# YujiaoShi/HighlyAccurate

Hardware: AMD Instinct MI355X
Metric: image-pairs/sec through N-iter LM pose loop, KITTI shapes (higher is better)
Workload: dtype bf16; 1 GPU; BASELINE configs[1]: LM_S2GP.forward(mode='test'), sat 512x512, grd 256x1024, VGG-16 two-branch, level 3, 5 LM iters x 3 levels, 3-DoF, random-init weights; pairs_per_gpu=32, global_batch=32, parallelism=batch-sharded x1, no collective

## Files before the change

### highlyaccurate_amd/VGG.py

```python
from __future__ import annotations

import ctypes as C

import torch
import torch.nn as nn

from . import _lib

_W_ORDER = ['conv0', 'conv2', 'conv5', 'conv7', 'conv10', 'conv12', 'conv14',
            'conv_dec1.1', 'conv_dec1.3', 'conv_dec2.1', 'conv_dec2.3', 'conv_dec3.1', 'conv_dec3.3',
            'conf0.1', 'conf1.1', 'conf2.1', 'conf3.1']
_LEVEL_SEL = {-1: [0], -2: [1], -3: [2], 2: [1, 2], 3: [0, 1, 2], 4: [0, 1, 2, 3]}
_CH = (256, 128, 64, 16)


def _dtype_code(precision: str) -> int:
    if precision == 'bf16':
        return _lib.HLA_BF16
    if precision == 'fp16':
        return _lib.HLA_F16
    if precision == 'fp32':
        return _lib.HLA_F32
    if precision == 'fp16x3':
        return _lib.HLA_F16X3
# ... 21 lines not shown
            b = sd[name + '.bias']
            if i == 0:
                versions.append((b.data_ptr(), b._version))
            b = b.detach().contiguous().float()
            keep.append(b)
            prm.b[i] = b.data_ptr()
    return prm, keep, tuple(versions)


def _packed_weights(module: 'VGGUnet', prm, versions, dt: int, device):
    key = (dt, str(device), versions)
    cache = module.__dict__.setdefault('_hla_packed', {})
    if cache.get('key') != key:
        lib = _lib.load()
        buf = cache.get('buf')
        nbytes = lib.hla_vgg_packed_weight_bytes(dt)
        if buf is None or buf.numel() != nbytes or buf.device != device:
            buf = torch.empty(nbytes, dtype=torch.uint8, device=device)
        _lib.check(lib.hla_vgg_pack_weights(C.byref(prm), _lib.ptr(buf), dt, _lib.stream_ptr()), 'hla_vgg_pack_weights')
        cache['key'], cache['buf'] = key, buf
    return cache['buf']


def _image_window(x: torch.Tensor):
    x = x.float()
    B, _, H, W = x.shape
    sb, sc, sh, sw = x.stride()
    if not (sw == 1 and sh == W and sc >= H * W and (B == 1 or sb == 3 * sc)):
        x = x.contiguous()
        sc = H * W
    return x, sc


@_lib.on_device(lambda module, x, *a, **k: x)
def vgg_forward_nhwc(module: 'VGGUnet', x: torch.Tensor, want_conf: bool = True, defer_norm: bool = False,
                     save_for_backward: bool = False, first_row8: int = 0, feat16: bool = False):
    _lib.require_gpu(x, 'VGGUnet input')
    if x.dim() != 4 or x.shape[1] != 3:
        raise ValueError(f'expected [B,3,H,W], got {tuple(x.shape)}')
    lib = _lib.load()
    x, x_plane = _image_window(x)
    B, _, H, W = x.shape
    _lib.same_device(('input', x), ('parameters', module.conv0.weight))
    dt = _dtype_code(module.precision)
    prm, keep, versions = _param_table(module)
    packed = _packed_weights(module, prm, versions, dt, x.device)
    L = 4 if module.level == 4 else 3
    fdt = torch.float32
    if feat16:
        if not (defer_norm and not save_for_backward and L == 3 and dt in (_lib.HLA_BF16, _lib.HLA_F16)):
            raise ValueError("feat16 needs precision 'bf16' / 'fp16', defer_norm=True, level 3 and no save_for_backward")
        fdt = torch.float16
    fold = bool(getattr(module, 'folded', False))
    if fold:
        if feat16 or first_row8:
            raise ValueError('VGGUnet_G2S: feat16 / first_row8 do not apply to the folded maps')
        if W % 16:
            raise ValueError(f'VGGUnet_G2S folds [h,w] -> [2h,w/2] down to the W/8-wide map: W must be a multiple of 16, got {W}')

    def hw(l, folded):
        h, w = H >> (3 - l), W >> (3 - l)
        return (2 * h, w // 2) if folded else (h, w)

    feats = [torch.empty(B, *hw(l, fold), 64 if l == 3 else _CH[l], device=x.device, dtype=fdt) for l in range(L)]
    confs = [torch.empty(B, *hw(l, fold and l > 0), device=x.device, dtype=torch.float32) if want_conf else None
             for l in range(L)]
    inv_norm = torch.empty(L, B, device=x.device, dtype=torch.float64)
    fp = (C.c_void_p * 4)(*([f.data_ptr() for f in feats] + [0] * (4 - L)))
    cp = (C.c_void_p * 4)(*([(c.data_ptr() if c is not None else 0) for c in confs] + [0] * (4 - L)))
    flags = (_lib.HLA_VGG_WANT_CONF if want_conf else 0) | (_lib.HLA_VGG_DEFER_NORM if defer_norm else 0) | \
            (_lib.HLA_VGG_FEAT16 if feat16 else 0) | (_lib.HLA_VGG_FOLD_DECODER if fold else 0)
    nbytes = lib.hla_vgg_workspace_bytes_flags(B, H, W, L, dt, flags) if fold else lib.hla_vgg_workspace_bytes(B, H, W, L, dt)
    ws = torch.empty(nbytes, dtype=torch.uint8, device=x.device)
    if save_for_backward:
        if not defer_norm:
            raise ValueError('save_for_backward needs defer_norm=True (the backward works on the raw maps)')
        flags |= _lib.HLA_VGG_SAVE_FOR_BACKWARD
    rc = lib.hla_vgg_forward(_lib.ptr(x), x_plane, C.byref(prm), _lib.ptr(packed), fp, cp, _lib.ptr(inv_norm), _lib.ptr(ws), nbytes,
                             B, H, W, L, dt, flags, int(first_row8), _lib.stream_ptr())
    _lib.check(rc, 'hla_vgg_forward')
    if save_for_backward:
        return feats, confs, inv_norm, dict(x=x, x_version=x._version, x_plane=x_plane, ws=ws, feats=feats, inv_norm=inv_norm, dt=dt, L=L)
    return feats, confs, inv_norm


@_lib.on_device(lambda module, ctx, *a, **k: ctx['x'])
def vgg_backward_nhwc(module: 'VGGUnet', ctx: dict, d_feats, confs=None, d_confs=None, scale_invariant: bool = False,
                      first_row8: int = 0, flat: bool = False, dense: bool = False, stats: dict = None,
                      wgrad_two_phase: int = 0):
    lib = _lib.load()
    x, dt = ctx['x'], ctx['dt']
    if x._version != ctx.get('x_version', x._version):
        raise RuntimeError('the input image saved for the backward of VGGUnet has been modified by an inplace operation '
                           f"(version {x._version}, expected {ctx['x_version']}): conv0's weight gradient reads it again")
    B, _, H, W = x.shape
    prm, keep, versions = _param_table(module)
    cache = module.__dict__.setdefault('_hla_packed_T', {})
    key = (dt, str(x.device), versions)
    if cache.get('key') != key:
        buf = torch.empty(lib.hla_vgg_packed_weight_T_bytes(dt), dtype=torch.uint8, device=x.device)
        _lib.check(lib.hla_vgg_pack_weights_T(C.byref(prm), _lib.ptr(buf), dt, _lib.stream_ptr()), 'hla_vgg_pack_weights_T')
        cache['key'], cache['buf'] = key, buf
    sd = dict(module.named_parameters())
    grads, gs = {}, _lib.VggGrads()
    shapes = [(name + '.weight', tuple(sd[name + '.weight'].shape)) for name in _W_ORDER[:11]] + \
             [(name + '.bias', tuple(sd[name + '.bias'].shape)) for name in _W_ORDER[:7]]
    sizes = [int(torch.Size(shp).numel()) for _, shp in shapes]
    flat_buf = torch.empty(sum(sizes), device=x.device, dtype=torch.float32)
    o = 0
    for (key, shp), n in zip(shapes, sizes):
        grads[key] = flat_buf[o:o + n].view(shp)
        o += n
    for i, name in enumerate(_W_ORDER[:11]):
        gs.dw[i] = grads[name + '.weight'].data_ptr()
        if i < 7:
            gs.db[i] = grads[name + '.bias'].data_ptr()
    L = ctx.get('L', 3)
    padded = {}
    if L == 4:
        for i, name, shape in ((11, 'conv_dec3.1', (64, 128, 3, 3)), (12, 'conv_dec3.3', (64, 64, 3, 3))):
            g = torch.empty(shape, device=x.device, dtype=torch.float32)
            padded[name + '.weight'] = g
            gs.dw[i] = g.data_ptr()
    cp = dcp = None
    if d_confs is not None:
        dcs = [d.contiguous().float() for d in d_confs]
        cp = (C.c_void_p * 4)(*([c.data_ptr() for c in confs] + [0] * (4 - L)))
        dcp = (C.c_void_p * 4)(*([d.data_ptr() for d in dcs] + [0] * (4 - L)))
        for l in range(L):
            name = f'conf{l}.1.weight'
            if l == 3:
                g = torch.empty(1, 64, 3, 3, device=x.device, dtype=torch.float32)
                padded[name] = g
            else:
                g = torch.empty_like(sd[name], dtype=torch.float32, memory_format=torch.contiguous_format)
                grads[name] = g
            gs.dw[13 + l] = g.data_ptr()
    dfs = [d.contiguous().float() for d in d_feats]
    fp = (C.c_void_p * 4)(*([f.data_ptr() for f in ctx['feats']] + [0] * (4 - L)))
    dp = (C.c_void_p * 4)(*([d.data_ptr() for d in dfs] + [0] * (4 - L)))
    fold = bool(getattr(module, 'folded', False))
    nbytes = lib.hla_vgg_bwd_workspace_bytes_flags(B, H, W, L, dt, _lib.HLA_VGG_BWD_FOLD_DECODER) if fold \
        else lib.hla_vgg_bwd_workspace_bytes(B, H, W, L, dt)
    ws = torch.empty(nbytes, dtype=torch.uint8, device=x.device)
    rc = lib.hla_vgg_backward(_lib.ptr(x), ctx.get('x_plane', 0), C.byref(prm), _lib.ptr(cache['buf']), _lib.ptr(ctx['ws']), fp, _lib.ptr(ctx['inv_norm']),
                              dp, cp, dcp, C.byref(gs), _lib.ptr(ws), nbytes, B, H, W, L, dt,
                              (_lib.HLA_VGG_BWD_SCALE_INVARIANT if scale_invariant else 0)
                              | (_lib.HLA_VGG_BWD_DENSE if dense else 0)
                              | (_lib.HLA_VGG_BWD_WGRAD_TWO_PHASE if int(wgrad_two_phase) & 1 else 0)
                              | (_lib.HLA_VGG_BWD_WGRAD0_UNFUSED if int(wgrad_two_phase) & 2 else 0)
                              | (_lib.HLA_VGG_BWD_FOLD_DECODER if getattr(module, 'folded', False) else 0),
                              int(first_row8), _lib.stream_ptr())
    _lib.check(rc, 'hla_vgg_backward')
    if stats is not None and fold:
        stats['live_tiles'], stats['total_tiles'] = 0, 0
    elif stats is not None:
        torch.cuda.current_stream().synchronize()
        live, total = C.c_longlong(0), C.c_longlong(0)
        _lib.check(lib.hla_vgg_backward_live_tiles(_lib.ptr(ws), B, H, W, L, dt, C.byref(live), C.byref(total)),
                   'hla_vgg_backward_live_tiles')
        stats['live_tiles'], stats['total_tiles'] = live.value, total.value
    for name, g in padded.items():
        co, ci = sd[name].shape[:2]
        grads[name] = g[:co, :ci].contiguous()
    return (grads, flat_buf) if flat else grads

# ... 78 lines not shown
```

### highlyaccurate_amd/_lib.py

```python
from __future__ import annotations

import ctypes as C
import os

import torch

HERE = os.path.dirname(os.path.abspath(__file__))
LIB_PATH = os.environ.get('HLA_LIB') or os.path.join(HERE, 'libhla.so')

HLA_F32, HLA_BF16, HLA_F16, HLA_F16X3 = 0, 1, 2, 3
HLA_VGG_WANT_CONF, HLA_VGG_DEFER_NORM, HLA_VGG_SAVE_FOR_BACKWARD, HLA_VGG_FEAT16 = 1, 2, 4, 8
HLA_VGG_FOLD_DECODER = 16
HLA_VGG_BWD_SCALE_INVARIANT = 1
HLA_VGG_BWD_DENSE = 2
HLA_VGG_BWD_WGRAD_TWO_PHASE = 4
HLA_VGG_BWD_WGRAD0_UNFUSED = 8
HLA_VGG_BWD_FOLD_DECODER = 16
ABI_VERSION = 24


class HlaError(RuntimeError):
    pass


class VggParams(C.Structure):
    _fields_ = [('w', C.c_void_p * 17), ('b', C.c_void_p * 7)]


class S2GLevel(C.Structure):
    _fields_ = [('sat_feat', C.c_void_p), ('grd_feat', C.c_void_p), ('grd_conf', C.c_void_p), ('xyz', C.c_void_p),
                ('sat_inv_norm', C.c_void_p), ('grd_inv_norm', C.c_void_p),
                ('A', C.c_int), ('h', C.c_int), ('w', C.c_int), ('C', C.c_int), ('row0', C.c_int), ('grd_row_skip', C.c_int),
                ('meter_per_pixel', C.c_double), ('centre', C.c_double), ('feat_dtype', C.c_int)]


class S2GConfig(C.Structure):
    _fields_ = [('ford', C.c_int), ('n_levels', C.c_int), ('n_iters', C.c_int), ('level_first', C.c_int),
                ('using_weight', C.c_int), ('use_hessian', C.c_int), ('dof', C.c_int),
                ('shift_range_lat', C.c_double), ('shift_range_lon', C.c_double), ('rotation_range', C.c_double),
                ('damping', C.c_double * 3), ('keep', C.c_void_p), ('keep_stride', C.c_size_t),
                ('optimizer', C.c_int), ('beta1', C.c_double), ('beta2', C.c_double), ('count_in_view', C.c_int),
                ('grd_grad_overwrite', C.c_int), ('deterministic', C.c_int), ('proj', C.c_int)]


class FillRegion(C.Structure):
    _fields_ = [('ptr', C.c_void_p), ('chunk_bytes', C.c_size_t), ('stride_bytes', C.c_size_t), ('n_chunks', C.c_int)]


class VggGrads(C.Structure):
    _fields_ = [('dw', C.c_void_p * 17), ('db', C.c_void_p * 7)]


class S2GLevelGrad(C.Structure):
    _fields_ = [('d_sat_feat', C.c_void_p), ('d_grd_feat', C.c_void_p), ('d_grd_conf', C.c_void_p)]


class ProfRecord(C.Structure):
    _fields_ = [('kernel_id', C.c_int), ('ms', C.c_float), ('flops', C.c_double), ('bytes', C.c_double)]


HLA_POSE_LOSS_F32, HLA_POSE_LOSS_F64 = 0, 1


class PoseLossArgs(C.Structure):
    _fields_ = [('x', C.c_void_p * 3), ('x_stride', (C.c_longlong * 3) * 3), ('gt', C.c_void_p * 3), ('gt_stride', C.c_longlong * 3),
                ('coe', C.c_double * 3), ('B', C.c_int), ('N', C.c_int), ('L', C.c_int), ('gt_dtype', C.c_int)]


_lib = None


def _check_binary(lib: C.CDLL, path: str) -> None:
    lib.hla_abi_version.restype = C.c_int
    have = lib.hla_abi_version()
    if have != ABI_VERSION:
        raise HlaError(f'{path}: ABI version {have}, this binding needs {ABI_VERSION}; rebuild it '
                       f'(python -m highlyaccurate_amd.build --force)')
    try:
        fn = lib.hla_sizeof_struct
    except AttributeError:
        raise HlaError(f'{path}: no hla_sizeof_struct export; rebuild it') from None
    fn.restype, fn.argtypes = C.c_size_t, [C.c_int]
    for sid, cls in enumerate((VggParams, VggGrads, S2GLevel, S2GConfig, S2GLevelGrad, ProfRecord, PoseLossArgs, FillRegion)):
        if fn(sid) != C.sizeof(cls):
            raise HlaError(f'{path}: sizeof({cls.__name__}) is {fn(sid)} in the library and {C.sizeof(cls)} in the binding')


def load() -> C.CDLL:
    global _lib
    if _lib is not None:
        return _lib
    from . import build as _b
    try:
        want = _b.source_hash()
    except _b.SourcesMissing as e:
        if not os.path.exists(LIB_PATH):
            raise HlaError(f'{LIB_PATH} is missing and so are its sources: {e}') from None
        want = _b.lib_hash(LIB_PATH)
    if _b.lib_hash(LIB_PATH) != want and not (os.environ.get('HLA_LIB') and os.environ.get('HLA_ALLOW_STALE') == '1'):
        if os.environ.get('HLA_LIB'):
            raise HlaError(f'{LIB_PATH} (HLA_LIB) was not built from the sources in {_b.CSRC}; rebuild it')
        if not _b.have_compiler():
            what = 'is missing' if not os.path.exists(LIB_PATH) else 'is stale (built from different sources)'
            raise HlaError(f'{LIB_PATH} {what} and there is no hipcc to rebuild it; highlyaccurate_amd has no fallback path')
        _b.build()
    lib = C.CDLL(LIB_PATH)
    _check_binary(lib, LIB_PATH)
    vp, i, sz = C.c_void_p, C.c_int, C.c_size_t
    lib.hla_last_error.restype = C.c_char_p
    lib.hla_source_hash.restype = C.c_char_p
    lib.hla_vgg_workspace_bytes.restype = sz
    lib.hla_vgg_workspace_bytes.argtypes = [i, i, i, i, i]
    lib.hla_vgg_workspace_bytes_flags.restype = sz
    lib.hla_vgg_workspace_bytes_flags.argtypes = [i, i, i, i, i, i]
    lib.hla_vgg_forward.restype = i
    lib.hla_vgg_forward.argtypes = [vp, sz, C.POINTER(VggParams), vp, C.POINTER(vp), C.POINTER(vp), vp, vp, sz,
                                    i, i, i, i, i, i, i, vp]
    lib.hla_vgg_packed_weight_bytes.restype = sz
    lib.hla_vgg_packed_weight_bytes.argtypes = [i]
    lib.hla_vgg_pack_weights.restype = i
    lib.hla_vgg_pack_weights.argtypes = [C.POINTER(VggParams), vp, i, vp]
    lib.hla_vgg_packed_weight_T_bytes.restype = sz
    lib.hla_vgg_packed_weight_T_bytes.argtypes = [i]
    lib.hla_vgg_pack_weights_T.restype = i
    lib.hla_vgg_pack_weights_T.argtypes = [C.POINTER(VggParams), vp, i, vp]
    lib.hla_vgg_bwd_workspace_bytes.restype = sz
    lib.hla_vgg_bwd_workspace_bytes.argtypes = [i, i, i, i, i]
    lib.hla_vgg_bwd_workspace_bytes_flags.restype = sz
    lib.hla_vgg_bwd_workspace_bytes_flags.argtypes = [i, i, i, i, i, i]
    lib.hla_vgg_backward_live_tiles.restype = i
    lib.hla_vgg_backward_live_tiles.argtypes = [vp, i, i, i, i, i, C.POINTER(C.c_longlong), C.POINTER(C.c_longlong)]
    lib.hla_vgg_backward.restype = i
    lib.hla_vgg_backward.argtypes = [vp, sz, C.POINTER(VggParams), vp, vp, C.POINTER(vp), vp, C.POINTER(vp), C.POINTER(vp), C.POINTER(vp), C.POINTER(VggGrads),
                                     vp, sz, i, i, i, i, i, i, i, vp]
    lib.hla_resize_bilinear.restype = i
    lib.hla_resize_bilinear.argtypes = [vp, vp, vp, i, vp, vp, i, vp, vp, i, i, i, i, i, vp]
    lib.hla_sat_tile.restype = i
    lib.hla_sat_tile.argtypes = [vp, vp, vp, i, i, i, vp]
    lib.hla_grid_sample.restype = i
    lib.hla_grid_sample.argtypes = [vp, vp, vp, vp, vp, i, i, i, i, i, i, i, vp]
    lib.hla_grid_sample_bwd.restype = i
    lib.hla_grid_sample_bwd.argtypes = [vp, vp, vp, vp, vp, vp, vp, vp, i, i, i, i, i, i, i, vp]
    lib.hla_s2g_workspace_bytes.restype = sz
    lib.hla_s2g_workspace_bytes.argtypes = [C.POINTER(S2GConfig), C.POINTER(S2GLevel), i]
    lib.hla_g2s_workspace_bytes.restype = sz
    lib.hla_g2s_workspace_bytes.argtypes = [C.POINTER(S2GConfig), C.POINTER(S2GLevel), i]
    lib.hla_g2s_lm_solve.restype = i
    lib.hla_g2s_lm_solve.argtypes = [C.POINTER(S2GConfig), C.POINTER(S2GLevel), vp, i, i, vp, vp, vp, vp, sz, i, vp]
    lib.hla_g2s_bwd_workspace_bytes.restype = sz
    lib.hla_g2s_bwd_workspace_bytes.argtypes = [C.POINTER(S2GConfig), C.POINTER(S2GLevel), i]
    lib.hla_g2s_lm_solve_bwd.restype = i
    lib.hla_g2s_lm_solve_bwd.argtypes = [C.POINTER(S2GConfig), C.POINTER(S2GLevel), C.POINTER(S2GLevelGrad), vp, i, i, vp, vp,
                                         vp, vp, vp, vp, sz, i, vp]
    lib.hla_s2g_lm_solve.restype = i
    lib.hla_s2g_lm_solve.argtypes = [C.POINTER(S2GConfig), C.POINTER(S2GLevel), vp, vp, vp, vp, vp, vp, vp, sz, i, vp]
    lib.hla_s2g_bwd_workspace_bytes.restype = sz
    lib.hla_s2g_bwd_workspace_bytes.argtypes = [C.POINTER(S2GConfig), C.POINTER(S2GLevel), i]
    lib.hla_s2g_lm_solve_bwd.restype = i
    lib.hla_s2g_lm_solve_bwd.argtypes = [C.POINTER(S2GConfig), C.POINTER(S2GLevel), C.POINTER(S2GLevelGrad), vp, vp, vp, vp,
                                         vp, vp, vp, vp, sz, i, vp]
    lib.hla_zero_fill.restype = i
    lib.hla_zero_fill.argtypes = [C.POINTER(FillRegion), i, i, vp]
    lib.hla_pose_loss.restype = i
    lib.hla_pose_loss.argtypes = [C.POINTER(PoseLossArgs), vp, vp]
    lib.hla_pose_loss_bwd.restype = i
    lib.hla_pose_loss_bwd.argtypes = [C.POINTER(PoseLossArgs), C.POINTER(vp), C.POINTER(vp), C.POINTER((C.c_longlong * 3) * 3), vp]
    ll, dbl = C.c_longlong, C.c_double
    lib.hla_orien_corr_workspace_bytes.restype = sz
    lib.hla_orien_corr_workspace_bytes.argtypes = [i, i, i, i, i]
    lib.hla_orien_corr.restype = i
    lib.hla_orien_corr.argtypes = [vp, vp, vp, vp, vp, vp, vp, vp, vp, sz, i, i, i, i, i, vp]
    lib.hla_orien_corr_bwd.restype = i
    lib.hla_orien_corr_bwd.argtypes = [vp, vp, vp, vp, vp, vp, vp, vp, vp, vp, vp, sz, i, i, i, i, i, vp]
    lib.hla_orien_window_bwd.restype = i
    lib.hla_orien_window_bwd.argtypes = [vp, vp, vp, vp, i, i, i, i, i, i, vp]
    lib.hla_orien_triplet_loss.restype = i
    lib.hla_orien_triplet_loss.argtypes = [vp, vp, ll, dbl, dbl, vp, i, i, i, vp]
    lib.hla_orien_triplet_loss_bwd.restype = i
    lib.hla_orien_triplet_loss_bwd.argtypes = [vp, vp, ll, dbl, dbl, vp, vp, i, i, vp]
    lib.hla_prof_enable.restype = i
    lib.hla_prof_enable.argtypes = [i]
    lib.hla_prof_kernel_name.restype = C.c_char_p
    lib.hla_prof_kernel_name.argtypes = [i]
    lib.hla_prof_mfma_peak.restype = i
    lib.hla_prof_mfma_peak.argtypes = [i, i, C.c_float, C.POINTER(C.c_float), vp]
    lib.hla_prof_fetch.restype = i
    lib.hla_prof_fetch.argtypes = [C.POINTER(ProfRecord), i, C.POINTER(i)]
    _lib = lib
    return lib


def zero_fill(regions, max_blocks: int = 0, stream=None) -> None:
    if not regions:
        return
    arr = (FillRegion * len(regions))()
    for k, (t, cb, sb, n) in enumerate(regions):
        arr[k].ptr = t.data_ptr() if hasattr(t, 'data_ptr') else int(t)
        arr[k].chunk_bytes, arr[k].stride_bytes, arr[k].n_chunks = int(cb), int(sb), int(n)
    check(load().hla_zero_fill(arr, len(regions), int(max_blocks), stream_ptr() if stream is None else stream), 'hla_zero_fill')

# ... 60 lines not shown
```

### highlyaccurate_amd/_s2gp.py

```python
from __future__ import annotations

import ctypes as C

import numpy as np
import torch
import torch.nn as nn

from . import _lib, utils
from .VGG import VGGUnet, vgg_forward_nhwc, vgg_backward_nhwc

KITTI_K = [[582.9802, 0.0, 496.2420], [0.0, 482.7076, 125.0034], [0.0, 0.0, 1.0]]
FORD_K_FL = [945.391406, 0.0, 855.502825, 0.0, 945.668274, 566.372868, 0.0, 0.0, 1.0]
FORD_H_FL, FORD_W_FL = 860, 1656


_FEAT_DTYPES = {torch.float32: _lib.HLA_F32, torch.bfloat16: _lib.HLA_BF16, torch.float16: _lib.HLA_F16}

PHASE_HOOK = None


def _phase(name: str):
    h = PHASE_HOOK
    if h is not None:
        h(name)


def ground_plane_table(K_ori, grd_H, grd_W, ori_H, ori_W):
    K = torch.tensor(K_ori, dtype=torch.float32).reshape(1, 3, 3)
    Ks = K.clone()
    Ks[:, :1, :] = K[:, :1, :] * grd_W / ori_W
    Ks[:, 1:2, :] = K[:, 1:2, :] * grd_H / ori_H
    Kinv = torch.inverse(Ks)
    v, u = torch.meshgrid(torch.arange(0, grd_H, dtype=torch.float32),
                          torch.arange(0, grd_W, dtype=torch.float32), indexing='ij')
    uv1 = torch.stack([u, v, torch.ones_like(u)], dim=-1).unsqueeze(0)
    xyz_w = torch.sum(Kinv[:, None, None, :, :] * uv1[:, :, :, None, :], dim=-1)
    y = xyz_w[..., 1:2]
    w = utils.Camera_height / torch.where(torch.abs(y) > utils.EPS, y, utils.EPS * torch.ones_like(y))
    return (xyz_w * w)[0].contiguous()


def polar_plane_table(grd_H, grd_W):
    v, u = torch.meshgrid(torch.arange(0, grd_H, dtype=torch.float32),
                          torch.arange(0, grd_W, dtype=torch.float32), indexing='ij')
    theta = u / grd_W * np.pi / 4
    radius = (1 - v / grd_H) * 30
    z = radius * torch.cos(np.pi / 4 - theta)
    x = -radius * torch.sin(np.pi / 4 - theta)
    y = utils.Camera_height * torch.ones_like(z)
    return torch.stack([x, y, z], dim=-1).contiguous()


def ford_K_network_input():
    K = torch.tensor(FORD_K_FL, dtype=torch.float32).reshape(3, 3)
    out = torch.zeros_like(K)
    out[0] = K[0] / FORD_W_FL * 1024
    out[1] = K[1] / FORD_H_FL * 256
    out[2] = K[2]
    return out.tolist()


def _loss_tensor_ops(shift_lats, shift_lons, thetas, gt_shift_lat, gt_shift_lon, gt_theta, coe_shift_lat, coe_shift_lon, coe_theta):
    d_lat = torch.abs(shift_lats - gt_shift_lat[:, None, None]).mean(dim=0)
    d_lon = torch.abs(shift_lons - gt_shift_lon[:, None, None]).mean(dim=0)
    d_th = torch.abs(thetas - gt_theta[:, None, None]).mean(dim=0)
    losses = coe_shift_lat * d_lat + coe_shift_lon * d_lon + coe_theta * d_th
    return (losses.mean(), losses[0] - losses[-1], d_lat[0] - d_lat[-1], d_lon[0] - d_lon[-1], d_th[0] - d_th[-1],
            losses[-1], d_lat[-1], d_lon[-1], d_th[-1])


def _pose_loss_args(xs, gts, coes):
    a = _lib.PoseLossArgs()
    B, N, L = xs[0].shape
    for k in range(3):
        a.x[k], a.gt[k], a.gt_stride[k], a.coe[k] = xs[k].data_ptr(), gts[k].data_ptr(), gts[k].stride(0), float(coes[k])
        for j in range(3):
            a.x_stride[k][j] = xs[k].stride(j)
    a.B, a.N, a.L = B, N, L
    a.gt_dtype = _lib.HLA_POSE_LOSS_F64 if gts[0].dtype == torch.float64 else _lib.HLA_POSE_LOSS_F32
    return a


class _PoseLossFn(torch.autograd.Function):

    @staticmethod
    def forward(ctx, cols, coes, gt_lat, gt_lon, gt_th, *xs):
        views = [xs[0][..., c] for c in cols] if cols is not None else list(xs)
        gts = (gt_lat, gt_lon, gt_th)
        L = views[0].shape[2]
        out = torch.empty(1 + 8 * L, dtype=gt_lat.dtype, device=views[0].device)
        args = _pose_loss_args(views, gts, coes)
        _lib.check(_lib.load().hla_pose_loss(C.byref(args), _lib.ptr(out), _lib.stream_ptr()), 'hla_pose_loss')
# ... 221 lines not shown
        p0 = init_pose.to(dev).float().contiguous() if init_pose is not None else None
        rc = lib.hla_s2g_lm_solve(C.byref(cfg), lv, _lib.ptr(R_FL), _lib.ptr(T_FL), _lib.ptr(p0), _lib.ptr(rand_uv),
                                  _lib.ptr(trace), _lib.ptr(neq), _lib.ptr(ws), nbytes, B, _lib.stream_ptr())
        _lib.check(rc, 'hla_s2g_lm_solve')
        risky = cfg.optimizer == 3 or (cfg.optimizer == 0 and (cfg.use_hessian or min(cfg.damping[i] for i in range(3)) <= 0.0))
        if risky or strict:
            raise_like_reference(trace, neq[:, :, 14] if strict else None, level_first,
                                 gn_norm2=neq[:, :, 0] if cfg.optimizer == 3 else None)
        self.last_trace, self.last_normal_eq = trace.detach(), neq
        return trace

    def lm_grad_buffers(self, sat_feats, grd_feats, grd_confs, row0s, row_skips, grd_first_row8=0, overwrite=True, deterministic=False):
        L = len(sat_feats)
        regions = []
        d_sat = [torch.empty_like(t) for t in sat_feats]
        if not deterministic:
            regions += [(d, d.numel() * 4, d.numel() * 4, 1) for d in d_sat]
        d_grd = []
        for l, t in enumerate(grd_feats):
            d = torch.empty_like(t)
            lo, hi = (max(0, (grd_first_row8 << l) - 2) if grd_first_row8 else 0), row0s[l] - row_skips[l]
            if not overwrite:
                hi = t.shape[1]
            if hi > lo:
                row = t.shape[2] * t.shape[3] * 4
                regions.append((d.data_ptr() + lo * row, (hi - lo) * row, t.shape[1] * row, t.shape[0]))
            d_grd.append(d)
        d_conf = [torch.empty_like(grd_confs[l]) if (self.using_weight and grd_confs[l] is not None) else None for l in range(L)]
        regions += [(d, d.numel() * 4, d.numel() * 4, 1) for d in d_conf if d is not None]
        d_lambda = torch.empty(4, device=sat_feats[0].device, dtype=torch.float64)
        keep = d_sat + d_grd
        for k0 in range(0, len(regions), 16):
            _lib.zero_fill(regions[k0:k0 + 16])
        del keep
        return d_sat, d_grd, d_conf, d_lambda

    @_lib.on_device(lambda self, sat_feats, *a, **k: sat_feats[0])
    def lm_backward(self, sat_feats, grd_feats, grd_confs, grd_hw, trace, normal_eq, d_trace, extra=None, level_first=0,
                    init_pose=None, sat_inv_norm=None, grd_inv_norm=None, keep=None, grd_first_row8=0, overwrite=True):
        lib = _lib.load()
        dev = sat_feats[0].device
        B, L = sat_feats[0].shape[0], len(sat_feats)
        cfg, lv, R_FL, T_FL = self._lm_structs(sat_feats, grd_feats, grd_confs, grd_hw, extra, level_first,
                                               sat_inv_norm, grd_inv_norm)
        if keep is not None:
            cfg.keep, cfg.keep_stride = keep.data_ptr(), keep.shape[1]
        det = bool(getattr(self.args, 'deterministic_backward', 0))
        cfg.deterministic = 1 if det else 0
        cfg.grd_grad_overwrite = 1 if overwrite else 0
        d_sat, d_grd, d_conf, d_lambda = self.lm_grad_buffers(sat_feats, grd_feats, grd_confs, [lv[l].row0 for l in range(L)],
                                                              [lv[l].grd_row_skip for l in range(L)], grd_first_row8, overwrite, det)
        gr = (_lib.S2GLevelGrad * L)()
        for l in range(L):
            gr[l].d_sat_feat, gr[l].d_grd_feat = d_sat[l].data_ptr(), d_grd[l].data_ptr()
            gr[l].d_grd_conf = d_conf[l].data_ptr() if d_conf[l] is not None else 0
        dtr = d_trace.to(dev).float().contiguous()
        nbytes = lib.hla_s2g_bwd_workspace_bytes(C.byref(cfg), lv, B)
        ws = torch.empty(nbytes, dtype=torch.uint8, device=dev)
        p0 = init_pose.to(dev).float().contiguous() if init_pose is not None else None
        for attempt, bits in enumerate((1, 30) if det else (0,)):
            cfg.deterministic = bits
            if attempt:
                for t in d_conf:
                    if t is not None:
                        t.zero_()
                if not overwrite:
                    for t in d_grd:
                        t.zero_()
            rc = lib.hla_s2g_lm_solve_bwd(C.byref(cfg), lv, gr, _lib.ptr(R_FL), _lib.ptr(T_FL), _lib.ptr(p0), _lib.ptr(trace),
                                          _lib.ptr(normal_eq), _lib.ptr(dtr), _lib.ptr(d_lambda), _lib.ptr(ws), nbytes, B,
                                          _lib.stream_ptr())
            _lib.check(rc, 'hla_s2g_lm_solve_bwd')
            if not det or float(d_lambda[3]) == 0.0:
                break
        else:
            raise RuntimeError(f'deterministic_backward: the fixed-point range of d(loss)/d(sat map) was exceeded in {int(d_lambda[3])} '
                               '(step, sample) pairs even with 2^20 of head room -- the adjoints of the LM chain grow by more than that '
                               'from its last step to an earlier one; the result is not valid (run without args.deterministic_backward)')
        return d_sat, d_grd, d_conf, d_lambda[:3]

    def _features(self, sat_map, grd_img, want_conf, return_confs):
        f16 = (self.SatFeatureNet.precision in ('bf16', 'fp16') and self.level == 3 and bool(getattr(self.args, 'lm_feat16', 1)))
        small = sat_map.shape[0] <= int(getattr(self.args, 'small_batch_two_streams', 4))
        if small:
            cur = torch.cuda.current_stream()
            side = _side_stream(sat_map.device)
            side.wait_stream(cur)
            with torch.cuda.stream(side):
                sat_feats, _, sat_inv = vgg_forward_nhwc(self.SatFeatureNet, sat_map, want_conf=False, defer_norm=True, feat16=f16)
            sat_map.record_stream(side)
        else:
            sat_feats, _, sat_inv = vgg_forward_nhwc(self.SatFeatureNet, sat_map, want_conf=False, defer_norm=True, feat16=f16)
        grd_in = grd_img
        dead_ok = (not return_confs and self.level == 3 and getattr(self.args, 'Optimizer', 'LM') == 'LM'
                   and bool(getattr(self.args, 'ground_crop', 1)) and not self.polar)
        skip = dead_ground_rows(grd_img.shape[-2]) if dead_ok else 0
        if skip:
            grd_in = grd_img[:, :, skip:, :]
        f8 = ((grd_img.shape[-2] // 8) // 2 - skip // 8) if dead_ok else 0
        f8 = f8 if f8 >= 4 else 0
        grd_feats, grd_confs, grd_inv = vgg_forward_nhwc(self.GrdFeatureNet, grd_in, want_conf=want_conf, defer_norm=True,
                                                         first_row8=f8, feat16=f16)
        if small:
            cur.wait_stream(side)
            for t in list(sat_feats) + [sat_inv]:
                t.record_stream(cur)
        L = self._levels
        return L(sat_feats), L(sat_inv), L(grd_feats), L(grd_confs), L(grd_inv)

    @_lib.on_device(lambda self, sat_map, *a, **k: sat_map)
    def localise(self, sat_map, grd_img, want_conf, extra, level_first, init_pose, return_confs=True):
        if sat_map.dim() != 4 or grd_img.dim() != 4 or sat_map.shape[0] != grd_img.shape[0] or sat_map.shape[1] != 3 \
                or grd_img.shape[1] != 3 or sat_map.shape[2] != sat_map.shape[3]:
            raise ValueError(f'expected sat_map [B,3,A,A] and grd_img [B,3,H,W] with one B, got {tuple(sat_map.shape)} '
                             f'and {tuple(grd_img.shape)}')
        _lib.same_device(('sat_map', sat_map), ('grd_img', grd_img), ('parameters', self.damping))
        if self.polar and self.ford and level_first:
            raise NotImplementedError("LM_S2GP_Ford(proj='polar') with level_first=1: the reference's level-first loop reads only "
                                      "the bottom half of the polar maps (it has no proj branch); that combination is not built")
        if torch.is_grad_enabled() and any(p.requires_grad for p in self.parameters()):
            names = [n for n, _ in self.named_parameters()]
            params = [p for _, p in self.named_parameters()]
            out = _LocaliseFn.apply(self, names, sat_map, grd_img, want_conf, extra, level_first, init_pose, *params)
            return out[0], list(out[1:]) if want_conf else [None] * self.level
        sat_feats, sat_inv, grd_feats, grd_confs, grd_inv = self._features(sat_map, grd_img, want_conf, return_confs)
        trace = self.lm_solve(sat_feats, grd_feats, grd_confs, grd_img.shape[-2:], extra, level_first, init_pose,
                              sat_inv, grd_inv)
        return trace, grd_confs


def draw_reinit(n_steps: int, B: int, device):
    r = torch.rand(n_steps, 2, B).mul_(2.0).add_(-1.0)
    if torch.device(device).type == 'cuda':
        return r.pin_memory().to(device, non_blocking=True)
    return r.to(device)


def raise_like_reference(trace, in_view, level_first, gn_norm2=None):
    B, N, L, _ = trace.shape
    steps = N * L
    tr = (trace.permute(0, 2, 1, 3) if level_first else trace).reshape(B, steps, 3)
    bad = ~torch.isfinite(tr).all(-1)
    if gn_norm2 is not None:
        first = torch.where(bad.any(1), bad.float().argmax(1), torch.full((B,), steps - 1, device=bad.device))
        poisoned = bad.any(1) & (gn_norm2.t().gather(1, first[:, None])[:, 0] == 0)
        bad = bad & ~poisoned[:, None]
    bad = bad.any(0)
    k_s = int(torch.nonzero(bad)[0]) if bool(bad.any()) else steps
    k_a = steps
    if in_view is not None:
        empty = in_view.sum(1) == 0
        k_a = int(torch.nonzero(empty)[0]) if bool(empty.any()) else steps
    if k_a < steps and k_a <= k_s:
        raise AssertionError(f'grid_sample: no pixel of the batch is sampled inside the map in LM step {k_a} (jacobian.py:172)')
    if k_s < steps:
        raise RuntimeError(f'linalg.inv: the normal matrix of LM step {k_s} is singular '
                           '(use_hessian / zero damping / Gauss-Newton with no Jacobian support in one pose component)')


_SIDE_STREAMS = {}


def _side_stream(device) -> 'torch.cuda.Stream':
    idx = torch.device(device).index if torch.device(device).index is not None else torch.cuda.current_device()
    st = _SIDE_STREAMS.get(idx)
    if st is None:
        st = _SIDE_STREAMS[idx] = torch.cuda.Stream(device=idx)
    return st


def dead_ground_rows(H: int) -> int:
    return max(0, ((H // 2 - 34) // 8) * 8)


def _bwd_first_row8(model, grd_hw, x21_rows: int) -> int:
    inv = getattr(model.args, 'Optimizer', 'LM') == 'LM' and not model.polar
    f8 = (grd_hw[0] // 8) // 2 - (grd_hw[0] - x21_rows * 2) // 8
    return f8 if (inv and f8 >= 4 and model.level == 3 and bool(getattr(model.args, 'bwd_trim', 1))) else 0


class _LocaliseFn(torch.autograd.Function):

    @staticmethod
# ... 98 lines not shown
```

### highlyaccurate_amd/csrc/capi.hip

```cpp
#include "common.h"
#include <string.h>

static thread_local char g_err[512] = "";

void hla_set_error(const char* fmt, ...) {
  va_list ap;
  va_start(ap, fmt);
  vsnprintf(g_err, sizeof(g_err), fmt, ap);
  va_end(ap);
}

extern "C" const char* hla_last_error(void) { return g_err; }
extern "C" int hla_abi_version(void) { return HLA_ABI_VERSION; }

#ifndef HLA_SOURCE_HASH_HEX
#define HLA_SOURCE_HASH_HEX "unknown"
#endif
static const char kSourceHash[] = "HLA_SOURCE_HASH=" HLA_SOURCE_HASH_HEX;
extern "C" const char* hla_source_hash(void) { return kSourceHash + 16; }

extern "C" size_t hla_sizeof_struct(int id) {
  switch (id) {
    case HLA_STRUCT_VGG_PARAMS: return sizeof(hla_vgg_params);
    case HLA_STRUCT_VGG_GRADS: return sizeof(hla_vgg_grads);
    case HLA_STRUCT_S2G_LEVEL: return sizeof(hla_s2g_level);
    case HLA_STRUCT_S2G_CONFIG: return sizeof(hla_s2g_config);
    case HLA_STRUCT_S2G_LEVEL_GRAD: return sizeof(hla_s2g_level_grad);
    case HLA_STRUCT_PROF_RECORD: return sizeof(hla_prof_record);
    case HLA_STRUCT_POSE_LOSS_ARGS: return sizeof(hla_pose_loss_args);
    case HLA_STRUCT_FILL_REGION: return sizeof(hla_fill_region);
    default: return 0;
  }
}
```

### highlyaccurate_amd/csrc/conv_kernels.h

```cpp
#pragma once
#include "common.h"
#include <type_traits>

typedef __bf16 bf16;
typedef _Float16 f16;
using f32x16 = __attribute__((ext_vector_type(16))) float;
using bf16x8 = __attribute__((ext_vector_type(8))) __bf16;
using f16x8 = __attribute__((ext_vector_type(8))) _Float16;
using f16x4 = __attribute__((ext_vector_type(4))) _Float16;

struct split32 {
  float v;
  split32() = default;
  __host__ __device__ explicit split32(float f) : v(f) {}
  __host__ __device__ explicit operator float() const { return v; }
};
template <typename T> struct Prec { static constexpr bool SPLIT = false; static constexpr int CEPL = 16 / (int)sizeof(T); };
template <> struct Prec<split32> { static constexpr bool SPLIT = true; static constexpr int CEPL = 8; };

__device__ __host__ __forceinline__ float split_scale(unsigned amax_bits) {
  int E = (int)(amax_bits >> 23) & 0xff;
  E = E < 81 ? 81 : (E > 201 ? 201 : E);
  const unsigned bits = (unsigned)(127 + 141 - E) << 23;
  float f;
// ... 234 lines not shown
    constexpr int EPV = 16 / (int)sizeof(E), NIT = 32 * CPP / 64;
    if (PLAIN || !(mask || add)) {
#pragma unroll
      for (int c0 = 0; c0 < 32 * CPP; c0 += 64) {
        const int c = c0 + lane;
        if (c0 < chunks && c < chunks) {
          const int px = c / CPP, part = c % CPP;
          if (px < npx_valid) {
            const unsigned off = (unsigned)px * (unsigned)Cout * (unsigned)sizeof(E) + part * 16;
            *(uint4*)((char*)dst + off) = *(const uint4*)(stage + px * PITCH + part * 16);
          }
        }
      }
      return vmax;
    }
    constexpr int G = NIT < GG ? NIT : GG;
#pragma unroll
    for (int g0 = 0; g0 < NIT; g0 += G) {
      bool ok[G], ap[G];
      unsigned off[G];
      int pxs[G], parts[G];
      uint4 mk[G], ad[G];
#pragma unroll
      for (int k = 0; k < G; ++k) {
        const int c0 = (g0 + k) * 64, c = c0 + lane;
        const int px = c / CPP, part = c % CPP;
        ok[k] = c0 < chunks && c < chunks && px < npx_valid;
        pxs[k] = px; parts[k] = part;
        off[k] = ok[k] ? (unsigned)px * (unsigned)Cout * (unsigned)sizeof(E) + part * 16 : 0u;
        ap[k] = add && ok[k] && px >= add_px_lo && px < add_px_hi;
      }
      if (mask) {
#pragma unroll
        for (int k = 0; k < G; ++k) mk[k] = *(const uint4*)((const char*)mask + off[k]);
      }
      if (add) {
#pragma unroll
        for (int k = 0; k < G; ++k) ad[k] = *(const uint4*)((const char*)add + (ap[k] ? off[k] : 0u));
      }
#pragma unroll
      for (int k = 0; k < G; ++k) {
        if (ok[k]) {
          uint4 v = *(const uint4*)(stage + pxs[k] * PITCH + parts[k] * 16);
          E e[EPV], m[EPV], a2[EPV];
          __builtin_memcpy(e, &v, 16);
          if (mask) __builtin_memcpy(m, &mk[k], 16);
          if (add) __builtin_memcpy(a2, &ad[k], 16);
#pragma unroll
          for (int j = 0; j < EPV; ++j) {
            float f = (float)e[j];
            if (mask && !((float)m[j] > 0.f)) f = 0.f;
            if (ap[k]) f += (float)a2[j];
            e[j] = (E)f;
            vmax = fmaxf(vmax, fabsf(f));
          }
          __builtin_memcpy(&v, e, 16);
          *(uint4*)((char*)dst + off[k]) = v;
        }
      }
    }
    return vmax;
  }
};

enum { EPI_GENERIC = 0,
       EPI_ACT = 1,
       EPI_ACT_RAW = 2,
       EPI_ACT_RAW_NOBIAS = 3,
       EPI_DGRAD = 4,
       EPI_DGRAD_WG0 = 5 };
__host__ __device__ __forceinline__ int epilogue_mode(const ConvArgs& a) {
  if (a.wg0_part) return EPI_DGRAD_WG0;
  if (a.mask_act && a.out_act && !a.relu_act && !a.bias && !a.out_raw && !a.sumsq && !a.idx_out && !a.pool_sum) return EPI_DGRAD;
  if (!a.out_act && a.out_raw && a.raw16 && a.sumsq && !a.bias && !a.mask_act && !a.add_src && !a.idx_out && !a.pool_sum)
    return EPI_ACT_RAW_NOBIAS;
  if (a.mask_act || a.add_src || a.idx_out || a.pool_sum || !a.out_act || !a.relu_act) return EPI_GENERIC;
  if (!a.out_raw) return a.sumsq ? EPI_GENERIC : EPI_ACT;
  return a.sumsq ? (a.bias ? EPI_ACT_RAW : EPI_ACT_RAW_NOBIAS) : EPI_GENERIC;
}
template <typename T, int MT, int NT, bool POOL, int EPI = EPI_GENERIC, bool R16 = false, int STGW = 0, int SHAPE = SHAPE_32x32x16>
__device__ __forceinline__ void conv_epilogue(typename AccMap<SHAPE>::Tile (&acc)[MT][NT], const ConvArgs& a, int b, int yrow0, int x0,
                                              int cb, float* red, char* stage, float dsc = 1.f,
                                              PixBox addb = PixBox{0, 1 << 30, 0, 1 << 30},
                                              const float4* prebias = nullptr) {
  using RawT = std::conditional_t<R16, f16, float>;
  constexpr bool GEN = EPI == EPI_GENERIC, RAW = EPI == EPI_ACT_RAW || EPI == EPI_ACT_RAW_NOBIAS, DG = EPI == EPI_DGRAD;
  constexpr bool NOBIAS = EPI == EPI_ACT_RAW_NOBIAS || DG || sizeof(T) == 2;
  const bool has_raw = GEN ? a.out_raw != nullptr : RAW;
  const bool has_act = GEN ? a.out_act != nullptr : true;
  const bool relu = GEN ? a.relu_act != 0 : !DG;
  const bool pool_sum = GEN && a.pool_sum;
  const bool has_sumsq = GEN ? a.sumsq != nullptr : RAW;
  int tid = threadIdx.x;
  asm volatile("" : "+v"(tid));
  const int lane = tid & 63, wv = __builtin_amdgcn_readfirstlane(tid >> 6), even = !POOL || !(lane & 1);
  using M = AccMap<SHAPE>;
  const int Ho = POOL ? a.H >> 1 : a.H, Wo = POOL ? a.W >> 1 : a.W;
  constexpr int NPX = POOL ? 16 : 32;
  int pxq[4];
  bool colok[4];
#pragma unroll
  for (int q = 0; q < 4; ++q) {
    const int xq = M::px(lane, q);
    pxq[q] = POOL ? xq >> 1 : xq;
    colok[q] = (x0 + xq < a.W) && even;
  }
  float4 bias[NT][4];
#pragma unroll
  for (int j = 0; j < NT; ++j)
#pragma unroll
    for (int q = 0; q < 4; ++q)
      bias[j][q] = make_float4(0.f, 0.f, 0.f, 0.f);
  if (!NOBIAS && prebias) {
#pragma unroll
    for (int j = 0; j < NT; ++j)
#pragma unroll
      for (int q = 0; q < 4; ++q) bias[j][q] = prebias[j * 4 + q];
  } else if (!NOBIAS && a.bias) {
#pragma unroll
    for (int j = 0; j < NT; ++j)
#pragma unroll
      for (int q = 0; q < 4; ++q) bias[j][q] = *(const float4*)(a.bias + cb + j * 32 + M::ch(lane, q));
  }
  const int xo0 = POOL ? x0 >> 1 : x0;
  const int nvalid = min(NPX, Wo - xo0);
  float ss = 0.f, mx = 0.f;
  constexpr int ROWB = 32 * RowStager<T, NT>::PITCH;
  constexpr bool BATCH = EPI == EPI_ACT && STGW >= 2 * ROWB;
  if constexpr (BATCH) {
    constexpr int STEP = POOL ? 2 : 1, NR = MT / STEP;
    constexpr int RB = STGW / ROWB >= NR ? NR : 2;
    static_assert(NR % RB == 0, "row batches");
#pragma unroll
    for (int r0 = 0; r0 < NR; r0 += RB) {
#pragma unroll
      for (int rr = 0; rr < RB; ++rr) {
        const int i = (r0 + rr) * STEP;
        const bool rowok = yrow0 + i < a.H;
#pragma unroll
        for (int j = 0; j < NT; ++j)
#pragma unroll
          for (int q = 0; q < 4; ++q) {
            float w[4];
#pragma unroll
            for (int e = 0; e < 4; ++e) {
              float t = M::get(acc[i][j], q, e);
              if (POOL) {
                t = fmaxf(t, M::get(acc[i + 1][j], q, e));
                t = fmaxf(t, lane_xor1(t));
              }
              if (Prec<T>::SPLIT) t *= dsc;
              w[e] = t;
            }
            if (!NOBIAS) { w[0] += bias[j][q].x; w[1] += bias[j][q].y; w[2] += bias[j][q].z; w[3] += bias[j][q].w; }
            w[0] = fmaxf(w[0], 0.f); w[1] = fmaxf(w[1], 0.f); w[2] = fmaxf(w[2], 0.f); w[3] = fmaxf(w[3], 0.f);
            if (Prec<T>::SPLIT && rowok && colok[q]) mx = fmaxf(fmaxf(mx, fmaxf(w[0], w[1])), fmaxf(w[2], w[3]));
            if (even) RowStager<T, NT>::put(stage + rr * ROWB, pxq[q], j * 32 + M::ch(lane, q), w[0], w[1], w[2], w[3]);
          }
      }
      __builtin_amdgcn_sched_barrier(0);
#pragma unroll
      for (int rr = 0; rr < RB; ++rr) {
        const int y = yrow0 + (r0 + rr) * STEP;
        const size_t pix0 = ((size_t)b * Ho + (POOL ? y >> 1 : y)) * Wo + xo0;
        if (y < a.H) RowStager<T, NT>::template flush<true>(stage + rr * ROWB, (T*)a.out_act + pix0 * a.Cout + cb, NPX, nvalid, a.Cout, lane);
      }
      __builtin_amdgcn_sched_barrier(0);
// ... 48 lines not shown
              w2 = (float)(f16)fminf(fmaxf(w2, -65504.f), 65504.f); w3 = (float)(f16)fminf(fmaxf(w3, -65504.f), 65504.f);
            }
            RowStager<RawT, NT>::put(stage, pxq[q], j * 32 + M::ch(lane, q), w0, w1, w2, w3);
            if (quad_ok(q)) ss = sumsq4(ss, w0, w1, w2, w3);
            if (a.out_act)
              RowStager<T, NT>::put(stage2, pxq[q], j * 32 + M::ch(lane, q), fmaxf(w0, 0.f), fmaxf(w1, 0.f), fmaxf(w2, 0.f), fmaxf(w3, 0.f));
          }
      }
      asm volatile("" : "+v"(ss));
      __builtin_amdgcn_sched_barrier(0);
      if (row_ok) {
        RowStager<RawT, NT>::template flush<true>(stage, (RawT*)a.out_raw + pix0 * a.Cout + cb, NPX, nvalid, a.Cout, lane);
        if (a.out_act) RowStager<T, NT>::template flush<true>(stage2, (T*)a.out_act + pix0 * a.Cout + cb, NPX, nvalid, a.Cout, lane);
      }
      __builtin_amdgcn_sched_barrier(0);
      continue;
    }
    if (has_raw) {
      if (even) {
#pragma unroll
        for (int j = 0; j < NT; ++j)
#pragma unroll
          for (int q = 0; q < 4; ++q) {
            RowStager<float, NT>::put(stage, pxq[q], j * 32 + M::ch(lane, q), v[j][q][0], v[j][q][1], v[j][q][2], v[j][q][3]);
            if (quad_ok(q)) ss = sumsq4(ss, v[j][q][0], v[j][q][1], v[j][q][2], v[j][q][3]);
          }
      }
      if (row_ok) RowStager<float, NT>::template flush<true>(stage, a.out_raw + pix0 * a.Cout + cb, NPX, nvalid, a.Cout, lane);
    }
    if (has_act) {
      if (even) {
#pragma unroll
        for (int j = 0; j < NT; ++j)
#pragma unroll
          for (int q = 0; q < 4; ++q) {
            float w0 = v[j][q][0], w1 = v[j][q][1], w2 = v[j][q][2], w3 = v[j][q][3];
            if (relu) { w0 = fmaxf(w0, 0.f); w1 = fmaxf(w1, 0.f); w2 = fmaxf(w2, 0.f); w3 = fmaxf(w3, 0.f); }
            if (Prec<T>::SPLIT && quad_ok(q) && !((GEN || DG) && (a.mask_act || a.add_src)))
              mx = fmaxf(fmaxf(mx, fmaxf(fabsf(w0), fabsf(w1))), fmaxf(fabsf(w2), fabsf(w3)));
            RowStager<T, NT>::put(stage, pxq[q], j * 32 + M::ch(lane, q), w0, w1, w2, w3);
          }
      }
      const size_t o = pix0 * a.Cout + cb;
      if (GEN || DG) {
        if (row_ok) {
          const float fm = RowStager<T, NT>::template flush<false, (MT >= 4 ? 4 : 2)>(stage, (T*)a.out_act + o, NPX, nvalid, a.Cout, lane,
                                                   a.mask_act ? (const T*)a.mask_act + o : nullptr,
                                                   (a.add_src && yo >= max(a.add_row_lo, addb.y0) && yo < addb.y1) ? (const T*)a.add_src + o : nullptr,
                                                   addb.x0 - xo0, addb.x1 - xo0);
          if (Prec<T>::SPLIT) mx = fmaxf(mx, fm);
        }
      } else {
        if (row_ok) RowStager<T, NT>::template flush<true>(stage, (T*)a.out_act + o, NPX, nvalid, a.Cout, lane);
      }
    }
    if (GEN && POOL && a.idx_out) {
#pragma unroll
      for (int j = 0; j < NT; ++j)
#pragma unroll
        for (int q = 0; q < 4; ++q) {
          float am[4];
#pragma unroll
          for (int e = 0; e < 4; ++e) {
            const float t0 = M::get(acc[i][j], q, e), u = M::get(acc[i + 1][j], q, e);
            const float rown = u > t0 ? 1.f : 0.f;
            const float t = fmaxf(t0, u);
            const float t2 = lane_xor1(t), r2 = lane_xor1(rown);
            am[e] = t2 > t ? 2.f * r2 + 1.f : 2.f * rown;
          }
          if (!(lane & 1)) RowStager<unsigned char, NT>::put(stage, pxq[q], j * 32 + M::ch(lane, q), am[0], am[1], am[2], am[3]);
        }
      if (row_ok) RowStager<unsigned char, NT>::flush(stage, a.idx_out + pix0 * a.Cout + cb, NPX, nvalid, a.Cout, lane);
    }
  }
  const bool want_max = Prec<T>::SPLIT && a.amax_out;
  if (has_sumsq || want_max) {
    ss = wave_sum_f32(ss);
    if (want_max) mx = wave_max_f32(mx);
    if (lane == 0) { red[wv] = ss; red[4 + wv] = mx; }
    __syncthreads();
    if (tid == 0) {
      if (has_sumsq) {
        const int np = a.tiles_x * a.tiles_y * gridDim.y;
        const int tile = (xcd_contiguous(blockIdx.x, gridDim.x) % (a.tiles_x * a.tiles_y)) * gridDim.y + blockIdx.y;
        a.sumsq[(size_t)b * np + tile] = ((double)red[0] + (double)red[1]) + ((double)red[2] + (double)red[3]);
      }
      if (want_max) {
        const unsigned mb = __float_as_uint(fmaxf(fmaxf(red[4], red[5]), fmaxf(red[6], red[7])));
        if (mb > __hip_atomic_load(a.amax_out + b, __ATOMIC_RELAXED, __HIP_MEMORY_SCOPE_AGENT)) atomicMax(a.amax_out + b, mb);
      }
    }
  }
}

template <typename T, int MT>
__device__ __forceinline__ void conv_epilogue_wg0(f32x16 (&acc)[MT][1], const ConvArgs& a, int b, int y0, int x0, char* lds, float dsc) {
  constexpr bool SPLIT = Prec<T>::SPLIT;
  using ET = std::conditional_t<SPLIT, float, T>;
  using FT = std::conditional_t<SPLIT, f16, ET>;
  constexpr int TH = 2 * MT, IH = TH + 2, IW = 48;
  constexpr int PITCH = RowStager<ET, 1>::PITCH, CPP = RowStager<ET, 1>::CPP, NIT = 32 * CPP / 64, EPV = 16 / (int)sizeof(ET);
  constexpr int HP = RowStager<f16, 1>::PITCH, HTILE = 32 * HP;
  constexpr int KPX = KStep<FT>::PX, STG = 5120;
  static_assert(32 * PITCH <= STG && 2 * HTILE <= STG, "wave stager");
  static_assert(4 * STG + 3 * IH * IW * 4 + 2 * 16 * 64 * 4 + 16 <= 2 * (TH + 2) * HWID * PSTR, "fits the halo buffers");
  int tid = threadIdx.x;
  asm volatile("" : "+v"(tid));
  const int lane = tid & 63, wv = __builtin_amdgcn_readfirstlane(tid >> 6), wm = wv >> 1, wn = wv & 1, x = lane & 31, g = lane >> 5;
  char* stage = lds + wv * STG;
  float* in = (float*)(lds + 4 * STG);
  float* xr = in + 3 * IH * IW;
  float* redm = xr + 2 * 16 * 64;
  const int nvalid = min(32, a.W - x0), cb = wn * 32;

  int pxs[NIT], parts[NIT];
  unsigned voff[NIT];
#pragma unroll
  for (int k = 0; k < NIT; ++k) {
    const int c = k * 64 + lane;
    pxs[k] = c / CPP; parts[k] = c % CPP;
    voff[k] = pxs[k] < nvalid ? (unsigned)pxs[k] * 64u * (unsigned)sizeof(ET) + parts[k] * 16 : 0u;
  }
  constexpr int PRE = sizeof(ET) == 2 ? MT : 2;
  uint4 mk[MT][NIT];
  auto load_mask = [&](int i) __attribute__((always_inline)) {
    const int y = min(y0 + wm * MT + i, a.H - 1);
    const char* mrow = (const char*)((const ET*)a.mask_act + (((size_t)b * a.H + y) * a.W + x0) * 64 + cb);
#pragma unroll
    for (int k = 0; k < NIT; ++k) mk[i][k] = *(const uint4*)(mrow + voff[k]);
  };
#pragma unroll
  for (int i = 0; i < PRE; ++i) load_mask(i);

  constexpr int NIN = (3 * IH * IW + 255) / 256;
  float vin[NIN], amx = 0.f;
#pragma unroll
  for (int it = 0; it < NIN; ++it) {
    const int e = tid + it * 256;
    const int c = e / (IH * IW), r = e % (IH * IW), iy = r / IW, ix = r % IW;
    const int y = y0 - 1 + iy, xx = x0 - 1 + ix;
    vin[it] = 0.f;
    if (e < 3 * IH * IW && ix < HWID && y >= 0 && y < a.H && xx >= 0 && xx < a.W)
      vin[it] = a.wg0_x[((size_t)b * 3 + c) * a.wg0_x_plane + (size_t)y * a.W + xx];
  }
#pragma unroll
  for (int it = 0; it < NIN; ++it) {
    const int e = tid + it * 256;
    if (e < 3 * IH * IW) in[e] = vin[it];
    if (SPLIT) amx = fmaxf(amx, fabsf(vin[it]));
  }
  if (SPLIT) {
    amx = wave_max_f32(amx);
    if (lane == 0) redm[wv] = amx;
  }
  __syncthreads();
  float s_in = 1.f;
  if (SPLIT) s_in = split_scale(__float_as_uint(fmaxf(fmaxf(redm[0], redm[1]), fmaxf(redm[2], redm[3]))));

  f32x16 accw;
#pragma unroll
  for (int r = 0; r < 16; ++r) accw[r] = 0.f;
  const int j = lane & 31, g5 = lane >> 5;
  const int jc = j < 27 ? j / 9 : 0, jky = (j % 9) / 3, jkx = j % 3;
#pragma unroll
  for (int i = 0; i < MT; ++i) {
    if (i + PRE < MT) load_mask(i + PRE);
    const int rt = wm * MT + i;
// ... 101 lines not shown
  const uint4* wq[NT];

  __device__ __forceinline__ void prime() {
#pragma unroll
    for (int d = 0; d < WD; ++d)
#pragma unroll
      for (int kg = 0; kg < 2; ++kg)
#pragma unroll
        for (int j = 0; j < NT; ++j) wb[d][kg][j] = wq[j][(d * 2 + kg) * 64];
  }
  __device__ __forceinline__ void next_stage() {
#pragma unroll
    for (int j = 0; j < NT; ++j) wq[j] += 18 * 64;
    if (9 % RS != 0) {
      uint4 tmp[WD][2][NT];
#pragma unroll
      for (int d = 0; d < WD; ++d)
#pragma unroll
        for (int kg = 0; kg < 2; ++kg)
#pragma unroll
          for (int j = 0; j < NT; ++j) tmp[d][kg][j] = wb[(9 + d) % RS][kg][j];
#pragma unroll
      for (int d = 0; d < WD; ++d)
#pragma unroll
        for (int kg = 0; kg < 2; ++kg)
#pragma unroll
          for (int j = 0; j < NT; ++j) wb[d][kg][j] = tmp[d][kg][j];
    }
  }
};

__device__ __forceinline__ void stagger_priority() {
  const unsigned slot = __builtin_amdgcn_s_getreg((3 << 11) | (0 << 6) | 4);
  if (slot & 1) __builtin_amdgcn_s_setprio(1);
}

template <typename T, int MT, int NT, int WD, int PF, int SHAPE = SHAPE_32x32x16, typename Mid>
__device__ __forceinline__ void stage_mma(typename AccMap<SHAPE>::Tile (&acc)[MT][NT], const char* cur, const FragOff& fo,
                                          WeightRing<T, MT, NT, WD, PF>& ring, Mid&& mid) {
  constexpr int RS = WD + 1;
#pragma unroll
  for (int tap = 0; tap < 9; ++tap) {
#pragma unroll
    for (int kg = 0; kg < 2; ++kg)
#pragma unroll
      for (int j = 0; j < NT; ++j) ring.wb[(tap + WD) % RS][kg][j] = ring.wq[j][((tap + WD) * 2 + kg) * 64];
    mid(tap);
    constexpr int FPT = MT * 2, DEPTH = PF;
    auto frag_ptr = [&](int f) {
      const int tp = tap + f / FPT, r = f % FPT;
      return cur + fo.o[tp % 3][r & 1] + (tp / 3 + (r >> 1)) * HWID * PSTR;
    };
    if (tap == 0) {
#pragma unroll
      for (int f = 0; f < DEPTH; ++f) ring.pf[f] = *(const uint4*)frag_ptr(f);
    }
    __builtin_amdgcn_sched_barrier(0);
#pragma unroll
    for (int f = 0; f < FPT; ++f) {
      const int slot = (tap * FPT + f) % (DEPTH + 1), nslot = (tap * FPT + f + DEPTH) % (DEPTH + 1);
      if (tap * FPT + f + DEPTH < 9 * FPT) ring.pf[nslot] = *(const uint4*)frag_ptr(f + DEPTH);
      const int i = f >> 1, kg = f & 1;
      if constexpr (Prec<T>::SPLIT) {
#pragma unroll
        for (int c = 0; c < (kg == 0 ? 2 : 1); ++c)
#pragma unroll
          for (int j = 0; j < NT; ++j) mma16<T>(acc[i][j], ring.wb[tap % RS][c][j], ring.pf[slot]);
      } else if constexpr (SHAPE == SHAPE_16x16x32) {
#pragma unroll
        for (int c = 0; c < 2; ++c)
#pragma unroll
          for (int j = 0; j < NT; ++j) mma32<T>(acc[i][j].t[2 * kg + c], ring.wb[tap % RS][c][j], ring.pf[slot]);
      } else {
#pragma unroll
        for (int j = 0; j < NT; ++j) mma16<T>(acc[i][j], ring.wb[tap % RS][kg][j], ring.pf[slot]);
      }
      __builtin_amdgcn_sched_barrier(0);
    }
  }
  ring.next_stage();
}

template <typename T, int MT, int NT, int WM, int WN, bool POOL, int WD, bool UNPOOL = false, int SHAPE = SHAPE_32x32x16>
__global__ __launch_bounds__(256, NT == 1 ? 3 : 2) void conv3x3_kernel(ConvArgs a) {
  static_assert(WM * WN == 4, "4 waves per block");
  static_assert(SHAPE == SHAPE_32x32x16 || (sizeof(T) == 2 && !UNPOOL), "16x16x32: bf16 / f16 forward kernels only");
  using M = AccMap<SHAPE>;
  constexpr int EPL = 16 / sizeof(T), KC = SB / sizeof(T);
  constexpr int TH = WM * MT, HPIX = (TH + 2) * HWID;
  constexpr int NPIECE = (HPIX * 4 + 255) / 256;
  constexpr bool DMA = sizeof(T) == 2 && !UNPOOL && !Prec<T>::SPLIT;
  constexpr int BUF = (DMA ? NPIECE * 64 : HPIX) * PSTR;
  constexpr int NHALF = (NPIECE + 1) / 2;
  constexpr int STG = 32 * (RowStager<float, NT>::PITCH + (sizeof(T) == 2 ? RowStager<T, NT>::PITCH : 0));
  constexpr int LDSB = 2 * BUF > 4 * STG ? 2 * BUF : 4 * STG;
  __shared__ __attribute__((aligned(16))) char lds[LDSB];
  __shared__ float red[8];

  HLA_STAMP(0);
  HLA_STAMP_HWID();
  const int t = threadIdx.x, lane = t & 63, wv = __builtin_amdgcn_readfirstlane(t >> 6), wm = wv / WN, wn = wv % WN;
  const int sy0 = a.src_row_lo, sy1 = a.H;
  int tx, ty, b;
  struct { int lo0, lo1, lo2, hi0, hi1, hi2; } sb = {0, 0, 0, a.W, a.W, a.W};
  if (a.dyn) {
    const ConvDyn& d = *(const ConvDyn*)(a.dyn + a.dyn_desc);
    const int nl = d.n_live, nlive = nl * a.B;
    if ((int)blockIdx.x >= nlive) return;
    int bid = xcd_contiguous(blockIdx.x, nlive);
    b = bid / nl;
    const int e = a.dyn[d.list + bid % nl];
    ty = e >> 16; tx = e & 0xffff;
    if (d.src_bands >= 0) {
      const int sh = (a.up1 || a.unpool_idx) ? 1 : 0, nb = ((a.H >> sh) + 7) >> 3, yy = a.row_begin + ty * TH;
      const int b0 = min(max(yy - 1, 0) >> sh >> 3, nb - 1), b1 = min(yy >> sh >> 3, nb - 1), b2 = min((yy + TH) >> sh >> 3, nb - 1);
      sb.lo0 = a.dyn[d.src_bands + 2 * b0] << sh; sb.hi0 = min(a.dyn[d.src_bands + 2 * b0 + 1] << sh, a.W);
      sb.lo1 = a.dyn[d.src_bands + 2 * b1] << sh; sb.hi1 = min(a.dyn[d.src_bands + 2 * b1 + 1] << sh, a.W);
      sb.lo2 = a.dyn[d.src_bands + 2 * b2] << sh; sb.hi2 = min(a.dyn[d.src_bands + 2 * b2 + 1] << sh, a.W);
    }
  } else {
    int bid = xcd_contiguous(blockIdx.x, gridDim.x);
    tx = bid % a.tiles_x; bid /= a.tiles_x;
    ty = bid % a.tiles_y;
    b = bid / a.tiles_y;
  }
  const int y0 = a.row_begin + ty * TH, x0 = tx * 32;
  const int nstage = (a.C1 + a.C2) / KC;
  const int part = t & 3, pbase = t >> 2;
  float sx = 1.f, dsc = 1.f;
  if constexpr (Prec<T>::SPLIT) {
    unsigned m = a.amax1[b];
    if (a.amax2) m = max(m, a.amax2[b]);
    sx = split_scale(m);
    dsc = 1.f / (sx * *a.wscale);
  }

  constexpr int ES = (int)sizeof(T);
  const int sh1 = (a.up1 || a.unpool_idx) ? 1 : 0, Hs1 = a.H >> sh1, Ws1 = a.W >> sh1;
  const char* s1b = (const char*)a.src1 + (size_t)b * Hs1 * Ws1 * a.C1 * ES;
  const char* s2b = (const char*)a.src2 + (size_t)b * a.H * a.W * a.C2 * ES;
  const unsigned char* idxb = a.unpool_idx ? a.unpool_idx + (size_t)b * Hs1 * Ws1 * a.C1 : nullptr;
  int off1[NPIECE], off2[NPIECE], wo[NPIECE];
  {
    const int lo0 = __builtin_amdgcn_readfirstlane(sb.lo0), lo1 = __builtin_amdgcn_readfirstlane(sb.lo1),
              lo2 = __builtin_amdgcn_readfirstlane(sb.lo2), hi0 = __builtin_amdgcn_readfirstlane(sb.hi0),
              hi1 = __builtin_amdgcn_readfirstlane(sb.hi1), hi2 = __builtin_amdgcn_readfirstlane(sb.hi2);
#pragma unroll
    for (int i = 0; i < NPIECE; ++i) {
      const int pix = pbase + 64 * i;
      const int hy = pix / HWID, hx = pix - hy * HWID;
      const int y = y0 - 1 + hy, x = x0 - 1 + hx;
      const int xlo = hy == 0 ? lo0 : (hy == TH + 1 ? lo2 : lo1), xhi = hy == 0 ? hi0 : (hy == TH + 1 ? hi2 : hi1);
      const bool ok = pix < HPIX && y >= sy0 && y < sy1 && x >= xlo && x < xhi;
      const int psrc = DMA ? (part ^ halo_key(hx)) : part;
      constexpr int BAD = DMA ? (int)0x80000000 : -1;
      off1[i] = ok ? ((((y >> sh1) * Ws1 + (x >> sh1)) * a.C1 * ES + psrc * 16) | (DMA ? 0 : (((y & 1) << 1) | (x & 1)))) : BAD;
      off2[i] = ok ? ((y * a.W + x) * a.C2 * ES + psrc * 16) : BAD;
      wo[i] = pix >= HPIX ? -1 : (Prec<T>::SPLIT ? halo_off(pix, hx, part >> 1) + (part & 1) * 8 : halo_off(pix, hx, part));
    }
  }
  constexpr int IDW = UNPOOL ? (EPL == 8 ? 2 : 1) : 1;
  struct StageIds { unsigned w[NHALF][IDW]; };
  auto load_stage = [&](int sg, int half, uint4 (&st)[NHALF], StageIds& ids) __attribute__((always_inline)) {
    const int c0 = sg * KC;
    const bool first = c0 < a.C1;
    const char* base = first ? s1b + (size_t)c0 * ES : s2b + (size_t)(c0 - a.C1) * ES;
#pragma unroll
    for (int ii = 0; ii < NHALF; ++ii) {
      const int i = half * NHALF + ii;
      uint4 v = make_uint4(0, 0, 0, 0);
      const int o = i < NPIECE ? (first ? off1[i] : off2[i]) : -1;
      if constexpr (UNPOOL) {
#pragma unroll
        for (int k = 0; k < IDW; ++k) ids.w[ii][k] = 0xffffffffu;
      }
      if (o >= 0) {
        const unsigned ob = (unsigned)o & ~15u;
        v = *(const uint4*)(base + ob);
        if constexpr (UNPOOL) {
          const unsigned char* idp = idxb + ob / ES + c0;
#pragma unroll
          for (int k = 0; k < IDW; ++k) ids.w[ii][k] = ((const unsigned*)idp)[k];
        }
      }
      st[ii] = v;
    }
  };
  auto write_stage = [&](char* buf, int sg, int half, uint4 (&st)[NHALF], const StageIds& ids) __attribute__((always_inline)) {
#pragma unroll
    for (int ii = 0; ii < NHALF; ++ii) {
      const int i = half * NHALF + ii;
      const int w = i < NPIECE ? wo[i] : -1;
      if constexpr (UNPOOL) {
        const bool first = sg * KC < a.C1;
        const unsigned pos = (unsigned)(i < NPIECE ? (first ? off1[i] : off2[i]) : 0) & 3u;
        uint4 v = st[ii];
        if constexpr (sizeof(T) == 2) {
          typedef short s16x2 __attribute__((ext_vector_type(2)));
          const unsigned m0 = ids.w[ii][0] ^ (pos * 0x01010101u), m1 = ids.w[ii][1] ^ (pos * 0x01010101u);
          auto keep = [](unsigned m, unsigned sel) {
            s16x2 w2 = __builtin_bit_cast(s16x2, __builtin_amdgcn_perm(0u, m, sel));
            w2 = (w2 - (short)1) >> 15;
            return __builtin_bit_cast(unsigned, w2);
          };
// ... 63 lines not shown

  const int ntg0 = (blockIdx.y * WN + wn) * NT;
  typename M::Tile acc[MT][NT];
#pragma unroll
  for (int j = 0; j < NT; ++j)
#pragma unroll
    for (int q = 0; q < 4; ++q) {
      float4 b4 = make_float4(0.f, 0.f, 0.f, 0.f);
      if (sizeof(T) == 2 && a.bias) b4 = *(const float4*)(a.bias + (ntg0 + j) * 32 + M::ch(lane, q));
#pragma unroll
      for (int i = 0; i < MT; ++i) {
        M::set(acc[i][j], q, 0, b4.x); M::set(acc[i][j], q, 1, b4.y); M::set(acc[i][j], q, 2, b4.z); M::set(acc[i][j], q, 3, b4.w);
      }
    }

  const FragOff fo = frag_offsets<SHAPE>(lane, wm * MT);
  constexpr int PF = NT == 1 ? (UNPOOL && sizeof(T) == 2 ? 3 : 4) : 3;
  WeightRing<T, MT, NT, WD, PF> ring;
#pragma unroll
  for (int j = 0; j < NT; ++j) ring.wq[j] = a.wpk + (size_t)(ntg0 + j) * nstage * 18 * 64 + lane;

  uint4 st[NHALF];
  StageIds ids;
  ring.prime();
  if constexpr (DMA) {
    dma_stage(0, 0);
    asm volatile("s_waitcnt vmcnt(0)" ::: "memory");
  } else {
    uint4 st1[NHALF];
    StageIds ids1;
    load_stage(0, 0, st, ids);
    load_stage(0, 1, st1, ids1);
    write_stage(lds, 0, 0, st, ids);
    write_stage(lds, 0, 1, st1, ids1);
  }
  __syncthreads();
  HLA_STAMP(1);
  stagger_priority();

  for (int sg = 0; sg < nstage; ++sg) {
    const bool more = sg + 1 < nstage;
    char* nxt = lds + ((sg + 1) & 1) * BUF;
    stage_mma<T, MT, NT, WD, PF, SHAPE>(acc, lds + (sg & 1) * BUF, fo, ring, [&](int tap) __attribute__((always_inline)) {
      if constexpr (DMA) {
        if (tap == HLA_CONV_DMA_TAP && more) dma_stage(sg + 1, (sg + 1) & 1);
      } else {
        if (tap == HALO_TAP0 && more) load_stage(sg + 1, 0, st, ids);
        if (tap == HALO_TAP1 && more) { write_stage(nxt, sg + 1, 0, st, ids); load_stage(sg + 1, 1, st, ids); }
      }
    });
    if constexpr (DMA) {
      static_assert(!DMA || HLA_CONV_DMA_TAP <= 8 - WD, "the halo DMA must be issued before the next stage's weight fragments");
      if (more) asm volatile("s_waitcnt vmcnt(%0)" ::"n"(2 * NT * WD) : "memory");
    } else {
      if (more) write_stage(nxt, sg + 1, 1, st, ids);
    }
    if (sg == 0) HLA_STAMP(2);
    __syncthreads();
    if (sg == 0) HLA_STAMP(3);
  }
  HLA_STAMP(4);
  static_assert((LDSB / 4) % 16 == 0, "stager alignment");
  {
    char* stager = lds + wv * (LDSB / 4);
    const int mode = epilogue_mode(a);
    PixBox addb{a.add_row_lo, 1 << 30, 0, 1 << 30};
    if (a.dyn) {
      const ConvDyn& d = *(const ConvDyn*)(a.dyn + a.dyn_desc);
      if (d.add_bands >= 0) {
        const int band = (POOL ? y0 >> 1 : y0) >> 3;
        addb.x0 = a.dyn[d.add_bands + 2 * band];
        addb.x1 = a.dyn[d.add_bands + 2 * band + 1];
      }
    }
    constexpr bool RAW_SPECIAL = POOL || NT == 1;
    constexpr bool T16 = sizeof(T) == 2;
    if constexpr (UNPOOL && NT == 1 && MT == 4 && WN == 2) {
      if (mode == EPI_DGRAD_WG0) {
        conv_epilogue_wg0<T, MT>(acc, a, b, y0, x0, lds, dsc);
        HLA_STAMP(5);
        return;
      }
    }
    if (mode == EPI_ACT) conv_epilogue<T, MT, NT, POOL, EPI_ACT, false, LDSB / 4, SHAPE>(acc, a, b, y0 + wm * MT, x0, ntg0 * 32, red, stager, dsc, addb);
    else if (T16 && RAW_SPECIAL && a.raw16 && mode == EPI_ACT_RAW)
      conv_epilogue<T, MT, NT, POOL, (T16 && RAW_SPECIAL) ? EPI_ACT_RAW : EPI_GENERIC, T16 && RAW_SPECIAL, 0, SHAPE>(acc, a, b, y0 + wm * MT, x0, ntg0 * 32, red, stager, dsc, addb);
    else if (T16 && a.raw16 && mode == EPI_ACT_RAW_NOBIAS)
      conv_epilogue<T, MT, NT, POOL, T16 ? EPI_ACT_RAW_NOBIAS : EPI_GENERIC, T16, 0, SHAPE>(acc, a, b, y0 + wm * MT, x0, ntg0 * 32, red, stager, dsc, addb);
    else if (RAW_SPECIAL && mode == EPI_ACT_RAW) conv_epilogue<T, MT, NT, POOL, RAW_SPECIAL ? EPI_ACT_RAW : EPI_GENERIC, false, 0, SHAPE>(acc, a, b, y0 + wm * MT, x0, ntg0 * 32, red, stager, dsc, addb);
    else if (SHAPE == SHAPE_32x32x16 && mode == EPI_DGRAD)
      conv_epilogue<T, MT, NT, POOL, SHAPE == SHAPE_32x32x16 ? EPI_DGRAD : EPI_GENERIC, false, 0, SHAPE>(acc, a, b, y0 + wm * MT, x0, ntg0 * 32, red, stager, dsc, addb);
    else if ((RAW_SPECIAL || sizeof(T) == 2) && mode == EPI_ACT_RAW_NOBIAS)
      conv_epilogue<T, MT, NT, POOL, (RAW_SPECIAL || sizeof(T) == 2) ? EPI_ACT_RAW_NOBIAS : EPI_GENERIC, false, 0, SHAPE>(acc, a, b, y0 + wm * MT, x0, ntg0 * 32, red, stager, dsc, addb);
    else conv_epilogue<T, MT, NT, POOL, EPI_GENERIC, false, 0, SHAPE>(acc, a, b, y0 + wm * MT, x0, ntg0 * 32, red, stager, dsc, addb);
  }
  HLA_STAMP(5);
}

struct Conv02Args {
  const float* x;
  size_t x_plane;
  const uint4* w0;
  const float* b0;
  const uint4* w2;
  const float* b2;
  void* out_act;
  void* a0_out;
  unsigned char* idx_out;
  void* a2_out;
  int B, H, W, tiles_x, tiles_y;
  int row_begin;
  const float* wtail;
  unsigned* amax_out;
  unsigned* amax_a2_out;
  unsigned* amax_a0_out;
#if HLA_CONV_STAMPS
  unsigned long long* stamps;
#endif
};

template <typename T> constexpr int conv02_rounds() { return sizeof(T) == 4 ? 2 : 1; }
template <typename T> constexpr int conv02_lds_bytes() {
  return (64 * (int)sizeof(T) / SB) / conv02_rounds<T>() * (10 * HWID * PSTR) + 3 * 12 * 36 * 4;
}

template <typename T, int WD>
__global__ __launch_bounds__(256, Prec<T>::SPLIT ? 2 : 3) void conv02_kernel(Conv02Args a0) {
  constexpr bool SPLIT = Prec<T>::SPLIT;
  constexpr bool FOLD = sizeof(T) == 2 && !SPLIT;
  constexpr int EPL = Prec<T>::CEPL, KC = SB / sizeof(T), NSG = 64 / KC, NFRAG = 32 / (2 * EPL), NH = SPLIT ? 2 : 1;
  constexpr int MT = 4, NT = 1, WN = 2, TH = 8, HPIX = (TH + 2) * HWID, BUF = HPIX * PSTR, IW = 36, IH = 12;
  constexpr int ROUNDS = conv02_rounds<T>(), SPR = NSG / ROUNDS, JPR = 2 / ROUNDS;
  extern __shared__ __attribute__((aligned(16))) char smem[];
  char* lds = smem;
  float* in = (float*)(smem + SPR * BUF);
  __shared__ float red[8];
  __shared__ float red2[4];
  float a0mx = 0.f;
#if HLA_CONV_STAMPS
  struct { unsigned long long* stamps; } a = {a0.stamps};
#endif
  HLA_STAMP(0);
  HLA_STAMP_HWID();

  const int t = threadIdx.x, lane = t & 63, wv = __builtin_amdgcn_readfirstlane(t >> 6), wm = wv / WN, wn = wv % WN;
  int bid = blockIdx.x;
  const int tx = bid % a0.tiles_x; bid /= a0.tiles_x;
  const int ty = bid % a0.tiles_y;
  const int b = bid / a0.tiles_y;
  const int y0 = a0.row_begin + ty * TH, x0 = tx * 32;
  const int x = lane & 31, g = lane >> 5;

  WeightRing<T, MT, NT, WD> ring;
  ring.wq[0] = a0.w2 + (size_t)wn * NSG * 18 * 64 + lane;
  ring.prime();

  float amx = 0.f;
  constexpr int NIN = (3 * IH * IW + 255) / 256;
  float vin[NIN];
#pragma unroll
  for (int it = 0; it < NIN; ++it) {
    const int e = t + it * 256;
    const int c = e / (IH * IW), r = e % (IH * IW), iy = r / IW, ix = r % IW;
    const int y = y0 - 2 + iy, xx = x0 - 2 + ix;
    vin[it] = 0.f;
    if (e < 3 * IH * IW && y >= 0 && y < a0.H && xx >= 0 && xx < a0.W)
      vin[it] = a0.x[((size_t)b * 3 + c) * a0.x_plane + (size_t)y * a0.W + xx];
  }
#pragma unroll
  for (int it = 0; it < NIN; ++it) {
    const int e = t + it * 256;
    if (e < 3 * IH * IW) in[e] = vin[it];
    if (SPLIT) amx = fmaxf(amx, fabsf(vin[it]));
  }
  uint4 wf0[JPR][NFRAG][NH];
  auto load_w0 = [&](int j0) __attribute__((always_inline)) {
#pragma unroll
    for (int jj = 0; jj < JPR; ++jj)
#pragma unroll
      for (int f = 0; f < NFRAG; ++f)
#pragma unroll
        for (int h = 0; h < NH; ++h) wf0[jj][f][h] = a0.w0[(((j0 + jj) * NFRAG + f) * NH + h) * 64 + lane];
  };
  load_w0(0);
  if (SPLIT) {
    amx = wave_max_f32(amx);
    if (lane == 0) red[4 + wv] = amx;
  }
  __syncthreads();
  HLA_STAMP(1);

  float4 bias0[JPR][4];
  auto load_b0 = [&](int j0) __attribute__((always_inline)) {
#pragma unroll
    for (int jj = 0; jj < JPR; ++jj)
#pragma unroll
      for (int q = 0; q < 4; ++q) bias0[jj][q] = *(const float4*)(a0.b0 + (j0 + jj) * 32 + q * 8 + g * 4);
  };
  float s_in = 1.f, s_a0 = 1.f, d0 = 1.f, dsc2 = 1.f;
  if constexpr (SPLIT) {
    const float m = fmaxf(fmaxf(red[4], red[5]), fmaxf(red[6], red[7]));
    float bm = fabsf(a0.b0[lane]);
    bm = wave_max_f32(bm);
    s_in = split_scale(__float_as_uint(m));
    s_a0 = split_scale(__float_as_uint(a0.wtail[16] * m + bm));
    d0 = 1.f / (s_in * a0.wtail[0]);
    dsc2 = 1.f / (s_a0 * a0.wtail[1]);
  }
  f32x16 acc[MT][NT];
  float4 bias2[4];
#pragma unroll
  for (int q = 0; q < 4; ++q) bias2[q] = make_float4(0.f, 0.f, 0.f, 0.f);
  const FragOff fo = frag_offsets(lane, wm * MT);
#pragma unroll
  for (int rd = 0; rd < ROUNDS; ++rd) {
  const int j0 = rd * JPR;
  if (rd == 0 && !FOLD) load_b0(0);
  if (rd > 0) __syncthreads();
  for (int m = wv; m * 32 < HPIX; m += 4) {
    const int p = m * 32 + x, pc = p < HPIX ? p : HPIX - 1;
    const int hy = pc / HWID, hx = pc - hy * HWID;
    const float* ib = in + hy * IW + hx;
    const int yy = y0 - 1 + hy, xx = x0 - 1 + hx;
    const bool inside = yy >= 0 && yy < a0.H && xx >= 0 && xx < a0.W;
    f32x16 c0[2];
#pragma unroll
    for (int j = j0; j < j0 + JPR; ++j)
#pragma unroll
      for (int r = 0; r < 16; ++r) c0[j][r] = 0.f;
// ... 84 lines not shown
  for (int sg = 0; sg < SPR; ++sg)
    stage_mma<T, MT, NT, WD>(acc, lds + sg * BUF, fo, ring, [](int) {});
  HLA_STAMP(4);
  if (rd + 1 < ROUNDS) {
#pragma unroll
    for (int jj = 0; jj < JPR; ++jj) {
#pragma unroll
      for (int f = 0; f < NFRAG; ++f)
#pragma unroll
        for (int h = 0; h < NH; ++h) asm volatile("" : "+v"(wf0[jj][f][h].x), "+v"(wf0[jj][f][h].y), "+v"(wf0[jj][f][h].z), "+v"(wf0[jj][f][h].w));
      if (!FOLD) {
#pragma unroll
        for (int q = 0; q < 4; ++q) asm volatile("" : "+v"(bias0[jj][q].x), "+v"(bias0[jj][q].y), "+v"(bias0[jj][q].z), "+v"(bias0[jj][q].w));
      }
    }
  } else if (sizeof(T) == 4) {
#pragma unroll
    for (int q = 0; q < 4; ++q) asm volatile("" : "+v"(bias2[q].x), "+v"(bias2[q].y), "+v"(bias2[q].z), "+v"(bias2[q].w));
  }
  if (rd + 1 == ROUNDS) __builtin_amdgcn_s_waitcnt(0x0F70);
  if (a0.a0_out) {
    constexpr int PPP = 64 * (int)sizeof(T) / 16 / ROUNDS;
    static_assert(TH * 32 * PPP % 256 == 0, "a0 pieces per thread");
    const size_t a0s = (size_t)a0.H * a0.W * 64 * sizeof(T);
    const unsigned long long pb = (unsigned long long)a0.a0_out + (size_t)b * a0s;
    const void* pu = (const void*)(((unsigned long long)__builtin_amdgcn_readfirstlane((int)(unsigned)(pb >> 32)) << 32) |
                                   (unsigned)__builtin_amdgcn_readfirstlane((int)(unsigned)pb));
    const __amdgpu_buffer_rsrc_t ra = __builtin_amdgcn_make_buffer_rsrc((void*)pu, 0, __builtin_amdgcn_readfirstlane((int)a0s), 0x00020000);
    typedef unsigned u32x4 __attribute__((ext_vector_type(4)));
#pragma unroll
    for (int it = 0; it < TH * 32 * PPP / 256; ++it) {
      const int e = t + it * 256;
      const int pxl = e / PPP, piece = e % PPP, sgi = piece / 4, part = piece % 4;
      const int r = pxl / 32, c = pxl % 32, yy = y0 + r, xx = x0 + c;
      const bool ok = yy < a0.H && xx < a0.W;
      const int off = ok ? (yy * a0.W + xx) * 64 * (int)sizeof(T) + (rd * PPP + piece) * 16 : (int)0x80000000;
      const char* sb = lds + sgi * BUF;
      const int hpix = (r + 1) * HWID + c + 1;
      if constexpr (SPLIT) {
        const f16x4 h = __builtin_bit_cast(f16x4, *(const uint2*)(sb + halo_off(hpix, c + 1, part >> 1) + (part & 1) * 8));
        const f16x4 l = __builtin_bit_cast(f16x4, *(const uint2*)(sb + halo_off(hpix, c + 1, 2 + (part >> 1)) + (part & 1) * 8));
        const float is = 1.f / s_a0;
        const float4 o4 = make_float4(((float)h[0] + (float)l[0]) * is, ((float)h[1] + (float)l[1]) * is,
                                      ((float)h[2] + (float)l[2]) * is, ((float)h[3] + (float)l[3]) * is);
        __builtin_amdgcn_raw_buffer_store_b128(__builtin_bit_cast(u32x4, o4), ra, off, 0, 0);
        if (ok) a0mx = fmaxf(fmaxf(a0mx, fmaxf(o4.x, o4.y)), fmaxf(o4.z, o4.w));
      } else {
        __builtin_amdgcn_raw_buffer_store_b128(__builtin_bit_cast(u32x4, *(const uint4*)(sb + halo_off(hpix, c + 1, part))), ra, off, 0, 0);
      }
    }
  }
  }
  if (SPLIT && a0.a0_out && a0.amax_a0_out) {
    a0mx = wave_max_f32(a0mx);
    if (lane == 0) red2[wv] = a0mx;
  }

#if HLA_CONV_STAMPS
  ConvArgs ae{};
#define a ae
#else
  ConvArgs a{};
#endif
  a.bias = a0.b2; a.out_act = a0.out_act; a.B = a0.B; a.H = a0.H; a.W = a0.W; a.Cout = 64; a.relu_act = 1;
  a.tiles_x = a0.tiles_x; a.tiles_y = a0.tiles_y; a.idx_out = a0.idx_out; a.amax_out = a0.amax_out;
  __syncthreads();
  if (SPLIT && a0.a0_out && a0.amax_a0_out && t == 0) {
    const unsigned mb = __float_as_uint(fmaxf(fmaxf(red2[0], red2[1]), fmaxf(red2[2], red2[3])));
    if (mb > __hip_atomic_load(a0.amax_a0_out + b, __ATOMIC_RELAXED, __HIP_MEMORY_SCOPE_AGENT)) atomicMax(a0.amax_a0_out + b, mb);
  }
  const float4* pb2 = sizeof(T) == 4 ? bias2 : nullptr;
  if (a0.a2_out) {
    ConvArgs f = a;
    f.out_act = a0.a2_out; f.idx_out = nullptr; f.amax_out = a0.amax_a2_out;
    conv_epilogue<T, MT, NT, false, EPI_ACT, false, SPR * BUF / 4>(acc, f, b, y0 + wm * MT, x0, wn * 32, red, lds + wv * (SPR * BUF / 4), dsc2, PixBox{0, 1 << 30, 0, 1 << 30}, pb2);
    if (SPLIT) __syncthreads();
  }
  if (a.idx_out) conv_epilogue<T, MT, NT, true, EPI_GENERIC>(acc, a, b, y0 + wm * MT, x0, wn * 32, red, lds + wv * (SPR * BUF / 4), dsc2, PixBox{0, 1 << 30, 0, 1 << 30}, pb2);
  else conv_epilogue<T, MT, NT, true, EPI_ACT, false, SPR * BUF / 4>(acc, a, b, y0 + wm * MT, x0, wn * 32, red, lds + wv * (SPR * BUF / 4), dsc2, PixBox{0, 1 << 30, 0, 1 << 30}, pb2);
#if HLA_CONV_STAMPS
#undef a
  { struct { unsigned long long* stamps; } a = {a0.stamps}; HLA_STAMP(5); }
#endif
}

template <typename T>
__device__ __forceinline__ void pack_weights_body(const float* __restrict__ w, T* __restrict__ out, int Cout, int Cin, int first,
                                                  size_t e0, size_t stride, const float* __restrict__ b0 = nullptr,
                                                  int shape = SHAPE_32x32x16) {
  constexpr int EPL = 16 / sizeof(T), KC = SB / sizeof(T), NFRAG = 32 / (2 * EPL);
  const size_t total = first == 1 ? (size_t)(Cout / 32) * NFRAG * 64 * EPL : (size_t)Cout * Cin * 9;
  for (size_t e = e0; e < total; e += stride) {
    size_t r = e;
    const int j = r % EPL; r /= EPL;
    const int lane = r % 64; r /= 64;
    float v = 0.f;
    if (first == 1) {
      const int f = r % NFRAG; r /= NFRAG;
      const int nt = (int)r;
      const int k = f * 2 * EPL + (lane >> 5) * EPL + j, cout = nt * 32 + (lane & 31);
      if (k < 27) v = w[(size_t)cout * 27 + k];
      else if (b0 && k == 27) v = (float)(T)b0[cout];
      else if (b0 && k == 28) v = b0[cout] - (float)(T)b0[cout];
    } else {
      const int kg = r % 2; r /= 2;
      const int tap = r % 9; r /= 9;
      const int nsg = Cin / KC;
      const int sg = r % nsg; r /= nsg;
      const int nt = (int)r;
      const bool s16 = sizeof(T) == 2 && shape == SHAPE_16x16x32;
      const int cout = s16 ? nt * 32 + kg * 16 + (lane & 15) : nt * 32 + (lane & 31);
      const int cin = s16 ? sg * KC + (lane >> 4) * EPL + j : sg * KC + kg * 2 * EPL + (lane >> 5) * EPL + j;
      v = first == 2 ? w[((size_t)cin * Cout + cout) * 9 + (8 - tap)] : w[((size_t)cout * Cin + cin) * 9 + tap];
    }
    out[e] = (T)v;
  }
}
template <typename T>
__global__ void pack_weights_kernel(const float* __restrict__ w, T* __restrict__ out, int Cout, int Cin, int first) {
  pack_weights_body<T>(w, out, Cout, Cin, first, (size_t)blockIdx.x * blockDim.x + threadIdx.x, (size_t)gridDim.x * blockDim.x);
}
struct PackTable {
  const float* w[16]; size_t off[16];
  int cout[16], cin[16], first[16];
  int shape[16];
  const float* b0;
};
template <typename T>
__global__ void pack_weights_multi_kernel(PackTable tb, char* __restrict__ packed) {
  const int l = blockIdx.y;
  pack_weights_body<T>(tb.w[l], (T*)(packed + tb.off[l]), tb.cout[l], tb.cin[l], tb.first[l],
                       (size_t)blockIdx.x * blockDim.x + threadIdx.x, (size_t)gridDim.x * blockDim.x, tb.first[l] == 1 ? tb.b0 : nullptr,
                       tb.shape[l]);
}

struct SplitPackTable {
  const float* w[16]; size_t off[16];
  int cout[16], cin[16], first[16], slot[16];
};
static __device__ __forceinline__ void pack_weights_split_body(const float* __restrict__ w, f16* __restrict__ out, int Cout, int Cin, int first,
                                                               const unsigned* __restrict__ wmax_bits, float* __restrict__ scale_out) {
  const float sw = split_scale(*wmax_bits);
  if (blockIdx.x == 0 && threadIdx.x == 0) *scale_out = sw;
  const size_t total = first == 1 ? (size_t)(Cout / 32) * 2 * 2 * 64 * 8 : (size_t)Cout * Cin * 9 * 2;
  for (size_t e = (size_t)blockIdx.x * blockDim.x + threadIdx.x; e < total; e += (size_t)gridDim.x * blockDim.x) {
    size_t r = e;
    const int j = r % 8; r /= 8;
    const int lane = r % 64; r /= 64;
    const int hl = r % 2; r /= 2;
    float v = 0.f;
    if (first == 1) {
      const int f = r % 2; r /= 2;
      const int nt = (int)r;
      const int k = f * 16 + (lane >> 5) * 8 + j, cout = nt * 32 + (lane & 31);
      if (k < 27) v = w[(size_t)cout * 27 + k];
    } else {
      const int tap = r % 9; r /= 9;
      const int nsg = Cin / 16;
      const int sg = r % nsg; r /= nsg;
      const int nt = (int)r;
      const int cout = nt * 32 + (lane & 31), cin = sg * 16 + (lane >> 5) * 8 + j;
      v = first == 2 ? w[((size_t)cin * Cout + cout) * 9 + (8 - tap)] : w[((size_t)cout * Cin + cin) * 9 + tap];
    }
    v *= sw;
    const f16 h = (f16)v;
    out[e] = hl ? (f16)(v - (float)h) : h;
// ... 26 lines not shown

static __global__ void absmax_kernel(const float* __restrict__ w, size_t n, int row, unsigned* __restrict__ amax, unsigned* __restrict__ l1max) {
  float m = 0.f;
  for (size_t e = (size_t)blockIdx.x * blockDim.x + threadIdx.x; e < n; e += (size_t)gridDim.x * blockDim.x) m = fmaxf(m, fabsf(w[e]));
  m = wave_max_f32(m);
  if ((threadIdx.x & 63) == 0) atomicMax(amax, __float_as_uint(m));
  if (l1max && blockIdx.x == 0)
    for (size_t r0 = threadIdx.x; r0 * row < n; r0 += blockDim.x) {
      float s = 0.f;
      for (int k = 0; k < row; ++k) s += fabsf(w[r0 * row + k]);
      atomicMax(l1max, __float_as_uint(s));
    }
}

constexpr int CONF_TH = 8, CONF_TW = 32, CONF_HW = CONF_TW + 2, CONF_HPIX = (CONF_TH + 2) * CONF_HW;
constexpr int CONF_NT = (CONF_HPIX + 31) / 32;
template <typename T, int C>
__global__ __launch_bounds__(256) void conf_kernel(const T* __restrict__ act, const float* __restrict__ w,
                                                   float* __restrict__ out, int B, int H, int W) {
  constexpr int EPL = 16 / sizeof(T), KS = 2 * EPL, NS = C / KS;
  constexpr bool SPLITW = sizeof(T) == 2;
  __shared__ float td[CONF_NT * 32 * 9];
  const int lane = threadIdx.x & 63, wv = threadIdx.x >> 6, n = lane & 31, g = lane >> 5;
  const int tiles_x = (W + CONF_TW - 1) / CONF_TW, tiles_y = (H + CONF_TH - 1) / CONF_TH;
  int bid = blockIdx.x;
  const int x0 = (bid % tiles_x) * CONF_TW; bid /= tiles_x;
  const int y0 = (bid % tiles_y) * CONF_TH;
  const size_t b = bid / tiles_y;
  uint4 wh[NS], wl[SPLITW ? NS : 1];
#pragma unroll
  for (int s = 0; s < NS; ++s) {
    T hi[EPL], lo[EPL];
#pragma unroll
    for (int k = 0; k < EPL; ++k) {
      const float v = n < 9 ? w[(s * KS + g * EPL + k) * 9 + n] : 0.f;
      hi[k] = (T)v;
      lo[k] = (T)(v - to_f32(hi[k]));
    }
    __builtin_memcpy(&wh[s], hi, 16);
    if (SPLITW) __builtin_memcpy(&wl[s], lo, 16);
  }
  for (int t = wv; t < CONF_NT; t += 4) {
    const int hp = t * 32 + n, hy = hp / CONF_HW, hx = hp - hy * CONF_HW, y = y0 - 1 + hy, x = x0 - 1 + hx;
    const bool ok = hp < CONF_HPIX && y >= 0 && y < H && x >= 0 && x < W;
    const T* src = act + ((b * H + (ok ? y : 0)) * W + (ok ? x : 0)) * C + g * EPL;
    uint4 a[NS];
#pragma unroll
    for (int s = 0; s < NS; ++s) a[s] = ok ? *(const uint4*)(src + s * KS) : make_uint4(0, 0, 0, 0);
    f32x16 acc;
#pragma unroll
    for (int r = 0; r < 16; ++r) acc[r] = 0.f;
#pragma unroll
    for (int s = 0; s < NS; ++s) {
      mma16<T>(acc, wh[s], a[s]);
      if (SPLITW) mma16<T>(acc, wl[s], a[s]);
    }
#pragma unroll
    for (int r = 0; r < 8; ++r) {
      const int tap = (r & 3) + 8 * (r >> 2) + 4 * g;
      if (tap < 9) td[hp * 9 + tap] = acc[r];
    }
  }
  __syncthreads();
  const int py = threadIdx.x / CONF_TW, px = threadIdx.x % CONF_TW, y = y0 + py, x = x0 + px;
  if (y < H && x < W) {
    float s = 0.f;
#pragma unroll
    for (int tap = 0; tap < 9; ++tap) s += td[((py + tap / 3) * CONF_HW + px + tap % 3) * 9 + tap];
    const float sg = 1.f / (1.f + __expf(-s));
    out[(b * H + y) * W + x] = 1.f / (1.f + __expf(sg));
  }
}

static __global__ __launch_bounds__(256) void inv_norm_kernel(const double* __restrict__ sumsq, int np, double* __restrict__ inv) {
  __shared__ double sh[4];
  const int b = blockIdx.x;
  double s = 0.0;
  for (int i = threadIdx.x; i < np; i += 256) s += sumsq[(size_t)b * np + i];
  s = wave_sum_f64(s);
  if ((threadIdx.x & 63) == 0) sh[threadIdx.x >> 6] = s;
  __syncthreads();
  if (threadIdx.x == 0) inv[b] = 1.0 / fmax(sqrt((sh[0] + sh[1]) + (sh[2] + sh[3])), 1e-12);
}
struct InvNormArgs { const double* ss[4]; int np[4]; double* inv; int B; };
static __global__ __launch_bounds__(256) void inv_norm_multi_kernel(InvNormArgs a) {
  __shared__ double sh[4];
  const int b = blockIdx.x, l = blockIdx.y, np = a.np[l];
  const double* sumsq = a.ss[l];
  double s = 0.0;
  for (int i = threadIdx.x; i < np; i += 256) s += sumsq[(size_t)b * np + i];
  s = wave_sum_f64(s);
  if ((threadIdx.x & 63) == 0) sh[threadIdx.x >> 6] = s;
  __syncthreads();
  if (threadIdx.x == 0) a.inv[(size_t)l * a.B + b] = 1.0 / fmax(sqrt((sh[0] + sh[1]) + (sh[2] + sh[3])), 1e-12);
}
static __global__ __launch_bounds__(256) void scale_kernel(float* __restrict__ x, const double* __restrict__ inv, size_t per_sample,
                                                    int blocks_per_sample) {
  const int b = blockIdx.x / blocks_per_sample, k = blockIdx.x % blocks_per_sample;
  const double scale = inv[b];
  float4* p = (float4*)(x + (size_t)b * per_sample);
  const size_t n4 = per_sample / 4;
  for (size_t i = (size_t)k * 256 + threadIdx.x; i < n4; i += (size_t)blocks_per_sample * 256) {
    float4 v = p[i];
    v.x = (float)((double)v.x * scale); v.y = (float)((double)v.y * scale);
    v.z = (float)((double)v.z * scale); v.w = (float)((double)v.w * scale);
    p[i] = v;
  }
}


constexpr int CONV_SMALL_GRID = 320;
enum { CONV_CLASS_NT2 = 0,
       CONV_CLASS_NT2_POOL = 1,
       CONV_CLASS_NT1 = 2 };
constexpr int kConvClassShape[3] = {SHAPE_16x16x32, SHAPE_16x16x32, SHAPE_32x32x16};
constexpr int conv_class(int cout, bool pool) { return cout >= 128 ? (pool ? CONV_CLASS_NT2_POOL : CONV_CLASS_NT2) : CONV_CLASS_NT1; }
template <typename T, bool BWD> constexpr int conv_shape(int cls) { return (sizeof(T) == 2 && !BWD) ? kConvClassShape[cls] : SHAPE_32x32x16; }
template <typename T, bool BWD = false>
static bool launch_conv(hipStream_t st, ConvArgs a, bool pool) {
  if (a.unpool_idx && !(BWD && !pool)) {
    hla_set_error("launch_conv: an un-pooled source needs the UNPOOL kernel (backward, no pooling epilogue)");
    return false;
  }
  a.tiles_x = (a.W + 31) / 32;
  a.tiles_y = (a.H - a.row_begin + 7) / 8;
#if HLA_CONV_STAMPS
  a.stamps = nullptr;
  if (g_hla_stamp.buf && g_hla_stamp.counter++ == g_hla_stamp.want) {
    a.stamps = g_hla_stamp.buf;
    g_hla_stamp.grid_x = a.tiles_x * a.tiles_y * a.B; g_hla_stamp.grid_y = a.Cout >= 128 ? a.Cout / 128 : 1;
  }
#endif
  const bool big = a.Cout >= 128;
  const dim3 grid(a.tiles_x * a.tiles_y * a.B, big ? a.Cout / 128 : 1);
  const size_t es = sizeof(T), P = (size_t)a.B * (a.H - a.row_begin) * a.W, Po = pool ? P / 4 : P;
  const double flops = 2.0 * 9.0 * (a.C1 + a.C2) * a.Cout * (double)P + (a.wg0_part ? 2.0 * 27 * 64 * (double)P : 0.0);
  const double bytes = (double)P * ((a.up1 ? a.C1 / 4.0 : a.C1) + a.C2) * es + (double)Po * a.Cout * ((a.out_act ? es : 0) + (a.out_raw ? 4 : 0));
  hla_prof_begin_dyn(a.Cout >= 128 ? (pool ? K_CONV_NT2_POOL : K_CONV_NT2) : (pool ? K_CONV_NT1_POOL : K_CONV_NT1), flops, bytes, st,
                     a.dyn ? a.dyn + a.dyn_desc : nullptr, a.tiles_x * a.tiles_y);
  constexpr int S_NT2 = conv_shape<T, BWD>(CONV_CLASS_NT2), S_NT2P = conv_shape<T, BWD>(CONV_CLASS_NT2_POOL),
                S_NT1 = conv_shape<T, BWD>(CONV_CLASS_NT1);
  if constexpr (!BWD) {
    const int gy = big ? a.Cout / 128 : 1;
    if (!a.dyn && !a.sumsq && !a.unpool_idx && a.tiles_x * a.tiles_y * a.B * gy < CONV_SMALL_GRID) {
      a.tiles_y = (a.H - a.row_begin + 3) / 4;
      const dim3 g4(a.tiles_x * a.tiles_y * a.B, gy);
      if (big) {
        if (pool) hipLaunchKernelGGL((conv3x3_kernel<T, 2, 2, 2, 2, true, 1, false, S_NT2P>), g4, dim3(256), 0, st, a);
        else hipLaunchKernelGGL((conv3x3_kernel<T, 2, 2, 2, 2, false, 1, false, S_NT2>), g4, dim3(256), 0, st, a);
      } else {
        if (pool) hipLaunchKernelGGL((conv3x3_kernel<T, 2, 1, 2, 2, true, 2, false, S_NT1>), g4, dim3(256), 0, st, a);
        else hipLaunchKernelGGL((conv3x3_kernel<T, 2, 1, 2, 2, false, 2, false, S_NT1>), g4, dim3(256), 0, st, a);
      }
      hla_prof_end(st);
      return true;
    }
  }
  if (big) {
    if (pool) hipLaunchKernelGGL((conv3x3_kernel<T, 4, 2, 2, 2, true, 1, false, S_NT2P>), grid, dim3(256), 0, st, a);
    else if (BWD && a.unpool_idx) hipLaunchKernelGGL((conv3x3_kernel<T, 4, 2, 2, 2, false, 1, BWD, S_NT2>), grid, dim3(256), 0, st, a);
    else hipLaunchKernelGGL((conv3x3_kernel<T, 4, 2, 2, 2, false, 1, false, S_NT2>), grid, dim3(256), 0, st, a);
  } else {
    if (pool) hipLaunchKernelGGL((conv3x3_kernel<T, 4, 1, 2, 2, true, 2, false, S_NT1>), grid, dim3(256), 0, st, a);
    else if (BWD && a.unpool_idx) hipLaunchKernelGGL((conv3x3_kernel<T, 4, 1, 2, 2, false, 2, BWD, S_NT1>), grid, dim3(256), 0, st, a);
    else hipLaunchKernelGGL((conv3x3_kernel<T, 4, 1, 2, 2, false, 2, false, S_NT1>), grid, dim3(256), 0, st, a);
  }
  hla_prof_end(st);
  return true;
}
```

### highlyaccurate_amd/csrc/vgg.hip

```cpp
#include "conv_kernels.h"
#include "vgg_layers.h"
#include <type_traits>

template <typename T>
void vgg_pack_all(const hla_vgg_params* prm, char* packed, int dtype, hipStream_t st) {
  float* tail = (float*)(packed + packed_offset(kAllLayers, dtype));
  unsigned* scratch = (unsigned*)tail + 32;
  if (Prec<T>::SPLIT) (void)hipMemsetAsync(tail, 0, kPackTailBytes, st);
  if constexpr (!Prec<T>::SPLIT) {
    PackTable tb{};
    tb.b0 = prm->b[0];
    int n = 0;
    for (int l = 0; l < kAllLayers; ++l) {
      if (l >= kPackedLayers && !prm->w[l]) continue;
      tb.w[n] = prm->w[l]; tb.off[n] = packed_offset(l, dtype); tb.cout[n] = kLayers[l].cout; tb.cin[n] = kLayers[l].cin;
      tb.first[n] = l == 0 ? 1 : 0;
      tb.shape[n] = l >= 2 ? conv_shape<T, false>(conv_class(kLayers[l].cout, kLayers[l].pool != 0)) : SHAPE_32x32x16;
      ++n;
    }
    hla_prof_begin(K_PACK, 0, (double)packed_offset(kAllLayers, dtype) * (1.0 + 4.0 / sizeof(T)), st);
    hipLaunchKernelGGL((pack_weights_multi_kernel<T>), dim3(256, n), dim3(256), 0, st, tb, packed);
    hla_prof_end(st);
    return;
  }
  if constexpr (Prec<T>::SPLIT) {
    SplitPackTable tb{};
    int n = 0;
    for (int l = 0; l < kAllLayers; ++l) {
      if (l >= kPackedLayers && !prm->w[l]) continue;
      tb.w[n] = prm->w[l]; tb.off[n] = packed_offset(l, dtype); tb.cout[n] = kLayers[l].cout; tb.cin[n] = kLayers[l].cin;
      tb.first[n] = l == 0 ? 1 : 0; tb.slot[n] = l;
      ++n;
    }
    hla_prof_begin(K_PACK, 0, (double)packed_offset(kAllLayers, dtype) * 3.0, st);
    hipLaunchKernelGGL(absmax_multi_kernel, dim3(64, n), dim3(256), 0, st, tb, scratch, (unsigned*)tail + 16);
    hipLaunchKernelGGL(pack_weights_split_multi_kernel, dim3(256, n), dim3(256), 0, st, tb, packed, (const unsigned*)scratch, tail);
    hla_prof_end(st);
  }
}

template <typename T>
int vgg_forward_t(const float* x, size_t x_plane, const hla_vgg_params* prm, const char* packed, int dtype, void* const feat[4],
                         float* const conf[4], double* inv_norm, char* ws, const VggPlan& pl, int B, int H, int W,
                         int flags, int first_row8, hipStream_t st) {
  const bool level4 = pl.x2r != 0;
  const int NL = level4 ? 4 : 3;
  const bool fold = (flags & HLA_VGG_FOLD_DECODER) != 0;
  auto dH = [&](int d) { return fold ? 2 * (H / d) : H / d; };
  auto dW = [&](int d) { return fold ? (W / d) / 2 : W / d; };
  auto W_ = [&](int l) { return (const uint4*)(packed + packed_offset(l, dtype)); };
  char* w = ws;
  constexpr bool SPLIT = Prec<T>::SPLIT;
  const float* wtail = (const float*)(packed + packed_offset(kAllLayers, dtype));
  unsigned* amax = (unsigned*)(w + pl.amax);
  auto AM = [&](int slot) { return (SPLIT && slot >= 0) ? amax + (size_t)slot * B : (unsigned*)nullptr; };
  if (SPLIT) HLA_CHECK_HIP(hipMemsetAsync(amax, 0, (size_t)kAmaxSlots * B * sizeof(unsigned), st));
  auto conv02 = [&]() -> int {
    Conv02Args a{};
    a.x_plane = x_plane ? x_plane : (size_t)H * W;
    a.x = x; a.w0 = W_(0); a.b0 = prm->b[0]; a.w2 = W_(1); a.b2 = prm->b[1];
    a.out_act = w + pl.x3;
    if (flags & HLA_VGG_SAVE_FOR_BACKWARD) {
      a.a0_out = w + pl.a0;
      a.idx_out = (unsigned char*)(w + pl.idx3);
    }
    if (level4) a.a2_out = w + pl.x2r;
    a.wtail = wtail; a.amax_out = AM(AM_X3); a.amax_a2_out = level4 ? AM(AM_X2) : nullptr;
    a.amax_a0_out = (flags & HLA_VGG_SAVE_FOR_BACKWARD) ? AM(AM_A0) : nullptr;
    const int f0 = (level4 || (flags & HLA_VGG_SAVE_FOR_BACKWARD)) ? 0 : first_row8;
    a.row_begin = f0 ? 8 * f0 - 32 : 0;
    a.B = B; a.H = H; a.W = W; a.tiles_x = (W + 31) / 32; a.tiles_y = (H - a.row_begin + 7) / 8;
    const double P = (double)B * (H - a.row_begin) * W;
    constexpr int lds_bytes = conv02_lds_bytes<T>();
    static HlaPerDeviceOnce attr_once;
    HLA_CHECK_HIP(attr_once.run([] {
      return hipFuncSetAttribute((const void*)conv02_kernel<T, 2>, hipFuncAttributeMaxDynamicSharedMemorySize, lds_bytes);
    }));
#if HLA_CONV_STAMPS
    a.stamps = nullptr;
    if (g_hla_stamp.buf && g_hla_stamp.want <= -10 && g_hla_stamp.want++ == -10) {
      a.stamps = g_hla_stamp.buf; g_hla_stamp.want = -1000;
      g_hla_stamp.grid_x = a.tiles_x * a.tiles_y * B; g_hla_stamp.grid_y = 1;
    }
#endif
    hla_prof_begin(K_CONV02, 2.0 * 9 * (3 + 64) * 64 * P, P * (3 * 4 + 16 * sizeof(T)), st);
    hipLaunchKernelGGL((conv02_kernel<T, 2>), dim3(a.tiles_x * a.tiles_y * B), dim3(256), lds_bytes, st, a);
    hla_prof_end(st);
    return HLA_OK;
  };
  const bool train = flags & HLA_VGG_SAVE_FOR_BACKWARD;
  int np_used[4] = {pl.np[0], pl.np[1], pl.np[2], pl.np[3]};
  bool launch_ok = true;
  auto conv = [&](int l, const void* s1, int C1, int H_, int W_h, void* act, int relu, bool pool, const void* s2 = nullptr,
                  int C2 = 0, int up1 = 0, void* raw = nullptr, double* ss = nullptr, unsigned char* idx = nullptr,
                  int row_begin = 0, int norm_level = -1) {
    if (pool != (kLayers[l].pool != 0)) {
      hla_set_error("vgg_forward: layer %d launched with pool = %d, the layer table says %d", l, (int)pool, kLayers[l].pool);
      launch_ok = false;
      return;
    }
    ConvArgs a{};
    a.raw16 = (raw && (flags & HLA_VGG_FEAT16)) ? 1 : 0;
    a.row_begin = row_begin < 0 ? 0 : row_begin;
    a.idx_out = train ? idx : nullptr;
    a.src1 = s1; a.src2 = s2;
    a.C1 = C1; a.C2 = C2; a.up1 = up1; a.wpk = W_(l);
    a.bias = kLayers[l].has_bias ? prm->b[l] : nullptr;
    a.out_act = act; a.out_raw = (float*)raw; a.sumsq = ss;
    a.B = B; a.H = H_; a.W = W_h; a.Cout = kLayers[l].cout;
    a.relu_act = relu;
    if (SPLIT) {
      static const signed char kAm[13][3] = {{-1, -1, -1}, {-1, -1, -1}, {AM_X3, -1, AM_A5}, {AM_A5, -1, AM_X8}, {AM_X8, -1, AM_A10},
                                             {AM_A10, -1, AM_A12}, {AM_A12, -1, AM_X15}, {AM_X15, AM_X8, AM_D1A}, {AM_D1A, -1, AM_X18},
                                             {AM_X18, AM_X3, AM_D2A}, {AM_D2A, -1, AM_X21}, {AM_X21, AM_X2, AM_D3A}, {AM_D3A, -1, AM_X24}};
      a.amax1 = AM(kAm[l][0]); a.amax2 = AM(kAm[l][1]); a.amax_out = AM(kAm[l][2]); a.wscale = wtail + l;
    }
    if (!launch_conv<T>(st, a, pool)) launch_ok = false;
    if (norm_level >= 0)
      np_used[norm_level] = ((W_h + 31) / 32) * ((H_ - a.row_begin + 7) / 8) * (a.Cout >= 128 ? a.Cout / 128 : 1);
  };
  const int f = (level4 || train) ? 0 : first_row8;
  const int wc = ((flags & HLA_VGG_WANT_CONF) && conf) ? 1 : 0;
  const int r_c5 = f ? 4 * f - 15 : 0, r_c7 = f ? 4 * f - 14 : 0, r_c10 = f ? 2 * f - 6 : 0, r_c12 = f ? 2 * f - 5 : 0,
            r_c14 = f ? 2 * f - 4 : 0, r_d11 = f ? 2 * f - 2 - wc : 0, r_d13 = f ? 2 * f - 1 - wc : 0,
            r_d21 = f ? 4 * f - 1 - wc : 0, r_d23 = f ? 4 * f - wc : 0;
  if (const int rc = conv02()) return rc;
  conv(2, w + pl.x3, 64, H / 2, W / 2, w + pl.a5, 1, false, nullptr, 0, 0, nullptr, nullptr, nullptr, r_c5);
  conv(3, w + pl.a5, 128, H / 2, W / 2, w + pl.x8, 1, true, nullptr, 0, 0, nullptr, nullptr,
       (unsigned char*)(w + pl.idx8), r_c7);
  conv(4, w + pl.x8, 128, H / 4, W / 4, w + pl.a10, 1, false, nullptr, 0, 0, nullptr, nullptr, nullptr, r_c10);
  conv(5, w + pl.a10, 256, H / 4, W / 4, w + pl.a12, 1, false, nullptr, 0, 0, nullptr, nullptr, nullptr, r_c12);
  conv(6, w + pl.a12, 256, H / 4, W / 4, w + pl.x15r, 1, true, nullptr, 0, 0, feat[0],
       (double*)(w + pl.ss[0]), (unsigned char*)(w + pl.idx15), r_c14, 0);
  conv(7, w + pl.x15r, 256, dH(4), dW(4), w + pl.d1a, 1, false, w + pl.x8, 128, 1, nullptr, nullptr, nullptr, r_d11);
  conv(8, w + pl.d1a, 128, dH(4), dW(4), w + pl.x18r, 1, false, nullptr, 0, 0, feat[1],
       (double*)(w + pl.ss[1]), nullptr, r_d13, 1);
  const bool x21r_dead = !level4 && !wc && !train && (flags & HLA_VGG_FEAT16) && sizeof(T) == 2;
  conv(9, w + pl.x18r, 128, dH(2), dW(2), w + pl.d2a, 1, false, w + pl.x3, 64, 1, nullptr, nullptr, nullptr, r_d21);
  conv(10, w + pl.d2a, 64, dH(2), dW(2), x21r_dead ? (char*)nullptr : w + pl.x21r, 1, false, nullptr, 0, 0, feat[2],
       (double*)(w + pl.ss[2]), nullptr, r_d23, 2);
  if (level4) {
    conv(11, w + pl.x21r, 64, dH(1), dW(1), w + pl.d3a, 1, false, w + pl.x2r, 64, 1);
    conv(12, w + pl.d3a, 64, dH(1), dW(1), w + pl.x24r, 1, false, nullptr, 0, 0, feat[3],
         (double*)(w + pl.ss[3]), nullptr, 0, 3);
  }
  if ((flags & HLA_VGG_WANT_CONF) && conf) {
    using CT = std::conditional_t<SPLIT, float, T>;
    const CT* acts[4] = {(const CT*)(w + pl.x15r), (const CT*)(w + pl.x18r), (const CT*)(w + pl.x21r), (const CT*)(w + pl.x24r)};
    const int Cs[4] = {256, 128, 64, 64}, hs[4] = {H / 8, dH(4), dH(2), dH(1)}, wsz[4] = {W / 8, dW(4), dW(2), dW(1)};
    for (int l = 0; l < NL; ++l) {
      if (!conf[l]) continue;
      const size_t npix = (size_t)B * hs[l] * wsz[l];
      const int grid = B * ((hs[l] + CONF_TH - 1) / CONF_TH) * ((wsz[l] + CONF_TW - 1) / CONF_TW);
      hla_prof_begin(K_CONF, 2.0 * 9 * Cs[l] * (double)npix, (double)npix * (Cs[l] * sizeof(CT) + 4), st);
      if (Cs[l] == 256) hipLaunchKernelGGL((conf_kernel<CT, 256>), dim3(grid), dim3(256), 0, st, acts[l], prm->w[13 + l], conf[l], B, hs[l], wsz[l]);
      else if (Cs[l] == 128) hipLaunchKernelGGL((conf_kernel<CT, 128>), dim3(grid), dim3(256), 0, st, acts[l], prm->w[13 + l], conf[l], B, hs[l], wsz[l]);
      else hipLaunchKernelGGL((conf_kernel<CT, 64>), dim3(grid), dim3(256), 0, st, acts[l], prm->w[13 + l], conf[l], B, hs[l], wsz[l]);
      hla_prof_end(st);
    }
  }
  {
    const size_t per[4] = {(size_t)(H / 8) * (W / 8) * 256, (size_t)(H / 4) * (W / 4) * 128, (size_t)(H / 2) * (W / 2) * 64,
                           (size_t)H * W * 64};
    double* inv = inv_norm ? inv_norm : (double*)(w + pl.inv);
    {
      InvNormArgs ia{};
      double bytes = 0;
      for (int l = 0; l < NL; ++l) { ia.ss[l] = (const double*)(w + pl.ss[l]); ia.np[l] = np_used[l]; bytes += (double)B * pl.np[l] * 8; }
      ia.inv = inv; ia.B = B;
      hla_prof_begin(K_L2NORM, 0, bytes, st);
      hipLaunchKernelGGL(inv_norm_multi_kernel, dim3(B, NL), dim3(256), 0, st, ia);
      hla_prof_end(st);
    }
    for (int l = 0; l < NL; ++l) {
      if (flags & HLA_VGG_DEFER_NORM) continue;
      int bps = (int)(per[l] / 4 / 256 / 4);
      bps = bps < 1 ? 1 : (bps > 64 ? 64 : bps);
      hla_prof_begin(K_L2NORM, 0, (double)B * per[l] * 8, st);
      hipLaunchKernelGGL(scale_kernel, dim3(B * bps), dim3(256), 0, st, (float*)feat[l], inv + (size_t)l * B, per[l], bps);
      hla_prof_end(st);
    }
  }
  HLA_CHECK_HIP(hipGetLastError());
  return launch_ok ? HLA_OK : HLA_ERR_ARG;
}

#if HLA_TU_DTYPE >= 0
template void vgg_pack_all<TuT>(const hla_vgg_params* prm, char* packed, int dtype, hipStream_t st);
template int vgg_forward_t<TuT>(const float* x, size_t x_plane, const hla_vgg_params* prm, const char* packed, int dtype, void* const feat[4],
                              float* const conf[4], double* inv_norm, char* ws, const VggPlan& pl, int B, int H, int W,
                              int flags, int first_row8, hipStream_t st);
#else
#define HLA_EXTERN_T(T) \
  extern template void vgg_pack_all<T>(const hla_vgg_params* prm, char* packed, int dtype, hipStream_t st); \
  extern template int vgg_forward_t<T>(const float* x, size_t x_plane, const hla_vgg_params* prm, const char* packed, int dtype, void* const feat[4],                               float* const conf[4], double* inv_norm, char* ws, const VggPlan& pl, int B, int H, int W,                               int flags, int first_row8, hipStream_t st);
HLA_EXTERN_T(float) HLA_EXTERN_T(bf16) HLA_EXTERN_T(f16) HLA_EXTERN_T(split32)

extern "C" size_t hla_vgg_packed_weight_bytes(int dtype) {
  return packed_offset(kAllLayers, dtype) + (dtype == HLA_F16X3 ? kPackTailBytes : 0);
}

extern "C" int hla_vgg_pack_weights(const hla_vgg_params* params, void* packed, int dtype, hla_stream_t stream) {
  HLA_REQUIRE(params && packed, "hla_vgg_pack_weights: null argument");
  HLA_REQUIRE(hla_dtype_ok(dtype), "hla_vgg_pack_weights: bad dtype %d", dtype);
  HLA_REQUIRE(params->w[0] && params->b[0], "hla_vgg_pack_weights: conv0's weight and bias are required (the bias is packed with it)");
  if (dtype == HLA_BF16) vgg_pack_all<bf16>(params, (char*)packed, dtype, (hipStream_t)stream);
  else if (dtype == HLA_F16) vgg_pack_all<f16>(params, (char*)packed, dtype, (hipStream_t)stream);
  else if (dtype == HLA_F16X3) vgg_pack_all<split32>(params, (char*)packed, dtype, (hipStream_t)stream);
  else vgg_pack_all<float>(params, (char*)packed, dtype, (hipStream_t)stream);
  HLA_CHECK_HIP(hipGetLastError());
  return HLA_OK;
}

extern "C" size_t hla_vgg_workspace_bytes(int B, int H, int W, int level, int dtype) {
  VggPlan p;
  vgg_plan(B, H, W, dtype, true, &p, level == 4);
  return p.total;
}

extern "C" size_t hla_vgg_workspace_bytes_flags(int B, int H, int W, int level, int dtype, int flags) {
  VggPlan p;
  vgg_plan(B, H, W, dtype, true, &p, level == 4, (flags & HLA_VGG_FOLD_DECODER) != 0);
  return p.total;
}

extern "C" int hla_vgg_forward(const float* x, size_t x_plane, const hla_vgg_params* params, const void* packed_weights,
                               void* const feat[4], float* const conf[4], double* inv_norm, void* workspace,
                               size_t workspace_bytes, int B, int H, int W, int level, int dtype, int flags,
                               int first_row8, hla_stream_t stream) {
  HLA_REQUIRE(x && params && packed_weights && feat && workspace, "hla_vgg_forward: null argument");
  HLA_REQUIRE(hla_dtype_ok(dtype), "hla_vgg_forward: dtype must be HLA_F32, HLA_BF16, HLA_F16 or HLA_F16X3 (got %d)", dtype);
  HLA_REQUIRE(B > 0 && H >= 8 && W >= 8 && H % 8 == 0 && W % 8 == 0, "hla_vgg_forward: H and W must be multiples of 8");
  HLA_REQUIRE(x_plane == 0 || x_plane >= (size_t)H * W, "hla_vgg_forward: x_plane (%zu) must be 0 or >= H*W", x_plane);
  HLA_REQUIRE((size_t)H * W * 64 * 4 < ((size_t)1 << 31), "hla_vgg_forward: image too large (H*W must be below 2^23 pixels)");
  HLA_REQUIRE(level == 3 || level == 4, "hla_vgg_forward: level must be 3 (x15,x18,x21) or 4 (+x24), got %d", level);
  HLA_REQUIRE(feat[0] && feat[1] && feat[2], "hla_vgg_forward: feat[0..2] are required");
  HLA_REQUIRE(level == 3 || (feat[3] && params->w[11] && params->w[12]),
              "hla_vgg_forward: level 4 needs feat[3] ([B,H,W,64], 16 real channels) and the zero-padded conv_dec3 weights in w[11], w[12]");
  HLA_REQUIRE(level == 3 || !(flags & HLA_VGG_WANT_CONF) || !conf || !conf[3] || params->w[16], "hla_vgg_forward: conf[3] needs w[16]");
  HLA_REQUIRE(!(flags & HLA_VGG_DEFER_NORM) || inv_norm, "hla_vgg_forward: HLA_VGG_DEFER_NORM needs inv_norm");
  HLA_REQUIRE(!(flags & HLA_VGG_FEAT16) || ((dtype == HLA_BF16 || dtype == HLA_F16) && (flags & HLA_VGG_DEFER_NORM) &&
                                            !(flags & HLA_VGG_SAVE_FOR_BACKWARD) && level == 3),
              "hla_vgg_forward: HLA_VGG_FEAT16 needs dtype HLA_BF16 / HLA_F16, HLA_VGG_DEFER_NORM, level 3 and no HLA_VGG_SAVE_FOR_BACKWARD");
  HLA_REQUIRE(first_row8 == 0 || (first_row8 >= 4 && first_row8 < H / 8), "hla_vgg_forward: first_row8 must be 0 or in [4, H/8)");
  HLA_REQUIRE(!(flags & HLA_VGG_FOLD_DECODER) || (W % 16 == 0 && first_row8 == 0 && !(flags & HLA_VGG_FEAT16)),
              "hla_vgg_forward: HLA_VGG_FOLD_DECODER needs W %% 16 == 0 (folded maps are W/16, W/8, W/4 wide), first_row8 == 0 and no "
              "HLA_VGG_FEAT16 (got W = %d, first_row8 = %d)", W, first_row8);
  VggPlan pl;
  vgg_plan(B, H, W, dtype, (flags & HLA_VGG_SAVE_FOR_BACKWARD) != 0, &pl, level == 4, (flags & HLA_VGG_FOLD_DECODER) != 0);
  if (workspace_bytes < pl.total) {
    hla_set_error("hla_vgg_forward: workspace %zu < %zu", workspace_bytes, pl.total);
    return HLA_ERR_WORKSPACE;
  }
  if (dtype == HLA_BF16)
    return vgg_forward_t<bf16>(x, x_plane, params, (const char*)packed_weights, dtype, feat, conf, inv_norm, (char*)workspace, pl,
                               B, H, W, flags, first_row8, (hipStream_t)stream);
  if (dtype == HLA_F16)
    return vgg_forward_t<f16>(x, x_plane, params, (const char*)packed_weights, dtype, feat, conf, inv_norm, (char*)workspace, pl,
                              B, H, W, flags, first_row8, (hipStream_t)stream);
  if (dtype == HLA_F16X3)
    return vgg_forward_t<split32>(x, x_plane, params, (const char*)packed_weights, dtype, feat, conf, inv_norm, (char*)workspace, pl,
                                  B, H, W, flags, first_row8, (hipStream_t)stream);
  return vgg_forward_t<float>(x, x_plane, params, (const char*)packed_weights, dtype, feat, conf, inv_norm, (char*)workspace, pl,
                              B, H, W, flags, first_row8, (hipStream_t)stream);
}
#endif
```

### include/hla.h

```cpp
#ifndef HLA_H
#define HLA_H

#include <stddef.h>
#include <stdint.h>

#ifdef __cplusplus
extern "C" {
#endif

typedef void* hla_stream_t;

typedef enum hla_status {
  HLA_OK = 0,
  HLA_ERR_ARG = -1,
  HLA_ERR_HIP = -2,
  HLA_ERR_WORKSPACE = -3
} hla_status;

typedef enum hla_dtype {
  HLA_F32 = 0,
  HLA_BF16 = 1,
  HLA_F16 = 2,
  HLA_F16X3 = 3
} hla_dtype;

const char* hla_last_error(void);

#define HLA_ABI_VERSION 24
int hla_abi_version(void);
const char* hla_source_hash(void);
typedef enum hla_struct_id {
  HLA_STRUCT_VGG_PARAMS = 0, HLA_STRUCT_VGG_GRADS = 1, HLA_STRUCT_S2G_LEVEL = 2, HLA_STRUCT_S2G_CONFIG = 3,
  HLA_STRUCT_S2G_LEVEL_GRAD = 4, HLA_STRUCT_PROF_RECORD = 5, HLA_STRUCT_POSE_LOSS_ARGS = 6, HLA_STRUCT_FILL_REGION = 7
} hla_struct_id;
size_t hla_sizeof_struct(int id);


typedef struct hla_vgg_params {
  const float* w[17];
  const float* b[7];
} hla_vgg_params;

enum {
  HLA_VGG_WANT_CONF = 1,
  HLA_VGG_DEFER_NORM = 2,
  HLA_VGG_SAVE_FOR_BACKWARD = 4,
  HLA_VGG_FOLD_DECODER = 16,
  HLA_VGG_FEAT16 = 8
};

size_t hla_vgg_packed_weight_bytes(int dtype);
int hla_vgg_pack_weights(const hla_vgg_params* params, void* packed, int dtype, hla_stream_t stream);

size_t hla_vgg_workspace_bytes(int B, int H, int W, int level, int dtype);
size_t hla_vgg_workspace_bytes_flags(int B, int H, int W, int level, int dtype, int flags);

int hla_vgg_forward(const float* x, size_t x_plane, const hla_vgg_params* params, const void* packed_weights, void* const feat[4],
                    float* const conf[4], double* inv_norm, void* workspace, size_t workspace_bytes, int B, int H,
                    int W, int level, int dtype, int flags, int first_row8, hla_stream_t stream);

typedef struct hla_vgg_grads {
  float* dw[17];
  float* db[7];
} hla_vgg_grads;

size_t hla_vgg_packed_weight_T_bytes(int dtype);
int hla_vgg_pack_weights_T(const hla_vgg_params* params, void* packed_T, int dtype, hla_stream_t stream);
size_t hla_vgg_bwd_workspace_bytes(int B, int H, int W, int level, int dtype);
size_t hla_vgg_bwd_workspace_bytes_flags(int B, int H, int W, int level, int dtype, int flags);

#define HLA_VGG_BWD_SCALE_INVARIANT 1
#define HLA_VGG_BWD_DENSE 2
#define HLA_VGG_BWD_WGRAD_TWO_PHASE 4
#define HLA_VGG_BWD_FOLD_DECODER 16
#define HLA_VGG_BWD_WGRAD0_UNFUSED 8
int hla_vgg_backward(const float* x, size_t x_plane, const hla_vgg_params* params, const void* packed_weights_T,
                     const void* fwd_workspace, const float* const feat[4], const double* inv_norm,
                     const float* const d_feat[4], const float* const conf[4], const float* const d_conf[4],
                     const hla_vgg_grads* grads, void* workspace, size_t workspace_bytes, int B, int H, int W, int level,
                     int dtype, int flags, int first_row8, hla_stream_t stream);

int hla_vgg_backward_live_tiles(const void* workspace, int B, int H, int W, int level, int dtype, long long* live,
                                long long* total);

int hla_sat_tile(const unsigned char* src, const double* stages, float* out, int B, int S, int crop, hla_stream_t stream);

int hla_resize_bilinear(const unsigned char* src, const int* hbounds, const int* htaps, int hksize, const int* vbounds,
                        const int* vtaps, int vksize, unsigned char* mid, float* out, int B, int H, int W, int out_h,
                        int out_w, hla_stream_t stream);

int hla_grid_sample(const float* image, const float* optical, const float* jac, float* out, float* jac_out,
                    int N, int C, int IH, int IW, int H, int W, int M, hla_stream_t stream);

int hla_grid_sample_bwd(const float* image, const float* optical, const float* jac, const float* d_out,
                        const float* d_jac_out, float* d_image, float* d_optical, float* d_jac,
                        int N, int C, int IH, int IW, int H, int W, int M, hla_stream_t stream);

typedef struct hla_s2g_level {
  const void* sat_feat;
  const void* grd_feat;
  const float* grd_conf;
  const float* xyz;
  const double* sat_inv_norm;
  const double* grd_inv_norm;
  int A, h, w, C;
  int row0;
  int grd_row_skip;
  double meter_per_pixel;
  double centre;
  int feat_dtype;
} hla_s2g_level;

typedef struct hla_s2g_config {
  int ford;
  int n_levels, n_iters;
  int level_first;
  int using_weight;
  int use_hessian;
  int dof;
  double shift_range_lat, shift_range_lon, rotation_range;
  double damping[3];
  const unsigned char* keep;
  size_t keep_stride;
  int optimizer;
  double beta1, beta2;
  int count_in_view;
  int grd_grad_overwrite;
  int deterministic;
  int proj;
} hla_s2g_config;

size_t hla_s2g_workspace_bytes(const hla_s2g_config* cfg, const hla_s2g_level* levels, int B);

int hla_s2g_lm_solve(const hla_s2g_config* cfg, const hla_s2g_level* levels, const float* R_FL,
                     const float* T_FL, const float* pose0, const float* rand_uv, float* trace,
                     double* normal_eq, void* workspace, size_t workspace_bytes, int B, hla_stream_t stream);

size_t hla_g2s_workspace_bytes(const hla_s2g_config* cfg, const hla_s2g_level* levels, int B);
int hla_g2s_lm_solve(const hla_s2g_config* cfg, const hla_s2g_level* levels, const float* camera_k, int ori_h, int ori_w,
                     const float* pose0, float* trace, double* normal_eq, void* workspace, size_t workspace_bytes,
                     int B, hla_stream_t stream);

// ... 73 lines not shown
```

Before: 5342 pairs/s.

## Launch satellite and ground VGG extractors as paired single-grid conv kernels

Adds a paired forward path that runs the satellite and ground VGG branches together, with each conv layer issued as one kernel whose grid covers both branches. Blocks pick their branch's argument block from the kernarg segment. This halves extractor launch count and lets the smaller ground branch fill CUs left idle by the satellite branch, replacing the serial per-branch launches for large batches. It falls back to separate launches when the layer plans differ, and adds a larger kernarg segment plus per-block argument loads.

```diff
diff --git a/highlyaccurate_amd/VGG.py b/highlyaccurate_amd/VGG.py
--- a/highlyaccurate_amd/VGG.py
+++ b/highlyaccurate_amd/VGG.py
@@ -127,6 +127,47 @@
     if save_for_backward:
         return feats, confs, inv_norm, dict(x=x, x_version=x._version, x_plane=x_plane, ws=ws, feats=feats, inv_norm=inv_norm, dt=dt, L=L)
     return feats, confs, inv_norm
+
+
+@_lib.on_device(lambda modules, xs, *a, **k: xs[0])
+def vgg_forward_pair_nhwc(modules, xs, first_row8=(0, 0), feat16: bool = False):
+    lib = _lib.load()
+    if len(modules) != 2 or len(xs) != 2:
+        raise ValueError('vgg_forward_pair_nhwc takes two modules and two images')
+    dt = _dtype_code(modules[0].precision)
+    if _dtype_code(modules[1].precision) != dt or any(m.level == 4 or getattr(m, 'folded', False) for m in modules):
+        raise ValueError('vgg_forward_pair_nhwc: two unfolded extractors of one precision, level 3')
+    if feat16 and dt not in (_lib.HLA_BF16, _lib.HLA_F16):
+        raise ValueError("feat16 needs precision 'bf16' / 'fp16'")
+    if xs[0].dim() != 4 or xs[1].dim() != 4 or xs[0].shape[1] != 3 or xs[1].shape[1] != 3 or xs[0].shape[0] != xs[1].shape[0]:
+        raise ValueError(f'expected two [B,3,H,W] images with one B, got {tuple(xs[0].shape)} and {tuple(xs[1].shape)}')
+    br = (_lib.VggBranch * 2)()
+    keep, out = [], []
+    for k, (module, x) in enumerate(zip(modules, xs)):
+        _lib.require_gpu(x, 'VGGUnet input')
+        x, x_plane = _image_window(x)
+        B, _, H, W = x.shape
+        _lib.same_device(('input', x), ('parameters', module.conv0.weight), ('first input', xs[0]))
+        prm, kp, versions = _param_table(module)
+        packed = _packed_weights(module, prm, versions, dt, x.device)
+        feats = [torch.empty(B, H >> (3 - l), W >> (3 - l), _CH[l], device=x.device, dtype=torch.float16 if feat16 else torch.float32)
+                 for l in range(3)]
+        inv_norm = torch.empty(3, B, device=x.device, dtype=torch.float64)
+        nbytes = lib.hla_vgg_workspace_bytes(B, H, W, 3, dt)
+        ws = torch.empty(nbytes, dtype=torch.uint8, device=x.device)
+        b = br[k]
+        b.x, b.x_plane, b.params, b.packed_weights = x.data_ptr(), x_plane, C.pointer(prm), packed.data_ptr()
+        for l in range(3):
+            b.feat[l] = feats[l].data_ptr()
+        b.inv_norm, b.workspace, b.workspace_bytes = inv_norm.data_ptr(), ws.data_ptr(), nbytes
+        b.H, b.W, b.first_row8 = H, W, int(first_row8[k])
+        keep += [x, prm, kp, packed, ws]
+        out.append((feats, inv_norm))
+    flags = _lib.HLA_VGG_DEFER_NORM | (_lib.HLA_VGG_FEAT16 if feat16 else 0)
+    paired = C.c_int(0)
+    rc = lib.hla_vgg_forward_pair(br, xs[0].shape[0], 3, dt, flags, C.byref(paired), _lib.stream_ptr())
+    _lib.check(rc, 'hla_vgg_forward_pair')
+    return out[0], out[1], bool(paired.value)
 
 
 @_lib.on_device(lambda module, ctx, *a, **k: ctx['x'])
diff --git a/highlyaccurate_amd/_lib.py b/highlyaccurate_amd/_lib.py
--- a/highlyaccurate_amd/_lib.py
+++ b/highlyaccurate_amd/_lib.py
@@ -16,7 +16,7 @@
 HLA_VGG_BWD_WGRAD_TWO_PHASE = 4
 HLA_VGG_BWD_WGRAD0_UNFUSED = 8
 HLA_VGG_BWD_FOLD_DECODER = 16
-ABI_VERSION = 24
+ABI_VERSION = 25
 
 
 class HlaError(RuntimeError):
@@ -41,6 +41,12 @@
                 ('damping', C.c_double * 3), ('keep', C.c_void_p), ('keep_stride', C.c_size_t),
                 ('optimizer', C.c_int), ('beta1', C.c_double), ('beta2', C.c_double), ('count_in_view', C.c_int),
                 ('grd_grad_overwrite', C.c_int), ('deterministic', C.c_int), ('proj', C.c_int)]
+
+
+class VggBranch(C.Structure):
+    _fields_ = [('x', C.c_void_p), ('x_plane', C.c_size_t), ('params', C.POINTER(VggParams)), ('packed_weights', C.c_void_p),
+                ('feat', C.c_void_p * 4), ('conf', C.c_void_p * 4), ('inv_norm', C.c_void_p), ('workspace', C.c_void_p),
+                ('workspace_bytes', C.c_size_t), ('H', C.c_int), ('W', C.c_int), ('first_row8', C.c_int)]
 
 
 class FillRegion(C.Structure):
@@ -81,7 +87,8 @@
     except AttributeError:
         raise HlaError(f'{path}: no hla_sizeof_struct export; rebuild it') from None
     fn.restype, fn.argtypes = C.c_size_t, [C.c_int]
-    for sid, cls in enumerate((VggParams, VggGrads, S2GLevel, S2GConfig, S2GLevelGrad, ProfRecord, PoseLossArgs, FillRegion)):
+    for sid, cls in enumerate((VggParams, VggGrads, S2GLevel, S2GConfig, S2GLevelGrad, ProfRecord, PoseLossArgs, FillRegion,
+                                VggBranch)):
         if fn(sid) != C.sizeof(cls):
             raise HlaError(f'{path}: sizeof({cls.__name__}) is {fn(sid)} in the library and {C.sizeof(cls)} in the binding')
 
@@ -116,6 +123,8 @@
     lib.hla_vgg_forward.restype = i
     lib.hla_vgg_forward.argtypes = [vp, sz, C.POINTER(VggParams), vp, C.POINTER(vp), C.POINTER(vp), vp, vp, sz,
                                     i, i, i, i, i, i, i, vp]
+    lib.hla_vgg_forward_pair.restype = i
+    lib.hla_vgg_forward_pair.argtypes = [C.POINTER(VggBranch), i, i, i, i, C.POINTER(i), vp]
     lib.hla_vgg_packed_weight_bytes.restype = sz
     lib.hla_vgg_packed_weight_bytes.argtypes = [i]
     lib.hla_vgg_pack_weights.restype = i
diff --git a/highlyaccurate_amd/_s2gp.py b/highlyaccurate_amd/_s2gp.py
--- a/highlyaccurate_amd/_s2gp.py
+++ b/highlyaccurate_amd/_s2gp.py
@@ -7,7 +7,7 @@
 import torch.nn as nn
 
 from . import _lib, utils
-from .VGG import VGGUnet, vgg_forward_nhwc, vgg_backward_nhwc
+from .VGG import VGGUnet, vgg_forward_nhwc, vgg_forward_pair_nhwc, vgg_backward_nhwc
 
 KITTI_K = [[582.9802, 0.0, 496.2420], [0.0, 482.7076, 125.0034], [0.0, 0.0, 1.0]]
 FORD_K_FL = [945.391406, 0.0, 855.502825, 0.0, 945.668274, 566.372868, 0.0, 0.0, 1.0]
@@ -395,6 +395,18 @@
     def _features(self, sat_map, grd_img, want_conf, return_confs):
         f16 = (self.SatFeatureNet.precision in ('bf16', 'fp16') and self.level == 3 and bool(getattr(self.args, 'lm_feat16', 1)))
         small = sat_map.shape[0] <= int(getattr(self.args, 'small_batch_two_streams', 4))
+        dead_ok = (not return_confs and self.level == 3 and getattr(self.args, 'Optimizer', 'LM') == 'LM'
+                   and bool(getattr(self.args, 'ground_crop', 1)) and not self.polar)
+        skip = dead_ground_rows(grd_img.shape[-2]) if dead_ok else 0
+        grd_in = grd_img[:, :, skip:, :] if skip else grd_img
+        f8 = ((grd_img.shape[-2] // 8) // 2 - skip // 8) if dead_ok else 0
+        f8 = f8 if f8 >= 4 else 0
+        if (not small and not want_conf and self.level != 4 and bool(getattr(self.args, 'pair_extractor_launches', 1))
+                and self.GrdFeatureNet.precision == self.SatFeatureNet.precision):
+            (sat_feats, sat_inv), (grd_feats, grd_inv), _ = vgg_forward_pair_nhwc(
+                (self.SatFeatureNet, self.GrdFeatureNet), (sat_map, grd_in), first_row8=(0, f8), feat16=f16)
+            L = self._levels
+            return L(sat_feats), L(sat_inv), L(grd_feats), L([None] * 3), L(grd_inv)
         if small:
             cur = torch.cuda.current_stream()
             side = _side_stream(sat_map.device)
@@ -404,14 +416,6 @@
             sat_map.record_stream(side)
         else:
             sat_feats, _, sat_inv = vgg_forward_nhwc(self.SatFeatureNet, sat_map, want_conf=False, defer_norm=True, feat16=f16)
-        grd_in = grd_img
-        dead_ok = (not return_confs and self.level == 3 and getattr(self.args, 'Optimizer', 'LM') == 'LM'
-                   and bool(getattr(self.args, 'ground_crop', 1)) and not self.polar)
-        skip = dead_ground_rows(grd_img.shape[-2]) if dead_ok else 0
-        if skip:
-            grd_in = grd_img[:, :, skip:, :]
-        f8 = ((grd_img.shape[-2] // 8) // 2 - skip // 8) if dead_ok else 0
-        f8 = f8 if f8 >= 4 else 0
         grd_feats, grd_confs, grd_inv = vgg_forward_nhwc(self.GrdFeatureNet, grd_in, want_conf=want_conf, defer_norm=True,
                                                          first_row8=f8, feat16=f16)
         if small:
diff --git a/highlyaccurate_amd/csrc/capi.hip b/highlyaccurate_amd/csrc/capi.hip
--- a/highlyaccurate_amd/csrc/capi.hip
+++ b/highlyaccurate_amd/csrc/capi.hip
@@ -29,6 +29,7 @@
     case HLA_STRUCT_PROF_RECORD: return sizeof(hla_prof_record);
     case HLA_STRUCT_POSE_LOSS_ARGS: return sizeof(hla_pose_loss_args);
     case HLA_STRUCT_FILL_REGION: return sizeof(hla_fill_region);
+    case HLA_STRUCT_VGG_BRANCH: return sizeof(hla_vgg_branch);
     default: return 0;
   }
 }
diff --git a/highlyaccurate_amd/csrc/conv_kernels.h b/highlyaccurate_amd/csrc/conv_kernels.h
--- a/highlyaccurate_amd/csrc/conv_kernels.h
+++ b/highlyaccurate_amd/csrc/conv_kernels.h
@@ -340,7 +340,8 @@
 __device__ __forceinline__ void conv_epilogue(typename AccMap<SHAPE>::Tile (&acc)[MT][NT], const ConvArgs& a, int b, int yrow0, int x0,
                                               int cb, float* red, char* stage, float dsc = 1.f,
                                               PixBox addb = PixBox{0, 1 << 30, 0, 1 << 30},
-                                              const float4* prebias = nullptr) {
+                                              const float4* prebias = nullptr,
+                                              int blk = 0, int nblk = 1) {
   using RawT = std::conditional_t<R16, f16, float>;
   constexpr bool GEN = EPI == EPI_GENERIC, RAW = EPI == EPI_ACT_RAW || EPI == EPI_ACT_RAW_NOBIAS, DG = EPI == EPI_DGRAD;
   constexpr bool NOBIAS = EPI == EPI_ACT_RAW_NOBIAS || DG || sizeof(T) == 2;
@@ -555,7 +556,7 @@
     if (tid == 0) {
       if (has_sumsq) {
         const int np = a.tiles_x * a.tiles_y * gridDim.y;
-        const int tile = (xcd_contiguous(blockIdx.x, gridDim.x) % (a.tiles_x * a.tiles_y)) * gridDim.y + blockIdx.y;
+        const int tile = (xcd_contiguous(blk, nblk) % (a.tiles_x * a.tiles_y)) * gridDim.y + blockIdx.y;
         a.sumsq[(size_t)b * np + tile] = ((double)red[0] + (double)red[1]) + ((double)red[2] + (double)red[3]);
       }
       if (want_max) {
@@ -823,7 +824,7 @@
 }
 
 template <typename T, int MT, int NT, int WM, int WN, bool POOL, int WD, bool UNPOOL = false, int SHAPE = SHAPE_32x32x16>
-__global__ __launch_bounds__(256, NT == 1 ? 3 : 2) void conv3x3_kernel(ConvArgs a) {
+__device__ __forceinline__ void conv3x3_body(const ConvArgs& a, const int blk, const int nblk) {
   static_assert(WM * WN == 4, "4 waves per block");
   static_assert(SHAPE == SHAPE_32x32x16 || (sizeof(T) == 2 && !UNPOOL), "16x16x32: bf16 / f16 forward kernels only");
   using M = AccMap<SHAPE>;
@@ -847,8 +848,8 @@
   if (a.dyn) {
     const ConvDyn& d = *(const ConvDyn*)(a.dyn + a.dyn_desc);
     const int nl = d.n_live, nlive = nl * a.B;
-    if ((int)blockIdx.x >= nlive) return;
-    int bid = xcd_contiguous(blockIdx.x, nlive);
+    if (blk >= nlive) return;
+    int bid = xcd_contiguous(blk, nlive);
     b = bid / nl;
     const int e = a.dyn[d.list + bid % nl];
     ty = e >> 16; tx = e & 0xffff;
@@ -860,7 +861,7 @@
       sb.lo2 = a.dyn[d.src_bands + 2 * b2] << sh; sb.hi2 = min(a.dyn[d.src_bands + 2 * b2 + 1] << sh, a.W);
     }
   } else {
-    int bid = xcd_contiguous(blockIdx.x, gridDim.x);
+    int bid = xcd_contiguous(blk, nblk);
     tx = bid % a.tiles_x; bid /= a.tiles_x;
     ty = bid % a.tiles_y;
     b = bid / a.tiles_y;
@@ -1090,19 +1091,59 @@
         return;
       }
     }
-    if (mode == EPI_ACT) conv_epilogue<T, MT, NT, POOL, EPI_ACT, false, LDSB / 4, SHAPE>(acc, a, b, y0 + wm * MT, x0, ntg0 * 32, red, stager, dsc, addb);
+    if (mode == EPI_ACT) conv_epilogue<T, MT, NT, POOL, EPI_ACT, false, LDSB / 4, SHAPE>(acc, a, b, y0 + wm * MT, x0, ntg0 * 32, red, stager, dsc, addb, nullptr, blk, nblk);
     else if (T16 && RAW_SPECIAL && a.raw16 && mode == EPI_ACT_RAW)
-      conv_epilogue<T, MT, NT, POOL, (T16 && RAW_SPECIAL) ? EPI_ACT_RAW : EPI_GENERIC, T16 && RAW_SPECIAL, 0, SHAPE>(acc, a, b, y0 + wm * MT, x0, ntg0 * 32, red, stager, dsc, addb);
+      conv_epilogue<T, MT, NT, POOL, (T16 && RAW_SPECIAL) ? EPI_ACT_RAW : EPI_GENERIC, T16 && RAW_SPECIAL, 0, SHAPE>(acc, a, b, y0 + wm * MT, x0, ntg0 * 32, red, stager, dsc, addb, nullptr, blk, nblk);
     else if (T16 && a.raw16 && mode == EPI_ACT_RAW_NOBIAS)
-      conv_epilogue<T, MT, NT, POOL, T16 ? EPI_ACT_RAW_NOBIAS : EPI_GENERIC, T16, 0, SHAPE>(acc, a, b, y0 + wm * MT, x0, ntg0 * 32, red, stager, dsc, addb);
-    else if (RAW_SPECIAL && mode == EPI_ACT_RAW) conv_epilogue<T, MT, NT, POOL, RAW_SPECIAL ? EPI_ACT_RAW : EPI_GENERIC, false, 0, SHAPE>(acc, a, b, y0 + wm * MT, x0, ntg0 * 32, red, stager, dsc, addb);
+      conv_epilogue<T, MT, NT, POOL, T16 ? EPI_ACT_RAW_NOBIAS : EPI_GENERIC, T16, 0, SHAPE>(acc, a, b, y0 + wm * MT, x0, ntg0 * 32, red, stager, dsc, addb, nullptr, blk, nblk);
+    else if (RAW_SPECIAL && mode == EPI_ACT_RAW) conv_epilogue<T, MT, NT, POOL, RAW_SPECIAL ? EPI_ACT_RAW : EPI_GENERIC, false, 0, SHAPE>(acc, a, b, y0 + wm * MT, x0, ntg0 * 32, red, stager, dsc, addb, nullptr, blk, nblk);
     else if (SHAPE == SHAPE_32x32x16 && mode == EPI_DGRAD)
-      conv_epilogue<T, MT, NT, POOL, SHAPE == SHAPE_32x32x16 ? EPI_DGRAD : EPI_GENERIC, false, 0, SHAPE>(acc, a, b, y0 + wm * MT, x0, ntg0 * 32, red, stager, dsc, addb);
+      conv_epilogue<T, MT, NT, POOL, SHAPE == SHAPE_32x32x16 ? EPI_DGRAD : EPI_GENERIC, false, 0, SHAPE>(acc, a, b, y0 + wm * MT, x0, ntg0 * 32, red, stager, dsc, addb, nullptr, blk, nblk);
     else if ((RAW_SPECIAL || sizeof(T) == 2) && mode == EPI_ACT_RAW_NOBIAS)
-      conv_epilogue<T, MT, NT, POOL, (RAW_SPECIAL || sizeof(T) == 2) ? EPI_ACT_RAW_NOBIAS : EPI_GENERIC, false, 0, SHAPE>(acc, a, b, y0 + wm * MT, x0, ntg0 * 32, red, stager, dsc, addb);
-    else conv_epilogue<T, MT, NT, POOL, EPI_GENERIC, false, 0, SHAPE>(acc, a, b, y0 + wm * MT, x0, ntg0 * 32, red, stager, dsc, addb);
+      conv_epilogue<T, MT, NT, POOL, (RAW_SPECIAL || sizeof(T) == 2) ? EPI_ACT_RAW_NOBIAS : EPI_GENERIC, false, 0, SHAPE>(acc, a, b, y0 + wm * MT, x0, ntg0 * 32, red, stager, dsc, addb, nullptr, blk, nblk);
+    else conv_epilogue<T, MT, NT, POOL, EPI_GENERIC, false, 0, SHAPE>(acc, a, b, y0 + wm * MT, x0, ntg0 * 32, red, stager, dsc, addb, nullptr, blk, nblk);
   }
   HLA_STAMP(5);
+}
+template <typename T, int MT, int NT, int WM, int WN, bool POOL, int WD, bool UNPOOL = false, int SHAPE = SHAPE_32x32x16>
+__global__ __launch_bounds__(256, NT == 1 ? 3 : 2) void conv3x3_kernel(ConvArgs a) {
+  conv3x3_body<T, MT, NT, WM, WN, POOL, WD, UNPOOL, SHAPE>(a, (int)blockIdx.x, (int)gridDim.x);
+}
+
+template <typename A> struct PairArgs { A s[2]; int n0; };
+template <typename A>
+__device__ __forceinline__ A pair_segment_args(bool second) {
+  static_assert(sizeof(A) % 4 == 0 && offsetof(PairArgs<A>, s) == 0, "the argument blocks lead the kernarg segment");
+  typedef const __attribute__((address_space(4))) unsigned* kptr_t;
+  const kptr_t kp = (kptr_t)__builtin_amdgcn_kernarg_segment_ptr() + (second ? sizeof(A) / 4 : 0);
+  unsigned w[sizeof(A) / 4];
+#pragma unroll
+  for (unsigned i = 0; i < sizeof(A) / 4; ++i) w[i] = kp[i];
+  A a;
+  __builtin_memcpy(&a, w, sizeof(A));
+  return a;
+}
+template <typename P> __device__ __forceinline__ P* pair_global(P* p) {
+  return (P*)(__attribute__((address_space(1))) P*)(unsigned long long)p;
+}
+__device__ __forceinline__ void pair_inference_args(ConvArgs& a) {
+  a.src1 = pair_global(a.src1); a.src2 = pair_global(a.src2); a.wpk = pair_global(a.wpk); a.bias = pair_global(a.bias);
+  a.out_act = pair_global(a.out_act); a.out_raw = pair_global(a.out_raw); a.sumsq = pair_global(a.sumsq);
+  a.amax1 = pair_global(a.amax1); a.amax2 = pair_global(a.amax2); a.amax_out = pair_global(a.amax_out); a.wscale = pair_global(a.wscale);
+  a.dyn = nullptr; a.dyn_desc = 0; a.src_row_lo = 0; a.add_row_lo = 0; a.unpool_idx = nullptr; a.mask_act = nullptr; a.add_src = nullptr;
+  a.idx_out = nullptr; a.pool_sum = 0; a.wg0_x = nullptr; a.wg0_x_plane = 0; a.wg0_part = nullptr;
+#if HLA_CONV_STAMPS
+  a.stamps = nullptr;
+#endif
+}
+template <typename T, int MT, int NT, int WM, int WN, bool POOL, int WD, int SHAPE>
+__global__ __launch_bounds__(256, NT == 1 ? 3 : 2) void conv3x3_pair_kernel(PairArgs<ConvArgs> p) {
+  const int n0 = p.n0;
+  const bool second = (int)blockIdx.x >= n0;
+  ConvArgs a = pair_segment_args<ConvArgs>(second);
+  pair_inference_args(a);
+  conv3x3_body<T, MT, NT, WM, WN, POOL, WD, false, SHAPE>(a, second ? (int)blockIdx.x - n0 : (int)blockIdx.x,
+                                                          second ? (int)gridDim.x - n0 : n0);
 }
 
 struct Conv02Args {
@@ -1133,7 +1174,7 @@
 }
 
 template <typename T, int WD>
-__global__ __launch_bounds__(256, Prec<T>::SPLIT ? 2 : 3) void conv02_kernel(Conv02Args a0) {
+__device__ __forceinline__ void conv02_body(const Conv02Args& a0, const int blk) {
   constexpr bool SPLIT = Prec<T>::SPLIT;
   constexpr bool FOLD = sizeof(T) == 2 && !SPLIT;
   constexpr int EPL = Prec<T>::CEPL, KC = SB / sizeof(T), NSG = 64 / KC, NFRAG = 32 / (2 * EPL), NH = SPLIT ? 2 : 1;
@@ -1152,7 +1193,7 @@
   HLA_STAMP_HWID();
 
   const int t = threadIdx.x, lane = t & 63, wv = __builtin_amdgcn_readfirstlane(t >> 6), wm = wv / WN, wn = wv % WN;
-  int bid = blockIdx.x;
+  int bid = blk;
   const int tx = bid % a0.tiles_x; bid /= a0.tiles_x;
   const int ty = bid % a0.tiles_y;
   const int b = bid / a0.tiles_y;
@@ -1403,6 +1444,23 @@
 #undef a
   { struct { unsigned long long* stamps; } a = {a0.stamps}; HLA_STAMP(5); }
 #endif
+}
+template <typename T, int WD>
+__global__ __launch_bounds__(256, Prec<T>::SPLIT ? 2 : 3) void conv02_kernel(Conv02Args a0) {
+  conv02_body<T, WD>(a0, (int)blockIdx.x);
+}
+template <typename T, int WD>
+__global__ __launch_bounds__(256, Prec<T>::SPLIT ? 2 : 3) void conv02_pair_kernel(PairArgs<Conv02Args> p) {
+  const int n0 = p.n0;
+  const bool second = (int)blockIdx.x >= n0;
+  Conv02Args a0 = pair_segment_args<Conv02Args>(second);
+  a0.x = pair_global(a0.x); a0.w0 = pair_global(a0.w0); a0.b0 = pair_global(a0.b0); a0.w2 = pair_global(a0.w2); a0.b2 = pair_global(a0.b2);
+  a0.out_act = pair_global(a0.out_act); a0.wtail = pair_global(a0.wtail); a0.amax_out = pair_global(a0.amax_out);
+  a0.a0_out = nullptr; a0.idx_out = nullptr; a0.a2_out = nullptr; a0.amax_a2_out = nullptr; a0.amax_a0_out = nullptr;
+#if HLA_CONV_STAMPS
+  a0.stamps = nullptr;
+#endif
+  conv02_body<T, WD>(a0, second ? (int)blockIdx.x - n0 : (int)blockIdx.x);
 }
 
 template <typename T>
@@ -1595,7 +1653,7 @@
   __syncthreads();
   if (threadIdx.x == 0) inv[b] = 1.0 / fmax(sqrt((sh[0] + sh[1]) + (sh[2] + sh[3])), 1e-12);
 }
-struct InvNormArgs { const double* ss[4]; int np[4]; double* inv; int B; };
+struct InvNormArgs { const double* ss[8]; int np[8]; double* inv[8]; };
 static __global__ __launch_bounds__(256) void inv_norm_multi_kernel(InvNormArgs a) {
   __shared__ double sh[4];
   const int b = blockIdx.x, l = blockIdx.y, np = a.np[l];
@@ -1605,7 +1663,7 @@
   s = wave_sum_f64(s);
   if ((threadIdx.x & 63) == 0) sh[threadIdx.x >> 6] = s;
   __syncthreads();
-  if (threadIdx.x == 0) a.inv[(size_t)l * a.B + b] = 1.0 / fmax(sqrt((sh[0] + sh[1]) + (sh[2] + sh[3])), 1e-12);
+  if (threadIdx.x == 0) a.inv[l][b] = 1.0 / fmax(sqrt((sh[0] + sh[1]) + (sh[2] + sh[3])), 1e-12);
 }
 static __global__ __launch_bounds__(256) void scale_kernel(float* __restrict__ x, const double* __restrict__ inv, size_t per_sample,
                                                     int blocks_per_sample) {
@@ -1629,55 +1687,91 @@
 constexpr int kConvClassShape[3] = {SHAPE_16x16x32, SHAPE_16x16x32, SHAPE_32x32x16};
 constexpr int conv_class(int cout, bool pool) { return cout >= 128 ? (pool ? CONV_CLASS_NT2_POOL : CONV_CLASS_NT2) : CONV_CLASS_NT1; }
 template <typename T, bool BWD> constexpr int conv_shape(int cls) { return (sizeof(T) == 2 && !BWD) ? kConvClassShape[cls] : SHAPE_32x32x16; }
-template <typename T, bool BWD = false>
-static bool launch_conv(hipStream_t st, ConvArgs a, bool pool) {
+struct ConvPlan { bool small; int gx, gy, kid; double flops, bytes; };
+template <typename T, bool BWD>
+static ConvPlan conv_plan(ConvArgs& a, bool pool) {
+  a.tiles_x = (a.W + 31) / 32;
+  a.tiles_y = (a.H - a.row_begin + 7) / 8;
+  const bool big = a.Cout >= 128;
+  ConvPlan p{};
+  p.gy = big ? a.Cout / 128 : 1;
+  const size_t es = sizeof(T), P = (size_t)a.B * (a.H - a.row_begin) * a.W, Po = pool ? P / 4 : P;
+  p.flops = 2.0 * 9.0 * (a.C1 + a.C2) * a.Cout * (double)P + (a.wg0_part ? 2.0 * 27 * 64 * (double)P : 0.0);
+  p.bytes = (double)P * ((a.up1 ? a.C1 / 4.0 : a.C1) + a.C2) * es + (double)Po * a.Cout * ((a.out_act ? es : 0) + (a.out_raw ? 4 : 0));
+  p.kid = big ? (pool ? K_CONV_NT2_POOL : K_CONV_NT2) : (pool ? K_CONV_NT1_POOL : K_CONV_NT1);
+  p.small = !BWD && !a.dyn && !a.sumsq && !a.unpool_idx && a.tiles_x * a.tiles_y * a.B * p.gy < CONV_SMALL_GRID;
+  if (p.small) a.tiles_y = (a.H - a.row_begin + 3) / 4;
+  p.gx = a.tiles_x * a.tiles_y * a.B;
+  return p;
+}
+template <typename T, int MT, int NT, bool POOL, int WD, bool UNPOOL, int SHAPE, bool PAIR>
+static void conv_dispatch(hipStream_t st, const ConvArgs& a, const ConvPlan& p, const ConvArgs& a2, const ConvPlan& p2) {
+  if constexpr (PAIR) {
+    static_assert(!UNPOOL, "two-segment launches: forward inference forms only");
+    PairArgs<ConvArgs> pa{{a, a2}, p.gx};
+    hipLaunchKernelGGL((conv3x3_pair_kernel<T, MT, NT, 2, 2, POOL, WD, SHAPE>), dim3(p.gx + p2.gx, p.gy), dim3(256), 0, st, pa);
+  } else {
+    hipLaunchKernelGGL((conv3x3_kernel<T, MT, NT, 2, 2, POOL, WD, UNPOOL, SHAPE>), dim3(p.gx, p.gy), dim3(256), 0, st, a);
+  }
+}
+template <typename T, bool BWD, bool PAIR>
+static bool launch_conv_impl(hipStream_t st, ConvArgs a, ConvArgs a2, bool pool) {
   if (a.unpool_idx && !(BWD && !pool)) {
     hla_set_error("launch_conv: an un-pooled source needs the UNPOOL kernel (backward, no pooling epilogue)");
     return false;
   }
-  a.tiles_x = (a.W + 31) / 32;
-  a.tiles_y = (a.H - a.row_begin + 7) / 8;
+  const ConvPlan p = conv_plan<T, BWD>(a, pool);
+  ConvPlan p2{};
+  if constexpr (PAIR) {
+    p2 = conv_plan<T, BWD>(a2, pool);
+    auto infer = [](const ConvArgs& c) {
+      return !c.dyn && !c.src_row_lo && !c.add_row_lo && !c.unpool_idx && !c.mask_act && !c.add_src && !c.idx_out && !c.pool_sum && !c.wg0_part;
+    };
+    if (BWD || !infer(a) || !infer(a2) || p2.small != p.small || p2.gy != p.gy || a2.Cout != a.Cout) {
+      hla_set_error("launch_conv: the two segments of a paired launch do not take the same kernel");
+      return false;
+    }
+  }
 #if HLA_CONV_STAMPS
-  a.stamps = nullptr;
-  if (g_hla_stamp.buf && g_hla_stamp.counter++ == g_hla_stamp.want) {
+  a.stamps = a2.stamps = nullptr;
+  if (!PAIR && g_hla_stamp.buf && g_hla_stamp.counter++ == g_hla_stamp.want) {
     a.stamps = g_hla_stamp.buf;
-    g_hla_stamp.grid_x = a.tiles_x * a.tiles_y * a.B; g_hla_stamp.grid_y = a.Cout >= 128 ? a.Cout / 128 : 1;
+    g_hla_stamp.grid_x = a.tiles_x * ((a.H - a.row_begin + 7) / 8) * a.B; g_hla_stamp.grid_y = p.gy;
   }
 #endif
   const bool big = a.Cout >= 128;
-  const dim3 grid(a.tiles_x * a.tiles_y * a.B, big ? a.Cout / 128 : 1);
-  const size_t es = sizeof(T), P = (size_t)a.B * (a.H - a.row_begin) * a.W, Po = pool ? P / 4 : P;
-  const double flops = 2.0 * 9.0 * (a.C1 + a.C2) * a.Cout * (double)P + (a.wg0_part ? 2.0 * 27 * 64 * (double)P : 0.0);
-  const double bytes = (double)P * ((a.up1 ? a.C1 / 4.0 : a.C1) + a.C2) * es + (double)Po * a.Cout * ((a.out_act ? es : 0) + (a.out_raw ? 4 : 0));
-  hla_prof_begin_dyn(a.Cout >= 128 ? (pool ? K_CONV_NT2_POOL : K_CONV_NT2) : (pool ? K_CONV_NT1_POOL : K_CONV_NT1), flops, bytes, st,
-                     a.dyn ? a.dyn + a.dyn_desc : nullptr, a.tiles_x * a.tiles_y);
+  hla_prof_begin_dyn(p.kid, p.flops + p2.flops, p.bytes + p2.bytes, st, a.dyn ? a.dyn + a.dyn_desc : nullptr, a.tiles_x * a.tiles_y);
   constexpr int S_NT2 = conv_shape<T, BWD>(CONV_CLASS_NT2), S_NT2P = conv_shape<T, BWD>(CONV_CLASS_NT2_POOL),
                 S_NT1 = conv_shape<T, BWD>(CONV_CLASS_NT1);
-  if constexpr (!BWD) {
-    const int gy = big ? a.Cout / 128 : 1;
-    if (!a.dyn && !a.sumsq && !a.unpool_idx && a.tiles_x * a.tiles_y * a.B * gy < CONV_SMALL_GRID) {
-      a.tiles_y = (a.H - a.row_begin + 3) / 4;
-      const dim3 g4(a.tiles_x * a.tiles_y * a.B, gy);
+  constexpr bool UNP = BWD && !PAIR;
+  if (p.small) {
+    if constexpr (!BWD) {
       if (big) {
-        if (pool) hipLaunchKernelGGL((conv3x3_kernel<T, 2, 2, 2, 2, true, 1, false, S_NT2P>), g4, dim3(256), 0, st, a);
-        else hipLaunchKernelGGL((conv3x3_kernel<T, 2, 2, 2, 2, false, 1, false, S_NT2>), g4, dim3(256), 0, st, a);
+        if (pool) conv_dispatch<T, 2, 2, true, 1, false, S_NT2P, PAIR>(st, a, p, a2, p2);
+        else conv_dispatch<T, 2, 2, false, 1, false, S_NT2, PAIR>(st, a, p, a2, p2);
       } else {
-        if (pool) hipLaunchKernelGGL((conv3x3_kernel<T, 2, 1, 2, 2, true, 2, false, S_NT1>), g4, dim3(256), 0, st, a);
-        else hipLaunchKernelGGL((conv3x3_kernel<T, 2, 1, 2, 2, false, 2, false, S_NT1>), g4, dim3(256), 0, st, a);
-      }
-      hla_prof_end(st);
-      return true;
-    }
+        if (pool) conv_dispatch<T, 2, 1, true, 2, false, S_NT1, PAIR>(st, a, p, a2, p2);
+        else conv_dispatch<T, 2, 1, false, 2, false, S_NT1, PAIR>(st, a, p, a2, p2);
+      }
+    }
+    hla_prof_end(st);
+    return true;
   }
   if (big) {
-    if (pool) hipLaunchKernelGGL((conv3x3_kernel<T, 4, 2, 2, 2, true, 1, false, S_NT2P>), grid, dim3(256), 0, st, a);
-    else if (BWD && a.unpool_idx) hipLaunchKernelGGL((conv3x3_kernel<T, 4, 2, 2, 2, false, 1, BWD, S_NT2>), grid, dim3(256), 0, st, a);
-    else hipLaunchKernelGGL((conv3x3_kernel<T, 4, 2, 2, 2, false, 1, false, S_NT2>), grid, dim3(256), 0, st, a);
+    if (pool) conv_dispatch<T, 4, 2, true, 1, false, S_NT2P, PAIR>(st, a, p, a2, p2);
+    else if (UNP && a.unpool_idx) conv_dispatch<T, 4, 2, false, 1, UNP, S_NT2, PAIR>(st, a, p, a2, p2);
+    else conv_dispatch<T, 4, 2, false, 1, false, S_NT2, PAIR>(st, a, p, a2, p2);
   } else {
-    if (pool) hipLaunchKernelGGL((conv3x3_kernel<T, 4, 1, 2, 2, true, 2, false, S_NT1>), grid, dim3(256), 0, st, a);
-    else if (BWD && a.unpool_idx) hipLaunchKernelGGL((conv3x3_kernel<T, 4, 1, 2, 2, false, 2, BWD, S_NT1>), grid, dim3(256), 0, st, a);
-    else hipLaunchKernelGGL((conv3x3_kernel<T, 4, 1, 2, 2, false, 2, false, S_NT1>), grid, dim3(256), 0, st, a);
+    if (pool) conv_dispatch<T, 4, 1, true, 2, false, S_NT1, PAIR>(st, a, p, a2, p2);
+    else if (UNP && a.unpool_idx) conv_dispatch<T, 4, 1, false, 2, UNP, S_NT1, PAIR>(st, a, p, a2, p2);
+    else conv_dispatch<T, 4, 1, false, 2, false, S_NT1, PAIR>(st, a, p, a2, p2);
   }
   hla_prof_end(st);
   return true;
 }
+template <typename T, bool BWD = false>
+static bool launch_conv(hipStream_t st, const ConvArgs& a, bool pool) { return launch_conv_impl<T, BWD, false>(st, a, ConvArgs{}, pool); }
+template <typename T>
+static bool launch_conv_pair(hipStream_t st, const ConvArgs& a, const ConvArgs& a2, bool pool) {
+  return launch_conv_impl<T, false, true>(st, a, a2, pool);
+}
diff --git a/highlyaccurate_amd/csrc/vgg.hip b/highlyaccurate_amd/csrc/vgg.hip
--- a/highlyaccurate_amd/csrc/vgg.hip
+++ b/highlyaccurate_amd/csrc/vgg.hip
@@ -39,12 +39,17 @@
   }
 }
 
-template <typename T>
-int vgg_forward_t(const float* x, size_t x_plane, const hla_vgg_params* prm, const char* packed, int dtype, void* const feat[4],
-                         float* const conf[4], double* inv_norm, char* ws, const VggPlan& pl, int B, int H, int W,
-                         int flags, int first_row8, hipStream_t st) {
+struct VggConvSet {
+  Conv02Args c02;
+  ConvArgs conv[kAllLayers];
+  bool used[kAllLayers], pool[kAllLayers];
+  int np_used[4];
+  bool ok;
+};
+template <typename T>
+static void vgg_build_convs(const float* x, size_t x_plane, const hla_vgg_params* prm, const char* packed, int dtype, void* const feat[4],
+                            bool want_conf, char* ws, const VggPlan& pl, int B, int H, int W, int flags, int first_row8, VggConvSet& S) {
   const bool level4 = pl.x2r != 0;
-  const int NL = level4 ? 4 : 3;
   const bool fold = (flags & HLA_VGG_FOLD_DECODER) != 0;
   auto dH = [&](int d) { return fold ? 2 * (H / d) : H / d; };
   auto dW = [&](int d) { return fold ? (W / d) / 2 : W / d; };
@@ -54,52 +59,36 @@
   const float* wtail = (const float*)(packed + packed_offset(kAllLayers, dtype));
   unsigned* amax = (unsigned*)(w + pl.amax);
   auto AM = [&](int slot) { return (SPLIT && slot >= 0) ? amax + (size_t)slot * B : (unsigned*)nullptr; };
-  if (SPLIT) HLA_CHECK_HIP(hipMemsetAsync(amax, 0, (size_t)kAmaxSlots * B * sizeof(unsigned), st));
-  auto conv02 = [&]() -> int {
-    Conv02Args a{};
+  const bool train = flags & HLA_VGG_SAVE_FOR_BACKWARD;
+  S = VggConvSet{};
+  S.ok = true;
+  for (int l = 0; l < 4; ++l) S.np_used[l] = pl.np[l];
+  {
+    Conv02Args& a = S.c02;
     a.x_plane = x_plane ? x_plane : (size_t)H * W;
     a.x = x; a.w0 = W_(0); a.b0 = prm->b[0]; a.w2 = W_(1); a.b2 = prm->b[1];
     a.out_act = w + pl.x3;
-    if (flags & HLA_VGG_SAVE_FOR_BACKWARD) {
+    if (train) {
       a.a0_out = w + pl.a0;
       a.idx_out = (unsigned char*)(w + pl.idx3);
     }
     if (level4) a.a2_out = w + pl.x2r;
     a.wtail = wtail; a.amax_out = AM(AM_X3); a.amax_a2_out = level4 ? AM(AM_X2) : nullptr;
-    a.amax_a0_out = (flags & HLA_VGG_SAVE_FOR_BACKWARD) ? AM(AM_A0) : nullptr;
-    const int f0 = (level4 || (flags & HLA_VGG_SAVE_FOR_BACKWARD)) ? 0 : first_row8;
+    a.amax_a0_out = train ? AM(AM_A0) : nullptr;
+    const int f0 = (level4 || train) ? 0 : first_row8;
     a.row_begin = f0 ? 8 * f0 - 32 : 0;
     a.B = B; a.H = H; a.W = W; a.tiles_x = (W + 31) / 32; a.tiles_y = (H - a.row_begin + 7) / 8;
-    const double P = (double)B * (H - a.row_begin) * W;
-    constexpr int lds_bytes = conv02_lds_bytes<T>();
-    static HlaPerDeviceOnce attr_once;
-    HLA_CHECK_HIP(attr_once.run([] {
-      return hipFuncSetAttribute((const void*)conv02_kernel<T, 2>, hipFuncAttributeMaxDynamicSharedMemorySize, lds_bytes);
-    }));
-#if HLA_CONV_STAMPS
-    a.stamps = nullptr;
-    if (g_hla_stamp.buf && g_hla_stamp.want <= -10 && g_hla_stamp.want++ == -10) {
-      a.stamps = g_hla_stamp.buf; g_hla_stamp.want = -1000;
-      g_hla_stamp.grid_x = a.tiles_x * a.tiles_y * B; g_hla_stamp.grid_y = 1;
-    }
-#endif
-    hla_prof_begin(K_CONV02, 2.0 * 9 * (3 + 64) * 64 * P, P * (3 * 4 + 16 * sizeof(T)), st);
-    hipLaunchKernelGGL((conv02_kernel<T, 2>), dim3(a.tiles_x * a.tiles_y * B), dim3(256), lds_bytes, st, a);
-    hla_prof_end(st);
-    return HLA_OK;
-  };
-  const bool train = flags & HLA_VGG_SAVE_FOR_BACKWARD;
-  int np_used[4] = {pl.np[0], pl.np[1], pl.np[2], pl.np[3]};
-  bool launch_ok = true;
+  }
   auto conv = [&](int l, const void* s1, int C1, int H_, int W_h, void* act, int relu, bool pool, const void* s2 = nullptr,
                   int C2 = 0, int up1 = 0, void* raw = nullptr, double* ss = nullptr, unsigned char* idx = nullptr,
                   int row_begin = 0, int norm_level = -1) {
     if (pool != (kLayers[l].pool != 0)) {
       hla_set_error("vgg_forward: layer %d launched with pool = %d, the layer table says %d", l, (int)pool, kLayers[l].pool);
-      launch_ok = false;
+      S.ok = false;
       return;
     }
-    ConvArgs a{};
+    ConvArgs& a = S.conv[l];
+    S.used[l] = true; S.pool[l] = pool;
     a.raw16 = (raw && (flags & HLA_VGG_FEAT16)) ? 1 : 0;
     a.row_begin = row_begin < 0 ? 0 : row_begin;
     a.idx_out = train ? idx : nullptr;
@@ -115,16 +104,14 @@
                                              {AM_X18, AM_X3, AM_D2A}, {AM_D2A, -1, AM_X21}, {AM_X21, AM_X2, AM_D3A}, {AM_D3A, -1, AM_X24}};
       a.amax1 = AM(kAm[l][0]); a.amax2 = AM(kAm[l][1]); a.amax_out = AM(kAm[l][2]); a.wscale = wtail + l;
     }
-    if (!launch_conv<T>(st, a, pool)) launch_ok = false;
     if (norm_level >= 0)
-      np_used[norm_level] = ((W_h + 31) / 32) * ((H_ - a.row_begin + 7) / 8) * (a.Cout >= 128 ? a.Cout / 128 : 1);
+      S.np_used[norm_level] = ((W_h + 31) / 32) * ((H_ - a.row_begin + 7) / 8) * (a.Cout >= 128 ? a.Cout / 128 : 1);
   };
   const int f = (level4 || train) ? 0 : first_row8;
-  const int wc = ((flags & HLA_VGG_WANT_CONF) && conf) ? 1 : 0;
+  const int wc = want_conf ? 1 : 0;
   const int r_c5 = f ? 4 * f - 15 : 0, r_c7 = f ? 4 * f - 14 : 0, r_c10 = f ? 2 * f - 6 : 0, r_c12 = f ? 2 * f - 5 : 0,
             r_c14 = f ? 2 * f - 4 : 0, r_d11 = f ? 2 * f - 2 - wc : 0, r_d13 = f ? 2 * f - 1 - wc : 0,
             r_d21 = f ? 4 * f - 1 - wc : 0, r_d23 = f ? 4 * f - wc : 0;
-  if (const int rc = conv02()) return rc;
   conv(2, w + pl.x3, 64, H / 2, W / 2, w + pl.a5, 1, false, nullptr, 0, 0, nullptr, nullptr, nullptr, r_c5);
   conv(3, w + pl.a5, 128, H / 2, W / 2, w + pl.x8, 1, true, nullptr, 0, 0, nullptr, nullptr,
        (unsigned char*)(w + pl.idx8), r_c7);
@@ -144,7 +131,94 @@
     conv(12, w + pl.d3a, 64, dH(1), dW(1), w + pl.x24r, 1, false, nullptr, 0, 0, feat[3],
          (double*)(w + pl.ss[3]), nullptr, 0, 3);
   }
-  if ((flags & HLA_VGG_WANT_CONF) && conf) {
+}
+
+template <typename T>
+static int launch_conv02(hipStream_t st, Conv02Args a, const Conv02Args* a1) {
+  constexpr int lds_bytes = conv02_lds_bytes<T>();
+#if HLA_CONV_STAMPS
+  a.stamps = nullptr;
+  if (!a1 && g_hla_stamp.buf && g_hla_stamp.want <= -10 && g_hla_stamp.want++ == -10) {
+    a.stamps = g_hla_stamp.buf; g_hla_stamp.want = -1000;
+    g_hla_stamp.grid_x = a.tiles_x * a.tiles_y * a.B; g_hla_stamp.grid_y = 1;
+  }
+#endif
+  auto P = [](const Conv02Args& c) { return (double)c.B * (c.H - c.row_begin) * c.W; };
+  const double Pt = P(a) + (a1 ? P(*a1) : 0.0);
+  if (a1) {
+    static HlaPerDeviceOnce attr_once;
+    HLA_CHECK_HIP(attr_once.run([] {
+      return hipFuncSetAttribute((const void*)conv02_pair_kernel<T, 2>, hipFuncAttributeMaxDynamicSharedMemorySize, lds_bytes);
+    }));
+    PairArgs<Conv02Args> pa{{a, *a1}, a.tiles_x * a.tiles_y * a.B};
+#if HLA_CONV_STAMPS
+    pa.s[1].stamps = nullptr;
+#endif
+    hla_prof_begin(K_CONV02, 2.0 * 9 * (3 + 64) * 64 * Pt, Pt * (3 * 4 + 16 * sizeof(T)), st);
+    hipLaunchKernelGGL((conv02_pair_kernel<T, 2>), dim3(pa.n0 + a1->tiles_x * a1->tiles_y * a1->B), dim3(256), lds_bytes, st, pa);
+    hla_prof_end(st);
+    return HLA_OK;
+  }
+  static HlaPerDeviceOnce attr_once;
+  HLA_CHECK_HIP(attr_once.run([] {
+    return hipFuncSetAttribute((const void*)conv02_kernel<T, 2>, hipFuncAttributeMaxDynamicSharedMemorySize, lds_bytes);
+  }));
+  hla_prof_begin(K_CONV02, 2.0 * 9 * (3 + 64) * 64 * Pt, Pt * (3 * 4 + 16 * sizeof(T)), st);
+  hipLaunchKernelGGL((conv02_kernel<T, 2>), dim3(a.tiles_x * a.tiles_y * a.B), dim3(256), lds_bytes, st, a);
+  hla_prof_end(st);
+  return HLA_OK;
+}
+
+struct VggNormNet { const VggConvSet* S; char* ws; const VggPlan* pl; double* inv_norm; void* const* feat; int H, W; };
+static int vgg_norms(hipStream_t st, int nb, const VggNormNet* net, int B, int NL, int flags) {
+  InvNormArgs ia{};
+  double bytes = 0;
+  for (int k = 0; k < nb; ++k)
+    for (int l = 0; l < NL; ++l) {
+      const VggNormNet& n = net[k];
+      ia.ss[k * NL + l] = (const double*)(n.ws + n.pl->ss[l]); ia.np[k * NL + l] = n.S->np_used[l];
+      ia.inv[k * NL + l] = (n.inv_norm ? n.inv_norm : (double*)(n.ws + n.pl->inv)) + (size_t)l * B;
+      bytes += (double)B * n.pl->np[l] * 8;
+    }
+  hla_prof_begin(K_L2NORM, 0, bytes, st);
+  hipLaunchKernelGGL(inv_norm_multi_kernel, dim3(B, nb * NL), dim3(256), 0, st, ia);
+  hla_prof_end(st);
+  for (int k = 0; k < nb; ++k) {
+    const int H = net[k].H, W = net[k].W;
+    const size_t per[4] = {(size_t)(H / 8) * (W / 8) * 256, (size_t)(H / 4) * (W / 4) * 128, (size_t)(H / 2) * (W / 2) * 64, (size_t)H * W * 64};
+    for (int l = 0; l < NL; ++l) {
+      if (flags & HLA_VGG_DEFER_NORM) continue;
+      int bps = (int)(per[l] / 4 / 256 / 4);
+      bps = bps < 1 ? 1 : (bps > 64 ? 64 : bps);
+      hla_prof_begin(K_L2NORM, 0, (double)B * per[l] * 8, st);
+      hipLaunchKernelGGL(scale_kernel, dim3(B * bps), dim3(256), 0, st, (float*)net[k].feat[l], ia.inv[k * NL + l], per[l], bps);
+      hla_prof_end(st);
+    }
+  }
+  return HLA_OK;
+}
+
+template <typename T>
+int vgg_forward_t(const float* x, size_t x_plane, const hla_vgg_params* prm, const char* packed, int dtype, void* const feat[4],
+                         float* const conf[4], double* inv_norm, char* ws, const VggPlan& pl, int B, int H, int W,
+                         int flags, int first_row8, hipStream_t st) {
+  const bool level4 = pl.x2r != 0;
+  const int NL = level4 ? 4 : 3;
+  const bool fold = (flags & HLA_VGG_FOLD_DECODER) != 0;
+  auto dH = [&](int d) { return fold ? 2 * (H / d) : H / d; };
+  auto dW = [&](int d) { return fold ? (W / d) / 2 : W / d; };
+  char* w = ws;
+  constexpr bool SPLIT = Prec<T>::SPLIT;
+  if (SPLIT) HLA_CHECK_HIP(hipMemsetAsync(w + pl.amax, 0, (size_t)kAmaxSlots * B * sizeof(unsigned), st));
+  const bool want_conf = (flags & HLA_VGG_WANT_CONF) && conf;
+  VggConvSet S;
+  vgg_build_convs<T>(x, x_plane, prm, packed, dtype, feat, want_conf, ws, pl, B, H, W, flags, first_row8, S);
+  if (!S.ok) return HLA_ERR_ARG;
+  if (const int rc = launch_conv02<T>(st, S.c02, nullptr)) return rc;
+  bool launch_ok = true;
+  for (int l = 2; l < kAllLayers; ++l)
+    if (S.used[l] && !launch_conv<T>(st, S.conv[l], S.pool[l])) launch_ok = false;
+  if (want_conf) {
     using CT = std::conditional_t<SPLIT, float, T>;
     const CT* acts[4] = {(const CT*)(w + pl.x15r), (const CT*)(w + pl.x18r), (const CT*)(w + pl.x21r), (const CT*)(w + pl.x24r)};
     const int Cs[4] = {256, 128, 64, 64}, hs[4] = {H / 8, dH(4), dH(2), dH(1)}, wsz[4] = {W / 8, dW(4), dW(2), dW(1)};
@@ -160,26 +234,40 @@
     }
   }
   {
-    const size_t per[4] = {(size_t)(H / 8) * (W / 8) * 256, (size_t)(H / 4) * (W / 4) * 128, (size_t)(H / 2) * (W / 2) * 64,
-                           (size_t)H * W * 64};
-    double* inv = inv_norm ? inv_norm : (double*)(w + pl.inv);
-    {
-      InvNormArgs ia{};
-      double bytes = 0;
-      for (int l = 0; l < NL; ++l) { ia.ss[l] = (const double*)(w + pl.ss[l]); ia.np[l] = np_used[l]; bytes += (double)B * pl.np[l] * 8; }
-      ia.inv = inv; ia.B = B;
-      hla_prof_begin(K_L2NORM, 0, bytes, st);
-      hipLaunchKernelGGL(inv_norm_multi_kernel, dim3(B, NL), dim3(256), 0, st, ia);
-      hla_prof_end(st);
-    }
-    for (int l = 0; l < NL; ++l) {
-      if (flags & HLA_VGG_DEFER_NORM) continue;
-      int bps = (int)(per[l] / 4 / 256 / 4);
-      bps = bps < 1 ? 1 : (bps > 64 ? 64 : bps);
-      hla_prof_begin(K_L2NORM, 0, (double)B * per[l] * 8, st);
-      hipLaunchKernelGGL(scale_kernel, dim3(B * bps), dim3(256), 0, st, (float*)feat[l], inv + (size_t)l * B, per[l], bps);
-      hla_prof_end(st);
-    }
+    const VggNormNet net{&S, ws, &pl, inv_norm, feat, H, W};
+    if (const int rc = vgg_norms(st, 1, &net, B, NL, flags)) return rc;
+  }
+  HLA_CHECK_HIP(hipGetLastError());
+  return launch_ok ? HLA_OK : HLA_ERR_ARG;
+}
+
+constexpr int HLA_PAIR_FALLBACK = -1000;
+template <typename T>
+int vgg_forward_pair_t(const hla_vgg_branch br[2], const VggPlan pl[2], int B, int dtype, int flags, hipStream_t st) {
+  constexpr bool SPLIT = Prec<T>::SPLIT;
+  VggConvSet S[2];
+  for (int k = 0; k < 2; ++k) {
+    vgg_build_convs<T>(br[k].x, br[k].x_plane, br[k].params, (const char*)br[k].packed_weights, dtype, br[k].feat, false,
+                       (char*)br[k].workspace, pl[k], B, br[k].H, br[k].W, flags, br[k].first_row8, S[k]);
+    if (!S[k].ok) return HLA_ERR_ARG;
+  }
+  for (int l = 2; l < kAllLayers; ++l) {
+    if (S[0].used[l] != S[1].used[l]) return HLA_PAIR_FALLBACK;
+    if (!S[0].used[l]) continue;
+    ConvArgs a0 = S[0].conv[l], a1 = S[1].conv[l];
+    if (conv_plan<T, false>(a0, S[0].pool[l]).small != conv_plan<T, false>(a1, S[1].pool[l]).small) return HLA_PAIR_FALLBACK;
+  }
+  if (SPLIT)
+    for (int k = 0; k < 2; ++k)
+      HLA_CHECK_HIP(hipMemsetAsync((char*)br[k].workspace + pl[k].amax, 0, (size_t)kAmaxSlots * B * sizeof(unsigned), st));
+  if (const int rc = launch_conv02<T>(st, S[0].c02, &S[1].c02)) return rc;
+  bool launch_ok = true;
+  for (int l = 2; l < kAllLayers; ++l)
+    if (S[0].used[l] && !launch_conv_pair<T>(st, S[0].conv[l], S[1].conv[l], S[0].pool[l])) launch_ok = false;
+  {
+    const VggNormNet nets[2] = {{&S[0], (char*)br[0].workspace, &pl[0], br[0].inv_norm, br[0].feat, br[0].H, br[0].W},
+                                {&S[1], (char*)br[1].workspace, &pl[1], br[1].inv_norm, br[1].feat, br[1].H, br[1].W}};
+    if (const int rc = vgg_norms(st, 2, nets, B, 3, flags)) return rc;
   }
   HLA_CHECK_HIP(hipGetLastError());
   return launch_ok ? HLA_OK : HLA_ERR_ARG;
@@ -190,11 +278,15 @@
 template int vgg_forward_t<TuT>(const float* x, size_t x_plane, const hla_vgg_params* prm, const char* packed, int dtype, void* const feat[4],
                               float* const conf[4], double* inv_norm, char* ws, const VggPlan& pl, int B, int H, int W,
                               int flags, int first_row8, hipStream_t st);
+template int vgg_forward_pair_t<TuT>(const hla_vgg_branch br[2], const VggPlan pl[2], int B, int dtype, int flags, hipStream_t st);
 #else
 #define HLA_EXTERN_T(T) \
   extern template void vgg_pack_all<T>(const hla_vgg_params* prm, char* packed, int dtype, hipStream_t st); \
   extern template int vgg_forward_t<T>(const float* x, size_t x_plane, const hla_vgg_params* prm, const char* packed, int dtype, void* const feat[4],                               float* const conf[4], double* inv_norm, char* ws, const VggPlan& pl, int B, int H, int W,                               int flags, int first_row8, hipStream_t st);
 HLA_EXTERN_T(float) HLA_EXTERN_T(bf16) HLA_EXTERN_T(f16) HLA_EXTERN_T(split32)
+#define HLA_EXTERN_PAIR_T(T) \
+  extern template int vgg_forward_pair_t<T>(const hla_vgg_branch br[2], const VggPlan pl[2], int B, int dtype, int flags, hipStream_t st);
+HLA_EXTERN_PAIR_T(float) HLA_EXTERN_PAIR_T(bf16) HLA_EXTERN_PAIR_T(f16) HLA_EXTERN_PAIR_T(split32)
 
 extern "C" size_t hla_vgg_packed_weight_bytes(int dtype) {
   return packed_offset(kAllLayers, dtype) + (dtype == HLA_F16X3 ? kPackTailBytes : 0);
@@ -264,4 +356,37 @@
   return vgg_forward_t<float>(x, x_plane, params, (const char*)packed_weights, dtype, feat, conf, inv_norm, (char*)workspace, pl,
                               B, H, W, flags, first_row8, (hipStream_t)stream);
 }
+
+extern "C" int hla_vgg_forward_pair(const hla_vgg_branch br[2], int B, int level, int dtype, int flags, int* paired_out, hla_stream_t stream) {
+  HLA_REQUIRE(br, "hla_vgg_forward_pair: null argument");
+  if (paired_out) *paired_out = 0;
+  auto plain = [&]() -> int {
+    for (int k = 0; k < 2; ++k)
+      if (const int rc = hla_vgg_forward(br[k].x, br[k].x_plane, br[k].params, br[k].packed_weights, br[k].feat, br[k].conf, br[k].inv_norm,
+                                         br[k].workspace, br[k].workspace_bytes, B, br[k].H, br[k].W, level, dtype, flags, br[k].first_row8, stream))
+        return rc;
+    return HLA_OK;
+  };
+  if (level != 3 || (flags & (HLA_VGG_SAVE_FOR_BACKWARD | HLA_VGG_FOLD_DECODER | HLA_VGG_WANT_CONF)) || !hla_dtype_ok(dtype)) return plain();
+  VggPlan pl[2];
+  for (int k = 0; k < 2; ++k) {
+    const hla_vgg_branch& b = br[k];
+    const bool ok = b.x && b.params && b.packed_weights && b.workspace && B > 0 && b.H >= 8 && b.W >= 8 && b.H % 8 == 0 && b.W % 8 == 0 &&
+                    (b.x_plane == 0 || b.x_plane >= (size_t)b.H * b.W) && (size_t)b.H * b.W * 64 * 4 < ((size_t)1 << 31) &&
+                    b.feat[0] && b.feat[1] && b.feat[2] && (!(flags & HLA_VGG_DEFER_NORM) || b.inv_norm) &&
+                    (!(flags & HLA_VGG_FEAT16) || ((dtype == HLA_BF16 || dtype == HLA_F16) && (flags & HLA_VGG_DEFER_NORM))) &&
+                    (b.first_row8 == 0 || (b.first_row8 >= 4 && b.first_row8 < b.H / 8));
+    if (!ok) return plain();
+    vgg_plan(B, b.H, b.W, dtype, false, &pl[k], false, false);
+    if (b.workspace_bytes < pl[k].total) return plain();
+  }
+  int rc;
+  if (dtype == HLA_BF16) rc = vgg_forward_pair_t<bf16>(br, pl, B, dtype, flags, (hipStream_t)stream);
+  else if (dtype == HLA_F16) rc = vgg_forward_pair_t<f16>(br, pl, B, dtype, flags, (hipStream_t)stream);
+  else if (dtype == HLA_F16X3) rc = vgg_forward_pair_t<split32>(br, pl, B, dtype, flags, (hipStream_t)stream);
+  else rc = vgg_forward_pair_t<float>(br, pl, B, dtype, flags, (hipStream_t)stream);
+  if (rc == HLA_PAIR_FALLBACK) return plain();
+  if (rc == HLA_OK && paired_out) *paired_out = 1;
+  return rc;
+}
 #endif
diff --git a/include/hla.h b/include/hla.h
--- a/include/hla.h
+++ b/include/hla.h
@@ -26,12 +26,13 @@
 
 const char* hla_last_error(void);
 
-#define HLA_ABI_VERSION 24
+#define HLA_ABI_VERSION 25
 int hla_abi_version(void);
 const char* hla_source_hash(void);
 typedef enum hla_struct_id {
   HLA_STRUCT_VGG_PARAMS = 0, HLA_STRUCT_VGG_GRADS = 1, HLA_STRUCT_S2G_LEVEL = 2, HLA_STRUCT_S2G_CONFIG = 3,
-  HLA_STRUCT_S2G_LEVEL_GRAD = 4, HLA_STRUCT_PROF_RECORD = 5, HLA_STRUCT_POSE_LOSS_ARGS = 6, HLA_STRUCT_FILL_REGION = 7
+  HLA_STRUCT_S2G_LEVEL_GRAD = 4, HLA_STRUCT_PROF_RECORD = 5, HLA_STRUCT_POSE_LOSS_ARGS = 6, HLA_STRUCT_FILL_REGION = 7,
+  HLA_STRUCT_VGG_BRANCH = 8
 } hla_struct_id;
 size_t hla_sizeof_struct(int id);
 
@@ -58,6 +59,21 @@
 int hla_vgg_forward(const float* x, size_t x_plane, const hla_vgg_params* params, const void* packed_weights, void* const feat[4],
                     float* const conf[4], double* inv_norm, void* workspace, size_t workspace_bytes, int B, int H,
                     int W, int level, int dtype, int flags, int first_row8, hla_stream_t stream);
+
+typedef struct hla_vgg_branch {
+  const float* x;
+  size_t x_plane;
+  const hla_vgg_params* params;
+  const void* packed_weights;
+  void* feat[4];
+  float* conf[4];
+  double* inv_norm;
+  void* workspace;
+  size_t workspace_bytes;
+  int H, W, first_row8;
+} hla_vgg_branch;
+
+int hla_vgg_forward_pair(const hla_vgg_branch br[2], int B, int level, int dtype, int flags, int* paired_out, hla_stream_t stream);
 
 typedef struct hla_vgg_grads {
   float* dw[17];
```

Measured after the change: 5518 pairs/s, median of 6. +3.3%, better.
